# openpifpaf/openpifpaf

Measured on AMD Instinct MI355X. Metric: images/sec end-to-end (backbone+CifCaf decode), resnet50 641px, higher is better.
Workload: dtype f32; 1 GPU; BASELINE configs[1] scaled to a batch: resnet50 641x641, batch 32 per GPU, CIF/CAF fields [32,17,5,81,81]+[32,19,8,81,81]; backbone=resnet50, backbone_dtype=fp32, conv3x3=winograd F(2x2,3x3) f32 for the stride-1 ones, decode_dtype=f32 (+f64 where the reference uses double), global_batch=32, batch_per_gpu=32, parallelism=single GPU, force_complete_pose=False

## Files before the change

### include/openpifpaf_amd.h

```cpp
#ifndef OPENPIFPAF_AMD_H_
#define OPENPIFPAF_AMD_H_

#include <stddef.h>
#include <stdint.h>

#ifdef __cplusplus
extern "C" {
#endif

#define OPA_OK 0
#define OPA_ERR_INVALID_ARGUMENT 1
#define OPA_ERR_HIP 2
#define OPA_ERR_UNSUPPORTED 3
#define OPA_ERR_WORKSPACE 4
#define OPA_ERR_NO_DEVICE 5

#define OPA_COUNT_OVERFLOW 0x40000000
#define OPA_COUNT_FAILED 0x20000000
#define OPA_COUNT_ROWS(c) ((c) & 0x0FFFFFFF)

typedef struct opa_params {
    double cif_threshold;
    int64_t cifhr_neighbors;
    double seed_threshold;
// ... 158 lines not shown
                 int64_t rows, int32_t channels, int32_t dtype, int32_t relu, void* stream);

int opa_gemm_bias_act_bf16(const void* a_dev, const void* w_dev, const void* bias_dev, const void* residual_dev,
                           void* out_dev, int64_t m, int32_t n, int32_t k, int32_t relu, void* stream);

int opa_gemm_pro_bias_act_bf16(const void* a_dev, const void* a_bias_dev, const void* w_dev, const void* bias_dev,
                               const void* residual_dev, void* out_dev, int64_t m, int32_t n, int32_t k,
                               int32_t relu, void* stream);

int opa_gemm_bias_act_f16(const void* a_dev, const void* w_dev, const void* bias_dev, const void* residual_dev,
                          void* out_dev, int64_t m, int32_t n, int32_t k, int32_t relu, void* stream);
int opa_gemm_pro_bias_act_f16(const void* a_dev, const void* a_bias_dev, const void* w_dev, const void* bias_dev,
                              const void* residual_dev, void* out_dev, int64_t m, int32_t n, int32_t k,
                              int32_t relu, void* stream);

int opa_gemm_bias_act_f32(const float* a_dev, const float* a_bias_dev, const float* w_dev, const float* bias_dev,
                          const float* residual_dev, float* out_dev, int64_t m, int32_t n, int32_t k,
                          int32_t relu, void* stream);

int opa_gemm_bias_act_f32x3(const float* a_dev, const float* a_bias_dev, const void* w3_dev, const float* bias_dev,
                            const float* residual_dev, float* out_dev, int64_t m, int32_t n, int32_t k,
                            int32_t relu, int32_t terms, void* stream);

int opa_gemm2_bias_act_f32x3(const float* a1_dev, int32_t k1, const float* a2_dev, int32_t k2, int32_t batch, int32_t h_in,
                             int32_t w_in, int32_t stride, const float* a_bias_dev, const void* w3cat_dev, const float* bias_dev,
                             float* out_dev, int32_t n, int32_t relu, int32_t terms, void* stream);

int opa_conv3x3_f32x3(const float* x_dev, const void* w3_dev, const float* bias_dev, float* out_dev, int32_t batch, int32_t h_in,
                      int32_t w_in, int32_t c_in, int32_t c_out, int32_t stride, int32_t relu, int32_t terms, void* stream);

int opa_conv3x3_dilated_f32x3(const float* x_dev, const void* w3_dev, const float* bias_dev, float* out_dev, int32_t batch, int32_t h_in,
                              int32_t w_in, int32_t c_in, int32_t c_out, int32_t stride, int32_t dilation, int32_t relu, int32_t terms,
                              void* stream);

int opa_maxpool3x3_bias_act(const void* x_dev, const void* bias_dev, void* out_dev, int32_t dtype, int32_t batch, int32_t h, int32_t w,
                            int32_t c, int32_t stride, int32_t relu, void* stream);

int opa_maxpool3x3_ceil_bias_act(const void* x_dev, const void* bias_dev, void* out_dev, int32_t dtype, int32_t batch, int32_t h, int32_t w,
                                 int32_t c, int32_t stride, int32_t relu, void* stream);

int opa_fire_expand_f32x3(const float* h_dev, const void* w_dev, const float* bias_dev, float* out_dev, int32_t batch, int32_t h, int32_t w,
                          int32_t c_squeeze, int32_t c_e1, int32_t c_e3, int32_t terms, void* stream);

int opa_conv_rows_f32x3(const float* x_dev, const void* w3_dev, const float* bias_dev, float* out_dev, int32_t batch, int32_t hp,
                        int32_t wp, int32_t pix, int32_t ho, int32_t wo, int32_t stride, int32_t ntaps, int32_t tap_floats,
                        int32_t c_out, int32_t relu, int32_t terms, void* stream);

int opa_gemm_unit_bias_act_f32x3(const float* a_dev, int64_t a_pitch, const void* w3_dev, const float* bias_dev,
                                 const float* partner_dev, int64_t partner_pitch, float* out_dev,
                                 int64_t m, int32_t n, int32_t k, int32_t relu, int32_t terms, void* stream);

int opa_gemm_unit_act_f32x3(const float* a_dev, int64_t a_pitch, const void* w3_dev, const float* bias_dev,
                            const float* partner_dev, int64_t partner_pitch, const float* residual_dev, int64_t residual_pitch,
                            float* out_dev, int64_t m, int32_t n, int32_t k, int32_t act, int32_t terms, void* stream);

int opa_gemm_unit_actp_f32x3(const float* a_dev, int64_t a_pitch, const void* w3_dev, const float* bias_dev,
                             const float* partner_dev, int64_t partner_pitch, const float* residual_dev, int64_t residual_pitch,
                             float* out_dev, int64_t m, int32_t n, int32_t k, int32_t act, float act_param, int32_t terms, void* stream);

int opa_gemm_unit_actp_bf16(const void* a_dev, int64_t a_pitch, const void* w_dev, const float* bias_dev,
                            const void* partner_dev, int64_t partner_pitch, const void* residual_dev, int64_t residual_pitch,
                            void* out_dev, int64_t m, int32_t n, int32_t k, int32_t act, float act_param, void* stream);

int opa_conv3x3_act_bf16(const void* x_dev, const void* w_dev, const float* bias_dev, const void* residual_dev, void* out_dev,
                         int32_t batch, int32_t h_in, int32_t w_in, int32_t c_in, int32_t c_out,
                         int32_t stride, int32_t dilation, int32_t relu, void* stream);

int opa_conv3x3_act_f16(const void* x_dev, const void* w_dev, const float* bias_dev, const void* residual_dev, void* out_dev,
                        int32_t batch, int32_t h_in, int32_t w_in, int32_t c_in, int32_t c_out,
                        int32_t stride, int32_t dilation, int32_t relu, void* stream);

int opa_gconv3x3_act_bf16(const void* x_dev, const void* w_dev, const float* bias_dev, void* out_dev,
                          int32_t batch, int32_t h_in, int32_t w_in, int32_t channels, int32_t group_width,
                          int32_t stride, int32_t dilation, int32_t relu, void* stream);

int opa_stem7x7_act_bf16(const void* x_dev, int64_t x_batch_stride, int64_t x_channel_stride, int64_t x_row_stride,
                         int64_t x_pixel_stride, const void* w_dev, const float* bias_dev, void* out_dev,
                         int32_t batch, int32_t h, int32_t w, int32_t c_out, int32_t stride, int32_t relu, void* stream);

int opa_gemm2_bias_act_bf16(const void* a1_dev, int32_t k1, const void* a2_dev, int32_t k2, int32_t batch, int32_t h_in, int32_t w_in,
                            int32_t stride, const void* a_bias_dev, const void* wcat_dev, const float* bias_dev, void* out_dev,
                            int32_t n, int32_t relu, void* stream);

int opa_gemm2_bias_act_f16(const void* a1_dev, int32_t k1, const void* a2_dev, int32_t k2, int32_t batch, int32_t h_in, int32_t w_in,
                           int32_t stride, const void* a_bias_dev, const void* wcat_dev, const float* bias_dev, void* out_dev,
                           int32_t n, int32_t relu, void* stream);

int opa_conv3x3_winograd_f32(const float* x_dev, const float* u_dev, const float* bias_dev, float* out_dev, int32_t batch,
                             int32_t h, int32_t w, int32_t c_in, int32_t c_out, int32_t relu, int32_t variant,
                             int32_t order, void* stream);

int opa_conv3x3_winograd_f32x3(const float* x_dev, const void* u3_dev, const float* bias_dev, float* out_dev, int32_t batch,
                               int32_t h, int32_t w, int32_t c_in, int32_t c_out, int32_t relu, int32_t variant,
                               int32_t order, void* stream);

int opa_dwconv_bias_act(const void* x_dev, int64_t x_pixel_stride, const void* w_dev, const void* bias_dev,
                        void* out_dev, int64_t out_pixel_stride, int32_t batch, int32_t h, int32_t w,
                        int32_t channels, int32_t k, int32_t stride, int32_t dtype, int32_t relu, void* stream);

int opa_dwconv_act(const void* x_dev, int64_t x_pixel_stride, const void* w_dev, const void* bias_dev,
                   void* out_dev, int64_t out_pixel_stride, int32_t batch, int32_t h, int32_t w,
                   int32_t channels, int32_t k, int32_t stride, int32_t dtype, int32_t act, void* stream);

int opa_dwconv_dilated_act(const void* x_dev, int64_t x_pixel_stride, const void* w_dev, const void* bias_dev,
                           void* out_dev, int64_t out_pixel_stride, int32_t batch, int32_t h, int32_t w,
                           int32_t channels, int32_t k, int32_t stride, int32_t dilation, int32_t dtype, int32_t act, void* stream);

int opa_dwconv_actp(const void* x_dev, int64_t x_pixel_stride, const void* w_dev, const void* bias_dev,
                    void* out_dev, int64_t out_pixel_stride, int32_t batch, int32_t h, int32_t w,
                    int32_t channels, int32_t k, int32_t stride, int32_t dilation, int32_t dtype, int32_t act, float act_param, void* stream);

int opa_stem3x3_actp(const float* x_dev, int64_t x_batch_stride, int64_t x_channel_stride, int64_t x_row_stride,
                     int64_t x_pixel_stride, const float* w_dev, const float* bias_dev, float* out_dev,
                     int32_t batch, int32_t h, int32_t w, int32_t channels_out, int32_t stride,
                     int32_t act, float act_param, void* stream);

int opa_gconv3x3_bias_act_f32(const float* x_dev, int64_t x_pixel_stride, const float* wt_dev, const float* bias_dev,
                              float* out_dev, int64_t out_pixel_stride, int32_t batch, int32_t h, int32_t w, int32_t channels,
                              int32_t group_width, int32_t stride, int32_t relu, void* stream);

int opa_channel_interleave(const void* a_dev, int64_t a_pixel_stride, const void* b_dev, int64_t b_pixel_stride,
                           void* out_dev, int64_t rows, int32_t half, int32_t dtype, void* stream);

#define OPA_SE_POOL_PIXELS 512
size_t opa_se_workspace_bytes(int32_t batch, int64_t pixels, int32_t channels);
int opa_se_pool(const float* x_dev, int64_t x_pixel_stride, int32_t batch, int64_t pixels, int32_t channels,
                void* workspace_dev, size_t workspace_bytes, void* stream);
int opa_se_gate(const void* workspace_dev, size_t workspace_bytes, int32_t batch, int64_t pixels, int32_t channels, int32_t squeeze,
                const float* w1_dev, const float* b1_dev, const float* w2_dev, const float* b2_dev, float* gate_dev, float* mean_dev,
                void* stream);
int opa_se_scale(float* x_dev, int64_t x_pixel_stride, int32_t batch, int64_t pixels, int32_t channels, const float* gate_dev,
                 void* stream);

#define OPA_GN_CHUNK_PIXELS 512
size_t opa_groupnorm_workspace_bytes(int32_t batch, int64_t pixels, int32_t channels);
int opa_groupnorm_actp(const float* x_dev, int64_t x_pixel_stride, const float* gamma_dev, const float* beta_dev, float* out_dev,
                       int64_t out_pixel_stride, int32_t batch, int64_t pixels, int32_t channels, int32_t groups, float eps,
                       int32_t act, float act_param, void* workspace_dev, size_t workspace_bytes, void* stream);

int opa_head_epilogue(const void* conv_dev, int32_t dtype, int32_t batch, int32_t hc, int32_t wc,
                      int32_t n_fields, int32_t n_components, int32_t upsample, int32_t n_confidences,
                      int32_t n_vectors, uint32_t vector_offset_mask, int32_t n_scales, float* out_dev, void* stream);

int opa_head_conv_fields_bf16(const void* x_dev, const void* w_dev, const float* bias_dev, float* out_dev,
                              int32_t batch, int32_t hc, int32_t wc, int32_t k,
                              int32_t n_fields, int32_t n_components, int32_t upsample, int32_t n_confidences,
                              int32_t n_vectors, uint32_t vector_offset_mask, int32_t n_scales, void* stream);

int opa_head_conv_fields_f16(const void* x_dev, const void* w_dev, const float* bias_dev, float* out_dev,
                             int32_t batch, int32_t hc, int32_t wc, int32_t k,
                             int32_t n_fields, int32_t n_components, int32_t upsample, int32_t n_confidences,
                             int32_t n_vectors, uint32_t vector_offset_mask, int32_t n_scales, void* stream);

typedef struct opa_pre_image {
    int64_t src_offset;
    int64_t mid_offset;
    int32_t h0, w0;
    int32_t th, tw;
    int32_t top, left;
    int32_t x_table, x_ksize;
    int32_t y_table, y_ksize;
} opa_pre_image;
size_t opa_pre_image_bytes(void);

size_t opa_preprocess_workspace_bytes(const opa_pre_image* images_host, int32_t batch, int32_t mode);

int opa_preprocess_u8(const opa_pre_image* images_host, const opa_pre_image* images_dev, int32_t batch,
                      const uint8_t* frames_dev, size_t frames_bytes, const int32_t* tables_dev, size_t tables_words,
                      uint8_t* workspace_dev, size_t workspace_bytes, const float* lut_dev, float* out_dev,
                      int32_t canvas_h, int32_t canvas_w, int32_t mode, int32_t channels_last, uint32_t fill_rgb,
                      void* stream);

int opa_profile_begin(void* stream);
int opa_profile_end(int32_t capacity, const char** names_out, float* ms_out, int32_t* n_out);

#ifdef __cplusplus
}
#endif
#endif
```

### openpifpaf_amd/_lib.py

```python
import ctypes
import os

HERE = os.path.dirname(os.path.abspath(__file__))
LIB_PATH = os.environ.get('OPA_LIB_PATH') or os.path.join(HERE, 'lib', 'libopenpifpaf_amd.so')

OPA_OK = 0
ERROR_NAMES = {1: 'INVALID_ARGUMENT', 2: 'HIP', 3: 'UNSUPPORTED', 4: 'WORKSPACE', 5: 'NO_DEVICE'}


class NativeLibraryMissing(ImportError):
    pass


class NativeError(RuntimeError):
    pass


class Params(ctypes.Structure):
    _fields_ = [
        ('cif_threshold', ctypes.c_double),
        ('cifhr_neighbors', ctypes.c_int64),
        ('seed_threshold', ctypes.c_double),
        ('caf_threshold', ctypes.c_double),
        ('cif_floor', ctypes.c_double),
        ('keypoint_threshold', ctypes.c_double),
        ('keypoint_threshold_rel', ctypes.c_double),
        ('nms_suppression', ctypes.c_double),
        ('nms_instance_threshold', ctypes.c_double),
        ('nms_keypoint_threshold', ctypes.c_double),
        ('force_complete_caf_th', ctypes.c_double),
        ('occupancy_reduction', ctypes.c_double),
        ('occupancy_min_scale', ctypes.c_double),
        ('greedy', ctypes.c_int32),
        ('reverse_match', ctypes.c_int32),
        ('force_complete', ctypes.c_int32),
        ('block_joints', ctypes.c_int32),
        ('ablation_cifseeds_nms', ctypes.c_int32),
        ('ablation_cifseeds_no_rescore', ctypes.c_int32),
        ('ablation_caf_no_rescore', ctypes.c_int32),
        ('ablation_cifhr_skip', ctypes.c_int32),
    ]

    def copy(self):
        other = Params()
        ctypes.memmove(ctypes.byref(other), ctypes.byref(self), ctypes.sizeof(Params))
        return other


ABI_VERSION = 9


class Debug(ctypes.Structure):
    _fields_ = [
        ('stage_worklist', ctypes.c_int32), ('scored_one_pass', ctypes.c_int32),
        ('assoc_growers', ctypes.c_int32), ('assoc_bbox', ctypes.c_int32),
        ('assoc_dedup', ctypes.c_int32), ('assoc_prededup', ctypes.c_int32), ('assoc_predict', ctypes.c_int32),
        ('assoc_predict_min_v', ctypes.c_float), ('assoc_predict_th', ctypes.c_float),
        ('assoc_collide', ctypes.c_int32), ('assoc_collide_shift', ctypes.c_int32), ('assoc_inherit', ctypes.c_int32),
        ('assoc_lookahead', ctypes.c_int32),
        ('assoc_timing', ctypes.c_int32), ('assoc_persistent', ctypes.c_int32), ('fc_split', ctypes.c_int32),
        ('assoc_watchdog_ticks', ctypes.c_int64),
    ]


class DetShape(ctypes.Structure):
    _fields_ = [(n, ctypes.c_int32) for n in ('batch', 'n_fields', 'field_h', 'field_w', 'stride', 'max_detections')]


class DetPost(ctypes.Structure):
    _fields_ = [('iou_threshold', ctypes.c_double), ('suppression', ctypes.c_double),
                ('instance_threshold', ctypes.c_double), ('by_category', ctypes.c_int32)]


CIFDET_NMS_MAX = 1024


class PreImage(ctypes.Structure):
    _fields_ = [('src_offset', ctypes.c_int64), ('mid_offset', ctypes.c_int64)] + [(n, ctypes.c_int32) for n in (
        'h0', 'w0', 'th', 'tw', 'top', 'left', 'x_table', 'x_ksize', 'y_table', 'y_ksize')]


class Shape(ctypes.Structure):
    _fields_ = [(n, ctypes.c_int32) for n in (
        'batch', 'n_cif', 'n_caf', 'cif_h', 'cif_w', 'caf_h', 'caf_w',
        'cif_stride', 'caf_stride', 'max_annotations', 'n_keypoints', 'cifhr_pool_tiles')]


_vp, _i32, _i64, _dbl, _sz = ctypes.c_void_p, ctypes.c_int32, ctypes.c_int64, ctypes.c_double, ctypes.c_size_t
_P = ctypes.POINTER
SYMBOLS = {
    'opa_abi_version': (ctypes.c_int, []),
    'opa_shape_bytes': (_sz, []),
    'opa_params_bytes': (_sz, []),
    'opa_debug_bytes': (_sz, []),
    'opa_default_debug': (None, [_P(Debug)]),
    'opa_cifcaf_set_debug': (ctypes.c_int, [_vp, _P(Debug)]),
    'opa_cifcaf_get_debug': (ctypes.c_int, [_vp, _P(Debug)]),
    'opa_version': (ctypes.c_char_p, []),
    'opa_last_error': (ctypes.c_char_p, []),
    'opa_device_count': (ctypes.c_int, []),
    'opa_set_quiet': (None, [ctypes.c_int]),
    'opa_set_seed_tie_order': (None, [ctypes.c_int]),
    'opa_get_seed_tie_order': (ctypes.c_int, []),
    'opa_default_params': (None, [_P(Params)]),
    'opa_get_params': (None, [_P(Params)]),
    'opa_set_params': (ctypes.c_int, [_P(Params)]),
    'opa_cifcaf_create': (ctypes.c_int, [_P(_vp), _i32, _vp, _i32]),
    'opa_cifcaf_destroy': (None, [_vp]),
    'opa_cifcaf_get_state': (ctypes.c_int, [_vp, _P(_i32), _vp, _P(_i32)]),
    'opa_cifcaf_set_tie_placement': (ctypes.c_int, [_vp, _i32]),
    'opa_cifcaf_workspace_bytes': (_sz, [_P(Shape)]),
    'opa_cifcaf_workspace_bytes_for': (_sz, [_P(Shape), _P(Params)]),
    'opa_cifcaf_decode': (ctypes.c_int, [_vp, _P(Shape), _P(Params), _vp, _vp, _vp, _vp, _i32,
                                         _vp, _sz, _vp, _vp, _vp, _vp]),
    'opa_cifcaf_cifhr_view': (ctypes.c_int, [_P(Shape), _P(_sz), _P(_i32), _P(_i32), _P(_i32), _P(_dbl)]),
    'opa_cifcaf_get_cifhr': (ctypes.c_int, [_P(Shape), _vp, _i32, _vp, _vp]),
    'opa_cifcaf_workspace_view': (ctypes.c_int, [_P(Shape), ctypes.c_char_p, _P(_sz), _P(_sz)]),
    'opa_cifhr_pitch': (_i32, [_i32, _i32]),
    'opa_cifhr_scratch_bytes': (_sz, [_i32, _i32, _i32, _i32]),
    'opa_cifhr_accumulate': (ctypes.c_int, [_vp, _i32, _i32, _i32, _i32, _i32, _dbl, _dbl, _P(Params),
                                            _vp, _vp, _sz, _vp]),
    'opa_cifseeds_scratch_bytes': (_sz, [_i32, _i32, _i32, _i32]),
    'opa_cifseeds_fill': (ctypes.c_int, [_vp, _i32, _i32, _i32, _i32, _i32, _vp, _P(Params),
                                         _vp, _vp, _vp, _vp, _sz, _vp]),
    'opa_cifdetseeds_fill': (ctypes.c_int, [_vp, _i32, _i32, _i32, _i32, _i32, _vp, _P(Params),
                                            _vp, _vp, _vp, _vp, _sz, _vp]),
    'opa_cafscored_fill': (ctypes.c_int, [_vp, _i32, _i32, _i32, _i32, _i32, _vp, _i32, _i32, _i32, _i32,
                                          _vp, _dbl, _dbl, _P(Params), _vp, _vp, _vp]),
    'opa_grow_connection_blend': (ctypes.c_int, [_vp, _i32, _dbl, _dbl, _dbl, _dbl, _i32, _P(_dbl), _vp]),
    'opa_cifdet_workspace_bytes': (_sz, [_P(DetShape)]),
    'opa_cifdet_decode': (ctypes.c_int, [_P(DetShape), _P(Params), _vp, _vp, _sz, _vp, _vp, _vp, _vp, _vp]),
    'opa_det_post_bytes': (_sz, []),
    'opa_default_det_post': (None, [_P(DetPost)]),
    'opa_cifdet_nms': (ctypes.c_int, [_P(DetPost), _i32, _i32, _vp, _vp, _vp, _vp, _vp, _vp, _vp, _vp, _vp]),
    'opa_cifdet_decode_nms': (ctypes.c_int, [_P(DetShape), _P(Params), _P(DetPost), _vp, _vp, _sz, _vp, _vp, _vp, _vp, _vp]),
    'opa_bias_act': (ctypes.c_int, [_vp, _vp, _vp, _i64, _i32, _i32, _i32, _vp]),
    'opa_gemm_bias_act_bf16': (ctypes.c_int, [_vp, _vp, _vp, _vp, _vp, _i64, _i32, _i32, _i32, _vp]),
    'opa_gemm_pro_bias_act_bf16': (ctypes.c_int, [_vp, _vp, _vp, _vp, _vp, _vp, _i64, _i32, _i32, _i32, _vp]),
    'opa_gemm_bias_act_f16': (ctypes.c_int, [_vp, _vp, _vp, _vp, _vp, _i64, _i32, _i32, _i32, _vp]),
    'opa_gemm_pro_bias_act_f16': (ctypes.c_int, [_vp, _vp, _vp, _vp, _vp, _vp, _i64, _i32, _i32, _i32, _vp]),
    'opa_gemm_bias_act_f32': (ctypes.c_int, [_vp, _vp, _vp, _vp, _vp, _vp, _i64, _i32, _i32, _i32, _vp]),
    'opa_gemm_bias_act_f32x3': (ctypes.c_int, [_vp, _vp, _vp, _vp, _vp, _vp, _i64, _i32, _i32, _i32, _i32, _vp]),
    'opa_gemm_unit_bias_act_f32x3': (ctypes.c_int, [_vp, _i64, _vp, _vp, _vp, _i64, _vp, _i64, _i32, _i32, _i32, _i32, _vp]),
    'opa_gemm_unit_act_f32x3': (ctypes.c_int, [_vp, _i64, _vp, _vp, _vp, _i64, _vp, _i64, _vp, _i64, _i32, _i32, _i32, _i32, _vp]),
    'opa_gemm_unit_actp_f32x3': (ctypes.c_int, [_vp, _i64, _vp, _vp, _vp, _i64, _vp, _i64, _vp, _i64, _i32, _i32, _i32, ctypes.c_float, _i32,
                                                _vp]),
    'opa_gemm_unit_actp_bf16': (ctypes.c_int, [_vp, _i64, _vp, _vp, _vp, _i64, _vp, _i64, _vp, _i64, _i32, _i32, _i32, ctypes.c_float, _vp]),
    'opa_conv3x3_act_bf16': (ctypes.c_int, [_vp, _vp, _vp, _vp, _vp] + [_i32] * 8 + [_vp]),
    'opa_conv3x3_act_f16': (ctypes.c_int, [_vp, _vp, _vp, _vp, _vp] + [_i32] * 8 + [_vp]),
    'opa_gconv3x3_act_bf16': (ctypes.c_int, [_vp, _vp, _vp, _vp] + [_i32] * 8 + [_vp]),
    'opa_stem7x7_act_bf16': (ctypes.c_int, [_vp, _i64, _i64, _i64, _i64, _vp, _vp, _vp] + [_i32] * 6 + [_vp]),
    'opa_conv_rows_f32x3': (ctypes.c_int, [_vp, _vp, _vp, _vp] + [_i32] * 12 + [_vp]),
    'opa_conv3x3_f32x3': (ctypes.c_int, [_vp, _vp, _vp, _vp, _i32, _i32, _i32, _i32, _i32, _i32, _i32, _i32, _vp]),
    'opa_conv3x3_dilated_f32x3': (ctypes.c_int, [_vp, _vp, _vp, _vp] + [_i32] * 9 + [_vp]),
    'opa_maxpool3x3_bias_act': (ctypes.c_int, [_vp, _vp, _vp] + [_i32] * 7 + [_vp]),
    'opa_maxpool3x3_ceil_bias_act': (ctypes.c_int, [_vp, _vp, _vp] + [_i32] * 7 + [_vp]),
    'opa_fire_expand_f32x3': (ctypes.c_int, [_vp, _vp, _vp, _vp] + [_i32] * 7 + [_vp]),
    'opa_gemm2_bias_act_f32x3': (ctypes.c_int, [_vp, _i32, _vp, _i32, _i32, _i32, _i32, _i32, _vp, _vp, _vp, _vp, _i32, _i32, _i32, _vp]),
    'opa_gemm2_bias_act_bf16': (ctypes.c_int, [_vp, _i32, _vp, _i32, _i32, _i32, _i32, _i32, _vp, _vp, _vp, _vp, _i32, _i32, _vp]),
    'opa_gemm2_bias_act_f16': (ctypes.c_int, [_vp, _i32, _vp, _i32, _i32, _i32, _i32, _i32, _vp, _vp, _vp, _vp, _i32, _i32, _vp]),
    'opa_conv3x3_winograd_f32': (ctypes.c_int, [_vp, _vp, _vp, _vp] + [_i32] * 8 + [_vp]),
    'opa_conv3x3_winograd_f32x3': (ctypes.c_int, [_vp, _vp, _vp, _vp] + [_i32] * 8 + [_vp]),
    'opa_dwconv_bias_act': (ctypes.c_int, [_vp, _i64, _vp, _vp, _vp, _i64, _i32, _i32, _i32, _i32, _i32, _i32, _i32, _i32, _vp]),
    'opa_dwconv_act': (ctypes.c_int, [_vp, _i64, _vp, _vp, _vp, _i64, _i32, _i32, _i32, _i32, _i32, _i32, _i32, _i32, _vp]),
    'opa_dwconv_dilated_act': (ctypes.c_int, [_vp, _i64, _vp, _vp, _vp, _i64, _i32, _i32, _i32, _i32, _i32, _i32, _i32, _i32, _i32, _vp]),
    'opa_dwconv_actp': (ctypes.c_int, [_vp, _i64, _vp, _vp, _vp, _i64, _i32, _i32, _i32, _i32, _i32, _i32, _i32, _i32, _i32, ctypes.c_float,
                                       _vp]),
    'opa_stem3x3_actp': (ctypes.c_int, [_vp, _i64, _i64, _i64, _i64, _vp, _vp, _vp, _i32, _i32, _i32, _i32, _i32, _i32, ctypes.c_float, _vp]),
    'opa_gconv3x3_bias_act_f32': (ctypes.c_int, [_vp, _i64, _vp, _vp, _vp, _i64, _i32, _i32, _i32, _i32, _i32, _i32, _i32, _vp]),
    'opa_se_workspace_bytes': (_sz, [_i32, _i64, _i32]),
    'opa_se_pool': (ctypes.c_int, [_vp, _i64, _i32, _i64, _i32, _vp, _sz, _vp]),
    'opa_se_gate': (ctypes.c_int, [_vp, _sz, _i32, _i64, _i32, _i32, _vp, _vp, _vp, _vp, _vp, _vp, _vp]),
    'opa_se_scale': (ctypes.c_int, [_vp, _i64, _i32, _i64, _i32, _vp, _vp]),
    'opa_groupnorm_workspace_bytes': (_sz, [_i32, _i64, _i32]),
    'opa_groupnorm_actp': (ctypes.c_int, [_vp, _i64, _vp, _vp, _vp, _i64, _i32, _i64, _i32, _i32, ctypes.c_float, _i32, ctypes.c_float, _vp, _sz,
                                          _vp]),
    'opa_channel_interleave': (ctypes.c_int, [_vp, _i64, _vp, _i64, _vp, _i64, _i32, _i32, _vp]),
    'opa_head_epilogue': (ctypes.c_int, [_vp, _i32, _i32, _i32, _i32, _i32, _i32, _i32, _i32, _i32, ctypes.c_uint32, _i32, _vp, _vp]),
    'opa_head_conv_fields_bf16': (ctypes.c_int, [_vp, _vp, _vp, _vp] + [_i32] * 9 + [ctypes.c_uint32, _i32, _vp]),
    'opa_head_conv_fields_f16': (ctypes.c_int, [_vp, _vp, _vp, _vp] + [_i32] * 9 + [ctypes.c_uint32, _i32, _vp]),
    'opa_pre_image_bytes': (_sz, []),
    'opa_preprocess_workspace_bytes': (_sz, [_P(PreImage), _i32, _i32]),
    'opa_preprocess_u8': (ctypes.c_int, [_P(PreImage), _vp, _i32, _vp, _sz, _vp, _sz, _vp, _sz, _vp, _vp, _i32, _i32, _i32, _i32,
                                         ctypes.c_uint32, _vp]),
    'opa_profile_begin': (ctypes.c_int, [_vp]),
    'opa_profile_end': (ctypes.c_int, [_i32, _P(ctypes.c_char_p), _P(ctypes.c_float), _P(_i32)]),
}

_lib = None


def available():
    return os.path.exists(LIB_PATH)


def lib():
    global _lib
    if _lib is None:
        if not os.path.exists(LIB_PATH):
            raise NativeLibraryMissing(
                'openpifpaf_amd: %s not found. The HIP extension is required (there is no CPU path); '
                'build it with `python -c "import __graft_entry__ as g; g.build()"`.' % LIB_PATH)
        handle = ctypes.CDLL(LIB_PATH)
        for name, (restype, argtypes) in SYMBOLS.items():
            fn = getattr(handle, name)
            fn.restype = restype
            fn.argtypes = argtypes
        if handle.opa_abi_version() != ABI_VERSION or handle.opa_shape_bytes() != ctypes.sizeof(Shape) or \
                handle.opa_params_bytes() != ctypes.sizeof(Params) or handle.opa_debug_bytes() != ctypes.sizeof(Debug) or \
                handle.opa_det_post_bytes() != ctypes.sizeof(DetPost) or \
                handle.opa_pre_image_bytes() != ctypes.sizeof(PreImage):
            raise NativeError('openpifpaf_amd: %s was built from another include/openpifpaf_amd.h (ABI %d, opa_shape %d bytes, '
                              'opa_params %d, opa_debug %d, opa_det_post %d, opa_pre_image %d; this package: ABI %d, %d, %d, %d, %d, %d): '
                              'rebuild it' % (
                                  LIB_PATH, handle.opa_abi_version(), handle.opa_shape_bytes(), handle.opa_params_bytes(),
                                  handle.opa_debug_bytes(), handle.opa_det_post_bytes(), handle.opa_pre_image_bytes(),
                                  ABI_VERSION, ctypes.sizeof(Shape), ctypes.sizeof(Params), ctypes.sizeof(Debug),
                                  ctypes.sizeof(DetPost), ctypes.sizeof(PreImage)))
        _lib = handle
    return _lib


def check(code, what=''):
    if code != OPA_OK:
        msg = lib().opa_last_error().decode('utf-8', 'replace')
        raise NativeError('%s failed: OPA_ERR_%s: %s' % (what or 'native call', ERROR_NAMES.get(code, code), msg))


def default_params(**overrides):
    p = Params()
    lib().opa_default_params(ctypes.byref(p))
    for k, v in overrides.items():
        if not hasattr(p, k):
            raise AttributeError('opa_params has no field %r' % k)
        setattr(p, k, v)
    return p


def default_debug(**overrides):
    d = Debug()
    lib().opa_default_debug(ctypes.byref(d))
    for k, v in overrides.items():
        if not hasattr(d, k):
            raise AttributeError('opa_debug has no field %r' % k)
        setattr(d, k, v)
    return d


def get_params():
    p = Params()
    lib().opa_get_params(ctypes.byref(p))
    return p


def set_params(p):
    check(lib().opa_set_params(ctypes.byref(p)), 'opa_set_params')


def profile_begin(stream_ptr):
    check(lib().opa_profile_begin(stream_ptr), 'opa_profile_begin')


def profile_end(capacity=64):
    names = (ctypes.c_char_p * capacity)()
    ms = (ctypes.c_float * capacity)()
    n = ctypes.c_int32()
    check(lib().opa_profile_end(capacity, names, ms, ctypes.byref(n)), 'opa_profile_end')
    return [(names[i].decode(), float(ms[i])) for i in range(min(n.value, capacity))]
```

### openpifpaf_amd/csrc/capi_trunk.hip

```cpp
#include "capi_internal.hpp"

#include <algorithm>
#include <cmath>
#include <initializer_list>
#include <string>

using namespace opa;

namespace {
struct Entry {
    const char* fn; hipStream_t st;
    Entry(const char* fn_, void* stream) : fn(fn_), st((hipStream_t)stream) {}
    int refuse(int code, const std::string& what) const { return fail(code, std::string(fn) + ": " + what); }
    int refuse(const char* what) const { return refuse(OPA_ERR_INVALID_ARGUMENT, what); }
    int launched(hipError_t e, const char* where, const char* mark = nullptr) const {
        if (e != hipSuccess) return fail_hip(e, where);
        if (mark) prof_mark(st, mark);
        return OPA_OK;
    }
};

bool misaligned(uintptr_t mask, std::initializer_list<const void*> pointers) {
    uintptr_t bits = 0;
    for (const void* p : pointers) bits |= (uintptr_t)p;
    return (bits & mask) != 0;
}

bool bad_terms(int32_t terms) { return terms != 6 && terms != 9; }

const char* bad_act_param(int32_t act, float act_param) {
    if (!std::isfinite(act_param)) return "act_param must be finite";
    if (act == 3 && act_param < 0.0f) return "act_param must not be negative with act 3 (the LeakyReLU's slope)";
    if (act == 4 && act_param <= 0.0f) return "act_param must be positive with act 4 (the clipped ReLU's cap)";
    return nullptr;
}
}

extern "C" {

int opa_bias_act(void* x_dev, const void* bias_dev, const void* residual_dev, int64_t rows, int32_t channels,
                 int32_t dtype, int32_t relu, void* stream) {
    const Entry E("opa_bias_act", stream);
    if (!x_dev || !bias_dev || rows < 0 || channels <= 0 || dtype < 0 || dtype > 2) return E.refuse("bad arguments");
    if (channels % (dtype == 0 ? 4 : 8) != 0 || misaligned(15, {x_dev, bias_dev, residual_dev}))
        return E.refuse("channels must fill 16-byte vectors and pointers be 16-B aligned");
    if (rows == 0) return OPA_OK;
    return E.launched(launch_bias_act(x_dev, bias_dev, residual_dev, rows, channels, dtype, relu, E.st), "bias_act", "bias_act_kernel");
}

static int gemm_bf16(const char* fn, int dtype, bool pro, const void* a_dev, const void* a_bias_dev, const void* w_dev, const void* bias_dev,
                     const void* residual_dev, void* out_dev, int64_t m, int32_t n, int32_t k, int32_t relu, void* stream) {
    const Entry E(fn, stream);
    if (!a_dev || (pro && !a_bias_dev) || !w_dev || !bias_dev || !out_dev || m < 0 || n <= 0 || k <= 0 || m > 0x7fffffffll)
        return E.refuse("bad arguments");
    if (k % 64 != 0 || n % 64 != 0) return E.refuse("K and N must be multiples of 64");
    if (misaligned(15, {a_dev, a_bias_dev, w_dev, out_dev, residual_dev})) return E.refuse("pointers must be 16-B aligned");
    if (m == 0) return OPA_OK;
    const hipError_t e = launch_gemm_bias_act(a_dev, w_dev, bias_dev, residual_dev, out_dev, (int)m, n, k, relu, E.st, a_bias_dev, dtype);
    if (dtype == 1)
        return E.launched(e, pro ? "gemm_pro_bias_act_f16" : "gemm_bias_act_f16", pro ? "gemm_pro_bias_act_f16_kernel" : "gemm_bias_act_f16_kernel");
    return E.launched(e, pro ? "gemm_pro_bias_act" : "gemm_bias_act", pro ? "gemm_pro_bias_act_kernel" : "gemm_bias_act_kernel");
}

int opa_gemm_bias_act_bf16(const void* a_dev, const void* w_dev, const void* bias_dev, const void* residual_dev,
                           void* out_dev, int64_t m, int32_t n, int32_t k, int32_t relu, void* stream) {
    return gemm_bf16("opa_gemm_bias_act_bf16", 2, false, a_dev, nullptr, w_dev, bias_dev, residual_dev, out_dev, m, n, k, relu, stream);
}

int opa_gemm_pro_bias_act_bf16(const void* a_dev, const void* a_bias_dev, const void* w_dev, const void* bias_dev,
                               const void* residual_dev, void* out_dev, int64_t m, int32_t n, int32_t k,
                               int32_t relu, void* stream) {
    return gemm_bf16("opa_gemm_pro_bias_act_bf16", 2, true, a_dev, a_bias_dev, w_dev, bias_dev, residual_dev, out_dev, m, n, k, relu, stream);
}

int opa_gemm_bias_act_f16(const void* a_dev, const void* w_dev, const void* bias_dev, const void* residual_dev,
                          void* out_dev, int64_t m, int32_t n, int32_t k, int32_t relu, void* stream) {
    return gemm_bf16("opa_gemm_bias_act_f16", 1, false, a_dev, nullptr, w_dev, bias_dev, residual_dev, out_dev, m, n, k, relu, stream);
}

int opa_gemm_pro_bias_act_f16(const void* a_dev, const void* a_bias_dev, const void* w_dev, const void* bias_dev,
                              const void* residual_dev, void* out_dev, int64_t m, int32_t n, int32_t k,
                              int32_t relu, void* stream) {
    return gemm_bf16("opa_gemm_pro_bias_act_f16", 1, true, a_dev, a_bias_dev, w_dev, bias_dev, residual_dev, out_dev, m, n, k, relu, stream);
}

int opa_gemm_bias_act_f32(const float* a_dev, const float* a_bias_dev, const float* w_dev, const float* bias_dev,
                          const float* residual_dev, float* out_dev, int64_t m, int32_t n, int32_t k,
                          int32_t relu, void* stream) {
    const Entry E("opa_gemm_bias_act_f32", stream);
    if (!a_dev || !w_dev || !bias_dev || !out_dev || m < 0 || n <= 0 || k <= 0 || m > 0x7fffffffll) return E.refuse("bad arguments");
    if (k % 32 != 0 || n % 64 != 0) return E.refuse("K must be a multiple of 32 and N of 64");
    if (misaligned(15, {a_dev, a_bias_dev, w_dev, out_dev, residual_dev, bias_dev})) return E.refuse("pointers must be 16-B aligned");
    if (m == 0) return OPA_OK;
    return E.launched(launch_gemm_f32_bias_act(a_dev, w_dev, bias_dev, residual_dev, out_dev, (int)m, n, k, relu, E.st, a_bias_dev),
                      "gemm_f32_bias_act", a_bias_dev ? "gemm_f32_pro_bias_act_kernel" : "gemm_f32_bias_act_kernel");
}

int opa_gemm_bias_act_f32x3(const float* a_dev, const float* a_bias_dev, const void* w3_dev, const float* bias_dev,
                            const float* residual_dev, float* out_dev, int64_t m, int32_t n, int32_t k,
                            int32_t relu, int32_t terms, void* stream) {
    const Entry E("opa_gemm_bias_act_f32x3", stream);
    if (!a_dev || !w3_dev || !bias_dev || !out_dev || m < 0 || n <= 0 || k <= 0 || m > 0x7fffffffll || bad_terms(terms))
        return E.refuse("bad arguments");
    if (k % 64 != 0 || n % 64 != 0) return E.refuse("K and N must be multiples of 64");
    if (misaligned(15, {a_dev, a_bias_dev, w3_dev, out_dev, residual_dev, bias_dev})) return E.refuse("pointers must be 16-B aligned");
    if (m == 0) return OPA_OK;
    return E.launched(launch_gemm_f32x3_bias_act(a_dev, (const unsigned short*)w3_dev, bias_dev, residual_dev, out_dev, (int)m, n, k, relu,
                                                 terms, E.st, a_bias_dev), "gemm_f32x3_bias_act", "gemm_f32x3_bias_act_kernel");
}

int opa_gemm2_bias_act_f32x3(const float* a1_dev, int32_t k1, const float* a2_dev, int32_t k2, int32_t batch, int32_t h_in,
                             int32_t w_in, int32_t stride, const float* a_bias_dev, const void* w3cat_dev, const float* bias_dev,
                             float* out_dev, int32_t n, int32_t relu, int32_t terms, void* stream) {
    const Entry E("opa_gemm2_bias_act_f32x3", stream);
    if (!a1_dev || !a2_dev || !w3cat_dev || !bias_dev || !out_dev || batch <= 0 || h_in <= 0 || w_in <= 0 || stride < 1 || n <= 0 ||
        k1 <= 0 || k2 <= 0 || bad_terms(terms))
        return E.refuse("bad arguments");
    if (k1 % 32 != 0 || (k1 + k2) % 64 != 0 || k2 % 4 != 0 || n % 64 != 0) return E.refuse("k1 % 32, (k1 + k2) % 64, k2 % 4, N % 64 must be 0");
    if (misaligned(15, {a1_dev, a2_dev, a_bias_dev, w3cat_dev, out_dev, bias_dev})) return E.refuse("pointers must be 16-B aligned");
    const long long ho = (h_in - 1) / stride + 1, wo = (w_in - 1) / stride + 1;
    if ((long long)batch * ho * wo > 0x7fffffffll || (long long)batch * h_in * w_in > 0x7fffffffll) return E.refuse("too many pixels");
    return E.launched(launch_gemm2_f32x3_bias_act(a1_dev, k1, a2_dev, k2, batch, h_in, w_in, stride, (const unsigned short*)w3cat_dev,
                                                  bias_dev, out_dev, n, relu, terms, E.st, a_bias_dev),
                      "gemm2_f32x3_bias_act", "gemm2_f32x3_bias_act_kernel");
}

int opa_conv_rows_f32x3(const float* x_dev, const void* w3_dev, const float* bias_dev, float* out_dev, int32_t batch, int32_t hp,
                        int32_t wp, int32_t pix, int32_t ho, int32_t wo, int32_t stride, int32_t ntaps, int32_t tap_floats,
                        int32_t c_out, int32_t relu, int32_t terms, void* stream) {
    const Entry E("opa_conv_rows_f32x3", stream);
    if (!x_dev || !w3_dev || !bias_dev || !out_dev || batch <= 0 || hp <= 0 || wp <= 0 || pix <= 0 || ho <= 0 || wo <= 0 || stride < 1 ||
        ntaps < 1 || ntaps > 32 || tap_floats <= 0 || c_out <= 0 || bad_terms(terms))
        return E.refuse("bad arguments");
    if (tap_floats % 32 != 0 || (ntaps * tap_floats) % 64 != 0 || c_out % 64 != 0 || pix % 4 != 0)
        return E.refuse("tap_floats % 32, ntaps * tap_floats % 64, c_out % 64, pix % 4 must be 0");
    if (misaligned(15, {x_dev, w3_dev, out_dev, bias_dev})) return E.refuse("pointers must be 16-B aligned");
    if ((long long)(ho - 1) * stride + ntaps > hp || ((long long)(wo - 1) * stride) * pix + tap_floats > (long long)wp * pix ||
        (long long)batch * hp * wp * pix * 4 > 0x7fffffffll || (long long)batch * ho * wo > 0x7fffffffll)
        return E.refuse("the taps leave the (padded) input, or it is 2 GB or more");
    return E.launched(launch_convrows_f32x3(x_dev, batch, hp, wp, pix, ho, wo, stride, ntaps, tap_floats, (const unsigned short*)w3_dev,
                                            bias_dev, out_dev, c_out, relu, terms, E.st), "conv_rows_f32x3", "conv_rows_f32x3_kernel");
}

static int conv3x3_f32x3(const char* fn, const float* x_dev, const void* w3_dev, const float* bias_dev, float* out_dev, int32_t batch,
                         int32_t h_in, int32_t w_in, int32_t c_in, int32_t c_out, int32_t stride, int32_t dilation, int32_t relu,
                         int32_t terms, void* stream) {
    const Entry E(fn, stream);
    if (!x_dev || !w3_dev || !bias_dev || !out_dev || batch < 0 || h_in < 0 || w_in < 0 || stride < 1 || dilation < 1 || c_in <= 0 ||
        c_out <= 0 || bad_terms(terms))
        return E.refuse("bad arguments");
    if (c_in % 64 != 0 || c_out % 64 != 0) return E.refuse("c_in and c_out must be multiples of 64");
    if (misaligned(15, {x_dev, w3_dev, out_dev, bias_dev})) return E.refuse("pointers must be 16-B aligned");
    if (((double)batch * h_in * w_in + (double)dilation * ((double)w_in + 1.0)) * c_in * 4.0 >= 2147483648.0)
// ... 360 lines not shown
    if (!stem3x3_channels_ok(channels_out)) return E.refuse("channels_out must be 16, 24, 32, 42 or 64");
    if (act < 0 || act > 4) return E.refuse("act must be 0 (none), 1 (ReLU), 2 (hardswish), 3 (LeakyReLU) or 4 (clipped ReLU)");
    if (const char* why = bad_act_param(act, act_param)) return E.refuse(why);
    if (batch == 0) return OPA_OK;
    const double last = ((double)batch - 1.0) * (double)x_batch_stride + 2.0 * (double)x_channel_stride +
                        ((double)h - 1.0) * (double)x_row_stride + ((double)w - 1.0) * (double)x_pixel_stride;
    if (last >= 2147483648.0) return E.refuse("x must span fewer than 2^31 elements (32-bit indices)");
    const double ho = (h - 1) / stride + 1, wo = (w - 1) / stride + 1;
    if ((double)batch * ho * wo * channels_out >= 2147483648.0) return E.refuse("out must hold fewer than 2^31 elements (32-bit indices)");
    if (batch > 65535) return E.refuse("batch must not exceed 65535 (grid.y)");
    return E.launched(launch_stem3x3(x_dev, x_batch_stride, x_channel_stride, x_row_stride, x_pixel_stride, w_dev, bias_dev, out_dev, batch,
                                     h, w, channels_out, stride, act, act_param, E.st), "stem3x3", "stem3x3_kernel");
}

static const char* se_check(int64_t x_pixel_stride, int32_t batch, int64_t pixels, int32_t channels) {
    if (batch <= 0 || batch > 65535 || pixels <= 0 || pixels > 65535ll * kSePoolPixels || channels <= 0 || channels > 8192)
        return "batch, pixels or channels out of range";
    if (channels % 4 != 0 || x_pixel_stride % 4 != 0 || x_pixel_stride < channels) return "channels and the pixel stride must be multiples of 4, the stride >= channels";
    return nullptr;
}

size_t opa_se_workspace_bytes(int32_t batch, int64_t pixels, int32_t channels) {
    if (batch <= 0 || pixels <= 0 || channels <= 0) return 0;
    return (size_t)batch * (size_t)se_pool_chunks(pixels) * (size_t)channels * sizeof(double);
}

int opa_se_pool(const float* x_dev, int64_t x_pixel_stride, int32_t batch, int64_t pixels, int32_t channels,
                void* workspace_dev, size_t workspace_bytes, void* stream) {
    const Entry E("opa_se_pool", stream);
    if (!x_dev || !workspace_dev) return E.refuse("bad arguments");
    if (const char* why = se_check(x_pixel_stride, batch, pixels, channels)) return E.refuse(why);
    if (misaligned(15, {x_dev, workspace_dev})) return E.refuse("pointers must be 16-B aligned");
    if (workspace_bytes < opa_se_workspace_bytes(batch, pixels, channels)) return E.refuse(OPA_ERR_WORKSPACE, "the workspace is too small");
    return E.launched(launch_se_pool(x_dev, x_pixel_stride, batch, pixels, channels, (double*)workspace_dev, E.st), "se pool");
}

int opa_se_gate(const void* workspace_dev, size_t workspace_bytes, int32_t batch, int64_t pixels, int32_t channels, int32_t squeeze,
                const float* w1_dev, const float* b1_dev, const float* w2_dev, const float* b2_dev, float* gate_dev, float* mean_dev,
                void* stream) {
    const Entry E("opa_se_gate", stream);
    if (!workspace_dev || !w1_dev || !b1_dev || !w2_dev || !b2_dev || !gate_dev || squeeze <= 0 || squeeze > 4096)
        return E.refuse("bad arguments");
    if (const char* why = se_check(channels, batch, pixels, channels)) return E.refuse(why);
    if (misaligned(15, {workspace_dev})) return E.refuse("workspace_dev must be 16-B aligned");
    if (workspace_bytes < opa_se_workspace_bytes(batch, pixels, channels)) return E.refuse(OPA_ERR_WORKSPACE, "the workspace is too small");
    return E.launched(launch_se_gate((const double*)workspace_dev, batch, pixels, channels, squeeze, w1_dev, b1_dev, w2_dev, b2_dev,
                                     gate_dev, mean_dev, E.st), "se gate");
}

int opa_se_scale(float* x_dev, int64_t x_pixel_stride, int32_t batch, int64_t pixels, int32_t channels, const float* gate_dev,
                 void* stream) {
    const Entry E("opa_se_scale", stream);
    if (!x_dev || !gate_dev) return E.refuse("bad arguments");
    if (const char* why = se_check(x_pixel_stride, batch, pixels, channels)) return E.refuse(why);
    if (misaligned(15, {x_dev, gate_dev})) return E.refuse("pointers must be 16-B aligned");
    return E.launched(launch_se_scale(x_dev, x_pixel_stride, batch, pixels, channels, gate_dev, E.st), "se scale");
}

size_t opa_groupnorm_workspace_bytes(int32_t batch, int64_t pixels, int32_t channels) {
    if (batch <= 0 || pixels <= 0 || channels <= 0) return 0;
    return groupnorm_partial_bytes(batch, pixels, channels) + (size_t)batch * (size_t)channels * 2 * sizeof(float);
}

int opa_groupnorm_actp(const float* x_dev, int64_t x_pixel_stride, const float* gamma_dev, const float* beta_dev, float* out_dev,
                       int64_t out_pixel_stride, int32_t batch, int64_t pixels, int32_t channels, int32_t groups, float eps,
                       int32_t act, float act_param, void* workspace_dev, size_t workspace_bytes, void* stream) {
    const Entry E("opa_groupnorm_actp", stream);
    if (!x_dev || !out_dev) return E.refuse("x_dev and out_dev must not be NULL");
    if (misaligned(7, {x_dev, out_dev}) || misaligned(3, {gamma_dev, beta_dev}) || misaligned(15, {workspace_dev}))
        return E.refuse("x_dev / out_dev must be 8-B, gamma_dev / beta_dev 4-B, workspace_dev 16-B aligned");
    if (batch < 0 || pixels <= 0 || channels <= 0 || groups <= 0)
        return E.refuse("batch must not be negative, pixels, channels and groups must be positive");
    if (channels % groups != 0) return E.refuse("channels must be a multiple of groups");
    if ((channels / groups) % 2 != 0) return E.refuse("channels / groups must be even");
    if (x_pixel_stride % 2 != 0 || out_pixel_stride % 2 != 0 || x_pixel_stride < channels || out_pixel_stride < channels)
        return E.refuse("pixel strides must be even and at least channels");
    if (!std::isfinite(eps) || eps < 0.0f) return E.refuse("eps must be finite and not negative");
    if (act < 0 || act > 4) return E.refuse("act must be 0 (none), 1 (ReLU), 2 (hardswish), 3 (LeakyReLU) or 4 (clipped ReLU)");
    if (const char* why = bad_act_param(act, act_param)) return E.refuse(why);
    if (out_dev == x_dev && out_pixel_stride != x_pixel_stride) return E.refuse("out_dev == x_dev (in place) needs equal pixel strides");
    if (batch == 0) return OPA_OK;
    if (batch > 65535) return E.refuse("batch must not exceed 65535 (grid.y)");
    if (pixels > 65535ll * kGnChunkPixels) return E.refuse("pixels must not exceed 65535 * OPA_GN_CHUNK_PIXELS (grid.y)");
    if (channels / groups > kGnMaxGroupWidth) return E.refuse("channels / groups must not exceed 2048");
    if ((double)pixels * (double)(channels / 2) >= 2147483648.0)
        return E.refuse("pixels * channels / 2 must stay below 2^31 (32-bit vector indices within an image)");
    if (!workspace_dev) return E.refuse(OPA_ERR_WORKSPACE, "workspace_dev must not be NULL");
    if (workspace_bytes < opa_groupnorm_workspace_bytes(batch, pixels, channels)) return E.refuse(OPA_ERR_WORKSPACE, "the workspace is too small");
    return E.launched(launch_groupnorm(x_dev, x_pixel_stride, gamma_dev, beta_dev, out_dev, out_pixel_stride, batch, pixels, channels, groups,
                                       eps, act, act_param, workspace_dev, E.st), "group norm");
}

int opa_channel_interleave(const void* a_dev, int64_t a_pixel_stride, const void* b_dev, int64_t b_pixel_stride,
                           void* out_dev, int64_t rows, int32_t half, int32_t dtype, void* stream) {
    const Entry E("opa_channel_interleave", stream);
    if (!a_dev || !b_dev || !out_dev || rows <= 0 || half <= 0 || a_pixel_stride < half || b_pixel_stride < half ||
        dtype < 0 || dtype > 2)
        return E.refuse("bad arguments");
    return E.launched(launch_channel_interleave(a_dev, a_pixel_stride, b_dev, b_pixel_stride, out_dev, rows, half, dtype, E.st),
                      "channel interleave");
}

int opa_head_epilogue(const void* conv_dev, int32_t dtype, int32_t batch, int32_t hc, int32_t wc,
                      int32_t n_fields, int32_t n_components, int32_t upsample, int32_t n_confidences,
                      int32_t n_vectors, uint32_t vector_offset_mask, int32_t n_scales, float* out_dev, void* stream) {
    const Entry E("opa_head_epilogue", stream);
    if (!conv_dev || !out_dev || batch <= 0 || hc <= 0 || wc <= 0 || n_fields <= 0 || n_components <= 0 ||
        dtype < 0 || dtype > 2 || (upsample != 1 && upsample != 2) || n_confidences < 0 || n_vectors < 0 || n_scales < 0 ||
        1 + n_confidences + 2 * n_vectors + n_scales > n_components)
        return E.refuse("bad arguments");
    return E.launched(launch_head_epilogue(conv_dev, dtype, batch, hc, wc, n_fields, n_components, upsample, n_confidences,
                                           n_vectors, vector_offset_mask, n_scales, out_dev, E.st), "head epilogue");
}

static int head_conv_fields_16(const char* fn, int dtype, const void* x_dev, const void* w_dev, const float* bias_dev, float* out_dev,
                               int32_t batch, int32_t hc, int32_t wc, int32_t k, int32_t n_fields, int32_t n_components, int32_t upsample,
                               int32_t n_confidences, int32_t n_vectors, uint32_t vector_offset_mask, int32_t n_scales, void* stream) {
    const Entry E(fn, stream);
    if (!x_dev || !w_dev || !bias_dev || !out_dev) return E.refuse("x_dev, w_dev, bias_dev and out_dev must not be NULL");
    if (misaligned(15, {x_dev, w_dev}) || misaligned(3, {bias_dev, out_dev}))
        return E.refuse("x_dev / w_dev must be 16-B, bias_dev / out_dev 4-B aligned");
    if (batch < 0) return E.refuse("negative batch");
    if (hc <= 0 || wc <= 0 || k <= 0 || n_fields <= 0 || n_components <= 0) return E.refuse("hc, wc, k, n_fields and n_components must be positive");
    if (k % 64 != 0) return E.refuse("k must be a multiple of 64");
    if (upsample != 1 && upsample != 2) return E.refuse("upsample must be 1 or 2");
    if (n_confidences < 0 || n_vectors < 0 || n_scales < 0 || 1ll + n_confidences + 2ll * n_vectors + n_scales != n_components)
        return E.refuse("n_components must be 1 + n_confidences + 2 * n_vectors + n_scales, no count negative");
    const double pixels = (double)batch * hc * wc, n = (double)n_fields * n_components * upsample * upsample;
    if (pixels * k >= 2147483648.0) return E.refuse("x must hold fewer than 2^31 elements (32-bit offsets)");
    if (n > 2147483584.0) return E.refuse("n_fields * n_components * upsample^2 must not exceed 2^31 - 64");
    const double ho = (double)hc * upsample - (upsample - 1), wo = (double)wc * upsample - (upsample - 1);
    if ((double)batch * n_fields * n_components * ho * wo >= 2147483648.0) return E.refuse("out must hold fewer than 2^31 elements (32-bit offsets)");
    if (batch == 0) return OPA_OK;
    if (head16_workgroups(batch, hc, wc, n_fields, n_components, upsample) > 0x7fffffffll) return E.refuse("too many tiles for grid.x");
    return E.launched(launch_head16(x_dev, w_dev, bias_dev, out_dev, batch, hc, wc, k, n_fields, n_components, upsample, n_confidences, n_vectors,
                                    vector_offset_mask, n_scales, E.st, dtype), dtype == 1 ? "head_conv_fields_f16" : "head_conv_fields_bf16",
                      dtype == 1 ? "head16_f16_kernel" : "head16_bf16_kernel");
}

int opa_head_conv_fields_bf16(const void* x_dev, const void* w_dev, const float* bias_dev, float* out_dev,
                              int32_t batch, int32_t hc, int32_t wc, int32_t k,
                              int32_t n_fields, int32_t n_components, int32_t upsample, int32_t n_confidences,
                              int32_t n_vectors, uint32_t vector_offset_mask, int32_t n_scales, void* stream) {
    return head_conv_fields_16("opa_head_conv_fields_bf16", 2, x_dev, w_dev, bias_dev, out_dev, batch, hc, wc, k, n_fields, n_components, upsample,
                               n_confidences, n_vectors, vector_offset_mask, n_scales, stream);
}

int opa_head_conv_fields_f16(const void* x_dev, const void* w_dev, const float* bias_dev, float* out_dev,
                             int32_t batch, int32_t hc, int32_t wc, int32_t k,
                             int32_t n_fields, int32_t n_components, int32_t upsample, int32_t n_confidences,
                             int32_t n_vectors, uint32_t vector_offset_mask, int32_t n_scales, void* stream) {
    return head_conv_fields_16("opa_head_conv_fields_f16", 1, x_dev, w_dev, bias_dev, out_dev, batch, hc, wc, k, n_fields, n_components, upsample,
                               n_confidences, n_vectors, vector_offset_mask, n_scales, stream);
}

size_t opa_pre_image_bytes(void) { return sizeof(opa_pre_image); }

static size_t pre_mid_bytes(const opa_pre_image& d) { return align_up((size_t)d.h0 * (((size_t)d.tw * 3 + 15) & ~(size_t)15)); }

static bool check_pre_sizes(const opa_pre_image* images, int32_t batch, const char* who, std::string* why) {
    if (!images) { *why = std::string(who) + ": images_host is null"; return false; }
    if (batch < 1 || batch > 65535) { *why = std::string(who) + ": batch must be 1..65535"; return false; }
    for (int32_t b = 0; b < batch; b++) {
        const opa_pre_image& d = images[b];
        const char* field = d.h0 < 1 ? "h0" : d.w0 < 1 ? "w0" : d.th < 1 ? "th" : d.tw < 1 ? "tw" : nullptr;
        if (field) { *why = std::string(who) + ": images[" + std::to_string(b) + "]." + field + " must be at least 1"; return false; }
        if ((int64_t)d.h0 * d.w0 > 0x3fffffff || (int64_t)d.h0 * d.tw > 0x3fffffff) {
            *why = std::string(who) + ": images[" + std::to_string(b) + "]: h0 * w0 and h0 * tw must stay below 2^30"; return false;
        }
    }
    return true;
}

size_t opa_preprocess_workspace_bytes(const opa_pre_image* images_host, int32_t batch, int32_t mode) {
    std::string why;
    if (!check_pre_sizes(images_host, batch, "opa_preprocess_workspace_bytes", &why)) { fail(0, why); return 0; }
    if (mode != 0 && mode != 1) { fail(0, "opa_preprocess_workspace_bytes: mode must be 0 or 1"); return 0; }
    size_t total = 0;
    if (mode == 0)
        for (int32_t b = 0; b < batch; b++)
            if (images_host[b].tw != images_host[b].w0) total += pre_mid_bytes(images_host[b]);
    return total;
}

int opa_preprocess_u8(const opa_pre_image* images_host, const opa_pre_image* images_dev, int32_t batch,
                      const uint8_t* frames_dev, size_t frames_bytes, const int32_t* tables_dev, size_t tables_words,
                      uint8_t* workspace_dev, size_t workspace_bytes, const float* lut_dev, float* out_dev,
                      int32_t canvas_h, int32_t canvas_w, int32_t mode, int32_t channels_last, uint32_t fill_rgb,
                      void* stream) {
    const char* who = "opa_preprocess_u8";
    auto bad = [&](const std::string& what) { return fail(OPA_ERR_INVALID_ARGUMENT, std::string(who) + ": " + what); };
    if (!images_dev) return bad("images_dev is null");
    if (!frames_dev) return bad("frames_dev is null");
    if (!tables_dev) return bad("tables_dev is null");
    if (!lut_dev) return bad("lut_dev is null");
    if (!out_dev) return bad("out_dev is null");
    std::string why;
    if (!check_pre_sizes(images_host, batch, who, &why)) return fail(OPA_ERR_INVALID_ARGUMENT, why);
    if (mode != 0 && mode != 1) return bad("mode must be 0 (Pillow) or 1 (zoom)");
    if (canvas_h < 1 || canvas_h > 65535) return bad("canvas_h must be 1..65535");
    if (canvas_w < 1) return bad("canvas_w must be at least 1");
    if (((uintptr_t)frames_dev | (uintptr_t)tables_dev | (uintptr_t)workspace_dev | (uintptr_t)images_dev) & 15)
        return bad("frames_dev, tables_dev, workspace_dev and images_dev must be 16-B aligned");
    if (frames_bytes % 16) return bad("frames_bytes must be a multiple of 16");
    unsigned h_blocks = 0;
    int in_cap = 1;
    size_t ws_need = 0;
    for (int32_t b = 0; b < batch; b++) {
        const opa_pre_image& d = images_host[b];
        const std::string at = "images[" + std::to_string(b) + "].";
        if (d.top < 0 || d.left < 0 || (int64_t)d.top + d.th > canvas_h || (int64_t)d.left + d.tw > canvas_w)
            return bad(at + "top / left: the placement lies outside the canvas");
        if (d.x_ksize < 1) return bad(at + "x_ksize must be at least 1");
        if (d.y_ksize < 1) return bad(at + "y_ksize must be at least 1");
        if (d.src_offset < 0 || (uint64_t)d.src_offset + (uint64_t)d.h0 * d.w0 * 3 > frames_bytes)
            return bad(at + "src_offset: the frame lies outside frames_bytes");
        const size_t x_words = mode ? ((3 * (size_t)d.tw + 1) & ~(size_t)1) + 4 * (size_t)d.tw : (size_t)(1 + d.x_ksize) * d.tw;
        const size_t y_words = mode ? ((3 * (size_t)d.th + 1) & ~(size_t)1) + 4 * (size_t)d.th : (size_t)(1 + d.y_ksize) * d.th;
        if (d.x_table < 0 || d.x_table % 4 || (size_t)d.x_table + x_words > tables_words)
            return bad(at + "x_table: the table lies outside tables_words or is not a multiple of 4 words");
        if (d.y_table < 0 || d.y_table % 4 || (size_t)d.y_table + y_words > tables_words)
            return bad(at + "y_table: the table lies outside tables_words or is not a multiple of 4 words");
        double span;
        if (mode) {
            if (d.x_ksize != 2 || d.y_ksize != 2) return bad(at + "x_ksize / y_ksize must be 2 in mode 1");
            span = std::ceil(255.0 * (d.tw > 1 ? (double)(d.w0 - 1) / (d.tw - 1) : 0.0)) + 3.0;
        } else if (d.tw != d.w0) {
            const double scale = (double)d.w0 / d.tw;
            span = std::ceil(255.0 * scale) + 2.0 * std::ceil(std::max(scale, 1.0)) + 4.0;
            if (d.mid_offset < 0 || d.mid_offset % 16) return bad(at + "mid_offset must be a non-negative multiple of 16");
            ws_need = std::max(ws_need, (size_t)d.mid_offset + pre_mid_bytes(d));
            const unsigned chunks = ((unsigned)d.tw + 255u) / 256u;
            h_blocks = std::max(h_blocks, (unsigned)d.h0 * chunks);
        } else {
            span = 1.0;
        }
        in_cap = std::max(in_cap, (int)std::min(span, (double)d.w0));
    }
    const size_t lds = mode ? preprocess_zoom_lds_bytes(in_cap) : preprocess_h_lds_bytes(in_cap);
    if (lds > 65536) return bad("w0 / tw: 256 output columns reach more source pixels than 64 KB of LDS hold");
    if (ws_need > 0 && !workspace_dev) return bad("workspace_dev is null");
    if (ws_need > workspace_bytes)
        return fail(OPA_ERR_WORKSPACE, std::string(who) + ": workspace_bytes is " + std::to_string(workspace_bytes) + ", the batch needs " + std::to_string(ws_need));
    hipError_t e = launch_preprocess(images_dev, batch, frames_dev, tables_dev, workspace_dev, lut_dev, out_dev, canvas_h, canvas_w,
                                     mode, channels_last, fill_rgb, h_blocks, in_cap, (hipStream_t)stream);
    if (e != hipSuccess) return fail_hip(e, "image preprocessing");
    return OPA_OK;
}

}
```

### openpifpaf_amd/csrc/common.hpp

```cpp
#pragma once

#include <hip/hip_runtime.h>
#include <stdint.h>
#include <stddef.h>
#include <type_traits>

#include "../../include/openpifpaf_amd.h"

namespace opa {

constexpr int kWave = 64;
constexpr int kHrTileW = 64;
constexpr int kHrTileH = 32;
constexpr int kHrLdsPitch = kHrTileW + 16;
constexpr int kSortLdsKeys = 8192;

struct Layout {
    int B, F, K, A, H, W, cH, cW, stride, cstride, max_ann;
    int hr_rows, hr_cols, hr_pitch;
    int hr_tpp, hr_pool_cap;
    int hr_spill_cap;
    int occ_h, occ_w;
    int cif_cells;
    int caf_cells;
// ... 119 lines not shown

struct AssocArgs {
    int B, K, F, A, max_ann, n_initial;
    int hr_rows, hr_cols;
    int occ_h, occ_w;
    int seed_cap, list_cap;
    const int32_t* seed_f; const float* seed_vxys; const int32_t* seed_count;
    const int32_t* seed_cell;
    const float* lists; const int32_t* list_counts;
    const float* lists_fc; const int32_t* list_counts_fc;
    const float* list_bbox;
    const float* list_bbox_fc;
    int bbox_chunks;
    const int32_t* hr_overflow;
    int tie_fused;
    TieArgs tie; SortArgs tie_sort;
    int timing;
    int collide;
    int inherit;
    size_t private_bytes;
    int dedup;
    const float* caf_raw; int caf_w; float caf_stride;
    int coll_shift;
    int lookahead;
    float predict_min_v;
    int predict; float predict_th;
    int prededup;
    int32_t* fc_meta;
    long long watchdog_ticks;
    int32_t* queue_order; int32_t* queue_head;
    int max_growers, fc_split;
    unsigned* occ;
    size_t occ_image_words;
    int32_t* stats;
    int32_t* trace;
    double* anns;
    int64_t* ann_ids;
    const float* initial; const int64_t* initial_ids;
    float* out; int64_t* out_ids; int32_t* out_count;
    int32_t* status;
};
void make_tie_args(TieArgs* a, SortArgs* g, unsigned long long* keys, int sort_cap, const int32_t* seed_count, const float* cif,
                   int F, int NC, int HW, int stride, int32_t* seed_f, float* seed_vxys, int32_t* seed_cell, int occ_h, int occ_w,
                   const TieScratch& t);
hipError_t launch_cifseeds_ties(const TieArgs& a, const SortArgs& g, int B, const DevParams& p, hipStream_t st);
hipError_t launch_assoc(const AssocArgs& a, const DevSkeleton& sk, const DevParams& p, hipStream_t st, const opa_debug& dbg);

struct DetArgs {
    int B, F, max_det, occ_h, occ_w, seed_cap;
    const int32_t* seed_f; const float* seed_vxywh; const int32_t* seed_count;
    unsigned char* occ;
    int64_t* categories; float* scores; float* boxes; int32_t* counts;
};
hipError_t launch_cifdet_collect(const DetArgs& a, const DevParams& p, hipStream_t st);

constexpr int kDetNmsMax = 1024;
struct DetNmsArgs {
    int B, max_det, by_category;
    double iou_threshold; float suppression, instance_threshold;
    const int64_t* categories; const float* scores; const float* boxes; const int32_t* counts;
    int64_t* out_categories; float* out_scores; float* out_boxes; int32_t* out_counts;
};
size_t cifdet_nms_lds_bytes(int max_det);
hipError_t launch_cifdet_nms(const DetNmsArgs& a, hipStream_t st);

hipError_t launch_bias_act(void* x, const void* bias, const void* res, long long rows, int channels, int dtype,
                           int relu, hipStream_t st);

template <auto... Vs, typename T, typename F>
hipError_t with_value(T v, F&& f) {
    hipError_t e = hipErrorInvalidValue;
    (void)((v == Vs && (e = f(std::integral_constant<decltype(Vs), Vs>{}), true)) || ...);
    return e;
}
template <typename F>
hipError_t with_flag(bool v, F&& f) { return with_value<false, true>(v, f); }

hipError_t launch_gemm_bias_act(const void* A, const void* W, const void* bias, const void* res, void* out,
                                int M, int N, int K, int relu, hipStream_t st, const void* a_bias, int dtype);

hipError_t launch_gemm_f32x3_bias_act(const float* A, const unsigned short* W3, const float* bias, const float* res, float* out,
                                      int M, int N, int K, int relu, int terms, hipStream_t st, const float* a_bias);
hipError_t launch_gemm2_f32x3_bias_act(const float* A1, int K1, const float* A2, int K2, int batch, int hi, int wi, int stride,
                                       const unsigned short* W3, const float* bias, float* out, int N, int relu, int terms,
                                       hipStream_t st, const float* a_bias);
hipError_t launch_convrows_f32x3(const float* x, int batch, int hp, int wp, int pix, int ho, int wo, int stride, int ntaps, int tap_floats,
                                 const unsigned short* W3, const float* bias, float* out, int N, int relu, int terms, hipStream_t st);
hipError_t launch_conv3x3_f32x3(const float* x, int batch, int hi, int wi, int C, int stride, int dilation, const unsigned short* W3,
                                const float* bias, float* out, int N, int relu, int terms, hipStream_t st);
int maxpool3x3_out(int h, int ceil_mode);
long long maxpool3x3_blocks(int B, int H, int W, int C, int ceil_mode = 0);
hipError_t launch_maxpool3x3(const void* x, const void* bias, void* out, int dtype, int B, int H, int W, int C, int relu, hipStream_t st,
                             int ceil_mode = 0);
bool stem3x3_channels_ok(int C);
long long stem3x3_tiles(int H, int W, int S);
hipError_t launch_stem3x3(const float* x, long long xb, long long xc, long long xr, long long xp, const float* w, const float* bias,
                          float* out, int B, int H, int W, int C, int S, int act, float act_param, hipStream_t st);
long long fire_expand_workgroups(int B, int H, int W);
hipError_t launch_fire_expand(const float* h, const unsigned short* w3, const float* bias, float* out, int B, int H, int W, int S,
                              int E1, int E3, int terms, hipStream_t st);
hipError_t launch_gemm_unit_act_f32x3(const float* A, int lda, const unsigned short* W3, const float* bias, const float* partner, int ldp,
                                      const float* residual, int ldr, float* out, int M, int N, int K, int act, int terms, hipStream_t st,
                                      float act_param = 0.0f);
hipError_t launch_gemm_unit_act_bf16(const void* A, long long lda, const void* W, const float* bias, const void* partner, long long ldp,
                                     const void* residual, long long ldr, void* out, int M, int n, int k, int act, float act_param,
                                     hipStream_t st);
long long conv3x3_bf16_workgroups(int B, int H, int W, int c_out, int S);
hipError_t launch_conv3x3_bf16(const void* x, const void* w, const float* bias, const void* residual, void* out, int B, int H, int W,
                               int c_in, int c_out, int S, int D, int relu, hipStream_t st, int dtype);
long long gconv3x3_bf16_workgroups(int B, int H, int W, int C, int S);
hipError_t launch_gconv3x3_bf16(const void* x, const void* w, const float* bias, void* out, int B, int H, int W, int C, int CG, int S,
                                int D, int relu, hipStream_t st);
long long stem7x7_bf16_workgroups(int B, int H, int W, int c_out, int S);
hipError_t launch_stem7x7_bf16(const void* x, long long xb, long long xc, long long xr, long long xp, const void* w, const float* bias,
                               void* out, int B, int H, int W, int c_out, int S, int relu, hipStream_t st);
long long gemm2_bf16_workgroups(int B, int H, int W, int n, int S);
hipError_t launch_gemm2_bf16(const void* a1, int k1, const void* x, int k2, int B, int H, int W, int S, const void* a_bias,
                             const void* wcat, const float* bias, void* out, int n, int relu, hipStream_t st, int dtype);
hipError_t launch_gemm_f32_bias_act(const float* A, const float* W, const float* bias, const float* res, float* out,
                                    int M, int N, int K, int relu, hipStream_t st, const float* a_bias = nullptr);
hipError_t launch_winograd_f23(const float* x, const float* U, float* y, const float* bias, int N, int H, int W, int Cin,
                               int Cout, int relu, int variant, int nb_major, hipStream_t st);
hipError_t launch_winograd_f23x3(const float* x, const unsigned short* U3, float* y, const float* bias, int N, int H, int W,
                                 int Cin, int Cout, int relu, int variant, int nb_major, hipStream_t st);

hipError_t launch_dwconv(const void* x, long long xs, const void* w, const void* bias, void* out, long long os,
                         int B, int H, int W, int C, int K, int S, int D, int dtype, int act, hipStream_t st, float cap = 0.0f);
hipError_t launch_channel_interleave(const void* a, long long as, const void* b, long long bs, void* out,
                                     long long rows, int half, int dtype, hipStream_t st);

long long gconv3x3_workgroups(int H, int W, int C, int S);
hipError_t launch_gconv3x3(const float* x, long long xs, const float* wt, const float* bias, float* out, long long os,
                           int B, int H, int W, int C, int CG, int S, int relu, hipStream_t st);

constexpr int kSePoolPixels = 512;
inline long long se_pool_chunks(long long hw) { return (hw + kSePoolPixels - 1) / kSePoolPixels; }
hipError_t launch_se_pool(const float* x, long long xs, int B, long long HW, int C, double* partial, hipStream_t st);
hipError_t launch_se_gate(const double* partial, int B, long long HW, int C, int S, const float* w1, const float* b1,
                          const float* w2, const float* b2, float* gate, float* mean_out, hipStream_t st);
hipError_t launch_se_scale(float* x, long long xs, int B, long long HW, int C, const float* gate, hipStream_t st);

constexpr int kGnChunkPixels = 512;
constexpr int kGnMaxGroupWidth = 2048;
inline long long gn_chunks(long long hw) { return (hw + kGnChunkPixels - 1) / kGnChunkPixels; }
size_t groupnorm_partial_bytes(int B, long long HW, int C);
hipError_t launch_groupnorm(const float* x, long long xs, const float* gamma, const float* beta, float* out, long long os, int B,
                            long long HW, int C, int G, float eps, int act, float act_param, void* workspace, hipStream_t st);

hipError_t launch_head_epilogue(const void* conv, int dtype, int B, int Hc, int Wc, int n_fields, int n_comp, int us,
                                int n_conf, int n_vec, unsigned offset_mask, int n_scales, float* out, hipStream_t st);
long long head16_workgroups(int B, int hc, int wc, int n_fields, int n_comp, int us);
hipError_t launch_head16(const void* x, const void* w, const float* bias, float* out, int B, int hc, int wc, int K, int n_fields,
                         int n_comp, int us, int n_conf, int n_vec, unsigned offset_mask, int n_scales, hipStream_t st, int dtype);

size_t preprocess_h_lds_bytes(int in_cap);
size_t preprocess_zoom_lds_bytes(int in_cap);
hipError_t launch_preprocess(const opa_pre_image* images, int batch, const unsigned char* frames, const int32_t* tables,
                             unsigned char* ws, const float* lut, float* out, int ch, int cw, int precise, int channels_last,
                             unsigned fill, unsigned h_blocks, int in_cap, hipStream_t st);

hipError_t launch_blend(const float* rows, int n, double x, double y, double s, double filter_sigmas,
                        int only_max, double* out4_dev, hipStream_t st);

}

#ifdef __HIPCC__
namespace opa {

__device__ __forceinline__ void sync_global() {
    __builtin_amdgcn_fence(__ATOMIC_RELEASE, "workgroup");
    __builtin_amdgcn_s_waitcnt(0x0F70);
    __builtin_amdgcn_s_barrier();
    __builtin_amdgcn_fence(__ATOMIC_ACQUIRE, "agent");
}

__device__ __forceinline__ int seed_cell_pack(const DevParams& p, int occ_h, int occ_w, double x, double y, double sigma);

__device__ __forceinline__ int lane_id() { return threadIdx.x & (kWave - 1); }

__device__ __forceinline__ float hardsigmoid_f32(float x) { return fminf(fmaxf(x + 3.0f, 0.0f), 6.0f) / 6.0f; }
__device__ __forceinline__ float hardswish_f32(float x) { return x * fminf(fmaxf(x + 3.0f, 0.0f), 6.0f) / 6.0f; }

__device__ __forceinline__ float x3_act_param(float x, int act, float p) {
    if (act == 3) return x < 0.0f ? x * p : x;
    return x < 0.0f ? 0.0f : (x > p ? p : x);
}

__device__ __forceinline__ float act_f32(float x, int act, float p) {
    if (act == 0) return x;
    if (act == 1) return x < 0.0f ? 0.0f : x;
    if (act == 2) return hardswish_f32(x);
    return x3_act_param(x, act, p);
}

__device__ __forceinline__ long long clampll(long long v, long long lo, long long hi) {
    return v < lo ? lo : (v > hi ? hi : v);
}

__device__ __forceinline__ long long trunc_ll(float v) { return (long long)v; }
__device__ __forceinline__ long long trunc_ll(double v) { return (long long)v; }

__device__ __forceinline__ int seed_cell_pack(const DevParams& p, int occ_h, int occ_w, double x, double y, double sigma) {
    if (p.occupancy_inv_reduction != 0.0) {
        x *= p.occupancy_inv_reduction; y *= p.occupancy_inv_reduction;
        sigma = fmax(p.occupancy_min_scale_reduced, sigma * p.occupancy_inv_reduction);
    } else if (p.occupancy_reduction != 1.0) {
        x /= p.occupancy_reduction; y /= p.occupancy_reduction;
        sigma = fmax(p.occupancy_min_scale_reduced, sigma / p.occupancy_reduction);
    }
    const int xi = (int)clampll(trunc_ll(x), 0, occ_w - 1), yi = (int)clampll(trunc_ll(y), 0, occ_h - 1);
    const int half = (int)fmin(fmax(sigma, 1.0), 255.0);
    return xi | (yi << 12) | (half << 24);
}

__device__ __forceinline__ float cifhr_value(const float* hr_image, int F, int rows, int cols, int pitch,
                                             long long f, float x, float y, float default_value,
                                             const unsigned* touch = nullptr, int touch_words = 0, int tiles_x = 0,
                                             const int32_t* slot = nullptr, int tpp = 0) {
    const float max_x = (float)((double)(float)cols - 0.51);
    const float max_y = (float)((double)(float)rows - 0.51);
    if (f >= F || (double)x < -0.49 || (double)y < -0.49 || x > max_x || y > max_y) return default_value;
    const long long yi = (long long)((double)y + 0.5);
    const long long xi = (long long)((double)x + 0.5);
    float raw;
    if (slot) {
        const int t = (int)(yi / kHrTileH) * tiles_x + (int)(xi / kHrTileW);
        const int sl = slot[(size_t)f * tpp + t];
        if (sl < 0) return default_value;
        raw = hr_image[(size_t)sl * (kHrTileH * kHrTileW) + (size_t)(yi % kHrTileH) * kHrTileW + (size_t)(xi % kHrTileW)];
    } else {
        if (touch) {
            const int t = (int)(yi / kHrTileH) * tiles_x + (int)(xi / kHrTileW);
            if (!((touch[(size_t)f * touch_words + (t >> 5)] >> (t & 31)) & 1u)) return default_value;
        }
        raw = hr_image[((size_t)f * rows + yi) * pitch + xi];
    }
    const float value = (float)((double)raw - 1.0);
    if ((double)value < 0.0) return default_value;
    return value;
}

}
#endif
```

### openpifpaf_amd/csrc/gemm_f32x3.hip

```cpp
#include <cstdlib>
#include <type_traits>
#include "common.hpp"
#include "split_bf16.hpp"

namespace opa {

typedef __attribute__((ext_vector_type(8))) __bf16 bf16x8_t;
typedef __attribute__((ext_vector_type(16))) float f32x16_t;
typedef __attribute__((ext_vector_type(4))) float f32x4_t;
typedef __attribute__((ext_vector_type(4))) unsigned int u32x4_t;
typedef __attribute__((ext_vector_type(2))) unsigned int u32x2_t;
typedef __attribute__((ext_vector_type(2))) float f32x2_t;

#ifndef OPA_X3_BK
#define OPA_X3_BK 32
#endif
#ifndef OPA_X3_WGS
#define OPA_X3_WGS 2
#endif
#ifndef OPA_X3_DIAG
#define OPA_X3_DIAG 0
#endif
#ifndef OPA_X3_ONE_ACC
#define OPA_X3_ONE_ACC 0
#endif
#ifndef OPA_X3_SWIZZLE
#define OPA_X3_SWIZZLE 1
#endif
constexpr int kX3BM = 128, kX3BK = OPA_X3_BK, kX3Pitch = OPA_X3_SWIZZLE ? kX3BK : kX3BK + 8;
__device__ __forceinline__ int x3_lds(int row, int k) {
    if (OPA_X3_SWIZZLE && kX3BK == 32) return row * kX3Pitch + ((((k >> 3) ^ (row >> 2)) & 3) << 3) + (k & 7);
    return row * kX3Pitch + k;
}

struct X3Second {
    const float* A2 = nullptr;
    int K1 = 0;
    int ho_wo = 1, wo = 1, hi_wi = 1, wi = 1, stride = 1;
    int hi = 1, C = 0, batch = 1;
    int pix = 1, taps_x = 1, ntaps = 1, padded = 0;
    int dil = 1;
    int lda = 0, ldp = 0, n_real = 0, k_real = 0;
    int act = 0; float act_param = 0.0f;
};

constexpr int kUxAct = 3, kUxHardswish = 2, kUxResidual = 4, kUxActParam = 8;

template <int BN, bool PARTNER, bool RELU, int UX = 0>
__device__ __forceinline__ void x3_unit_epilogue(float* smem_f, const f32x16_t (&acc)[2][BN / 64], const f32x16_t (&low)[2][BN / 64],
                                                 const float* __restrict__ bias, const float* __restrict__ partner,
                                                 float* __restrict__ out, int M, int m0, int n0, int lane, int wave, int ldp, int n_real,
                                                 int act, float act_param) {
    constexpr int WN = BN / 2, NT = WN / 32;
    constexpr int PPR = WN / 2;
    constexpr int PPL = 32 * PPR / 64;
    constexpr int PPRE = PPL > 8 ? 8 : PPL;
    const int wm = wave >> 1, wn = wave & 1;
    float* patch = smem_f + wave * (32 * WN);
#pragma unroll
    for (int i = 0; i < 2; i++) {
        f32x2_t pv[PPRE];
        if (PARTNER) {
#pragma unroll
            for (int t = 0; t < PPRE; t++) {
                const int v = t * 64 + lane;
                const int row = v / PPR, col = n0 + wn * WN + (v % PPR) * 2;
                const int m = m0 + wm * 64 + i * 32 + row;
                pv[t] = (f32x2_t){0.f, 0.f};
                if (m < M && col < n_real) pv[t] = *reinterpret_cast<const f32x2_t*>(partner + (size_t)m * ldp + col);
            }
        }
#pragma unroll
        for (int j = 0; j < NT; j++) {
            const int col = j * 32 + (lane & 31);
            const float b = bias[n0 + wn * WN + col];
#pragma unroll
            for (int r = 0; r < 16; r++) {
                const int row = (r & 3) + 8 * (r >> 2) + 4 * (lane >> 5);
                patch[row * WN + col] = (OPA_X3_ONE_ACC ? acc[i][j][r] : acc[i][j][r] + low[i][j][r]) + b;
            }
        }
        __builtin_amdgcn_fence(__ATOMIC_ACQ_REL, "wavefront");
        __builtin_amdgcn_wave_barrier();
#pragma unroll
        for (int t = 0; t < PPL; t++) {
            const int v = t * 64 + lane;
            const int row = v / PPR, c2 = (v % PPR) * 2, col = n0 + wn * WN + c2;
            const int m = m0 + wm * 64 + i * 32 + row;
            if (m < M && col < n_real) {
                f32x2_t f = *reinterpret_cast<const f32x2_t*>(patch + row * WN + c2);
                if constexpr (PARTNER && (UX & kUxResidual) != 0) {
                    f32x2_t pp;
                    if (t < PPRE) pp = pv[t < PPRE ? t : 0];
                    else pp = *reinterpret_cast<const f32x2_t*>(partner + (size_t)m * ldp + col);
                    f[0] += pp[0]; f[1] += pp[1];
                }
                if (RELU) { f[0] = fmaxf(f[0], 0.0f); f[1] = fmaxf(f[1], 0.0f); }
                if constexpr ((UX & kUxAct) == kUxHardswish) { f[0] = hardswish_f32(f[0]); f[1] = hardswish_f32(f[1]); }
                if constexpr ((UX & kUxActParam) != 0) { f[0] = x3_act_param(f[0], act, act_param); f[1] = x3_act_param(f[1], act, act_param); }
                if (PARTNER && (UX & kUxResidual) == 0) {
                    f32x2_t pp;
                    if (t < PPRE) pp = pv[t < PPRE ? t : 0];
                    else pp = *reinterpret_cast<const f32x2_t*>(partner + (size_t)m * ldp + col);
                    *reinterpret_cast<f32x4_t*>(out + (size_t)m * (2 * (size_t)n_real) + 2 * col) = (f32x4_t){pp[0], f[0], pp[1], f[1]};
                } else {
                    *reinterpret_cast<f32x2_t*>(out + (size_t)m * n_real + col) = f;
                }
            }
        }
        __builtin_amdgcn_fence(__ATOMIC_ACQ_REL, "wavefront");
        __builtin_amdgcn_wave_barrier();
        asm volatile("" ::: "memory");
    }
}

template <int BN, bool RES, bool RELU, bool PRO, int TERMS, int SRC, bool UNIT = false, int UX = 0>
__global__ __launch_bounds__(256, OPA_X3_WGS) void gemm_f32x3_bias_act_kernel(
        const float* __restrict__ A, const unsigned short* __restrict__ W3, const float* __restrict__ bias,
        const float* __restrict__ res, float* __restrict__ out, int M, int N, int K, const float* __restrict__ a_bias,
        const X3Second sec) {
    constexpr int WN = BN / 2;
    constexpr int NT = WN / 32;
    constexpr int LDS_A = kX3BM * kX3Pitch, LDS_B = BN * kX3Pitch;
#ifndef OPA_X3_PAD_LDS
#define OPA_X3_PAD_LDS 0
#endif
    constexpr int STAGE_BYTES = 3 * (LDS_A + LDS_B) * 2 + OPA_X3_PAD_LDS;
    constexpr int EPI_BYTES = 4 * 32 * WN * 4;
    constexpr int SMEM_BYTES = STAGE_BYTES > EPI_BYTES ? STAGE_BYTES : EPI_BYTES;
    __shared__ __attribute__((aligned(16))) unsigned char smem[SMEM_BYTES + (RES && !UNIT ? BN * 4 : 0)];
    unsigned short* sA = reinterpret_cast<unsigned short*>(smem);
    unsigned short* sB = sA + 3 * LDS_A;

    const int tid = threadIdx.x, lane = tid & 63, wave = tid >> 6;
    const int wm = wave >> 1, wn = wave & 1;
    const int n_tiles = N / BN;
    const unsigned nwg = gridDim.x, xcd = blockIdx.x & 7u, in_xcd = blockIdx.x >> 3;
    const unsigned q = nwg >> 3, r8 = nwg & 7u;
    const unsigned logical = (xcd < r8 ? xcd * (q + 1) : r8 * (q + 1) + (xcd - r8) * q) + in_xcd;
    const int m0 = (int)(logical / n_tiles) * kX3BM;
    const int n0 = (int)(logical % n_tiles) * BN;

    constexpr int NL = OPA_X3_ONE_ACC ? 1 : 2;
    f32x16_t acc[2][NT], low_[NL][NT];
    f32x16_t (&low)[2][NT] = OPA_X3_ONE_ACC ? acc : reinterpret_cast<f32x16_t (&)[2][NT]>(low_);
#pragma unroll
    for (int i = 0; i < 2; i++)
#pragma unroll
        for (int j = 0; j < NT; j++)
#pragma unroll
            for (int r = 0; r < 16; r++) { acc[i][j][r] = 0.0f; if (!OPA_X3_ONE_ACC) low[i][j][r] = 0.0f; }

    constexpr int VA = kX3BK / 4;
    constexpr int RPP = 256 / VA;
    constexpr int NPA = kX3BM / RPP;
    constexpr int WQ = kX3BK / 8;
    const int s_row = tid / VA, s_col = (tid % VA) * 4;
    constexpr int WTOT = 3 * BN * WQ;
    constexpr int WV = (WTOT + 255) / 256;
    f32x4_t ra0[NPA], ra1[NPA];
    u32x4_t rb[WV];
    constexpr bool TWO = SRC == 1, TAPS = SRC == 2;
    const int rows_here = M - m0 < kX3BM ? M - m0 : kX3BM;
    const int KA = TWO ? sec.K1 : TAPS ? sec.C : UNIT ? sec.lda : K;
    const int shift = TAPS && !sec.padded ? sec.dil * (sec.wi + 1) * sec.pix : 0;
    const float* a1_base = TAPS ? A - (size_t)shift : A + (size_t)m0 * KA;
    const int a1_bytes = TAPS ? (int)(((size_t)sec.batch * sec.hi_wi * sec.pix + shift) * 4)
                       : UNIT ? (int)(((size_t)(rows_here - 1) * KA + sec.k_real) * 4) : (int)((size_t)rows_here * KA * 4);
    const __amdgpu_buffer_rsrc_t a_rsrc = __builtin_amdgcn_make_buffer_rsrc(const_cast<float*>(a1_base), 0, a1_bytes, 0x00020000);
    const int K2 = K - KA;
    auto in_row = [&](int m) -> long long {
        const int b = m / sec.ho_wo, r = m - b * sec.ho_wo, oy = r / sec.wo, ox = r - oy * sec.wo;
        return (long long)b * sec.hi_wi + (long long)oy * sec.stride * sec.wi + (long long)ox * sec.stride;
    };
    long long row0_2 = 0;
    const float* a2_base = nullptr;
    int a2_bytes = 0;
    unsigned pa2[NPA];
    if constexpr (TWO) {
        row0_2 = in_row(__builtin_amdgcn_readfirstlane(m0));
        const int m_end = m0 + rows_here - 1;
        a2_base = sec.A2 + (size_t)row0_2 * K2;
        a2_bytes = (int)((size_t)(in_row(__builtin_amdgcn_readfirstlane(m_end)) - row0_2 + 1) * K2 * 4);
    }
    const __amdgpu_buffer_rsrc_t w_rsrc = __builtin_amdgcn_make_buffer_rsrc(
        const_cast<unsigned short*>(W3 + (size_t)n0 * K), 0, (int)(((size_t)3 * N - n0) * K * 2), 0x00020000);
    unsigned pa[NPA], pb[WV];
    unsigned vmask[NPA];
    int sb_off[WV];
#pragma unroll
    for (int p = 0; p < NPA; p++) {
        int m = m0 + p * RPP + s_row;
        if (m > M - 1) m = M - 1;
        pa[p] = ((unsigned)(m - m0) * (unsigned)KA + (unsigned)s_col) * 4u;
        vmask[p] = 0u;
        if constexpr (TAPS) {
            const int b = m / sec.ho_wo, r = m - b * sec.ho_wo, oy = r / sec.wo, ox = r - oy * sec.wo;
            pa[p] = (unsigned)((long long)b * sec.hi_wi + (long long)oy * sec.stride * sec.wi + (long long)ox * sec.stride) * (unsigned)sec.pix * 4u
                    + (unsigned)s_col * 4u;
            if (sec.padded) vmask[p] = 0xffffffffu;
            else
                for (int t = 0; t < sec.ntaps; t++) {
                    const int iy = oy * sec.stride - sec.dil + sec.dil * (t / sec.taps_x), ix = ox * sec.stride - sec.dil + sec.dil * (t % sec.taps_x);
                    if (iy >= 0 && iy < sec.hi && ix >= 0 && ix < sec.wi) vmask[p] |= 1u << t;
                }
        }
        if constexpr (TWO) pa2[p] = ((unsigned)(in_row(m) - row0_2) * (unsigned)K2 + (unsigned)s_col) * 4u;
    }
#pragma unroll
    for (int t = 0; t < WV; t++) {
        const int v = t * 256 + tid < WTOT ? t * 256 + tid : WTOT - 1;
        const int plane = v / (BN * WQ), rem = v - plane * (BN * WQ), row = rem / WQ, c = (rem % WQ) * 8;
        pb[t] = (((unsigned)plane * (unsigned)N + (unsigned)row) * (unsigned)K + (unsigned)c) * 2u;
        sb_off[t] = plane * LDS_B + x3_lds(row, c);
    }
    auto fetch_a = [&](f32x4_t (&ra)[NPA], int k0) {
        if constexpr (TAPS) {
            const int t = k0 / KA, kc = k0 - t * KA;
            const int soff = (int)((((unsigned)(sec.dil * (t / sec.taps_x)) * (unsigned)sec.wi + (unsigned)(sec.dil * (t % sec.taps_x))) * (unsigned)sec.pix + (unsigned)kc) * 4u);
#pragma unroll
            for (int p = 0; p < NPA; p++)
                ra[p] = __builtin_bit_cast(f32x4_t, __builtin_amdgcn_raw_buffer_load_b128(a_rsrc, (vmask[p] >> t) & 1u ? pa[p] : 0xFFFFFFF0u, soff, 0));
        } else if constexpr (TWO) {
            const bool second = k0 >= KA;
            const __amdgpu_buffer_rsrc_t rs = __builtin_amdgcn_make_buffer_rsrc(
                const_cast<float*>(second ? a2_base : a1_base), 0, second ? a2_bytes : a1_bytes, 0x00020000);
            const int ks = (second ? k0 - KA : k0) * 4;
#pragma unroll
            for (int p = 0; p < NPA; p++)
                ra[p] = __builtin_bit_cast(f32x4_t, __builtin_amdgcn_raw_buffer_load_b128(rs, second ? pa2[p] : pa[p], ks, 0));
        } else if constexpr (UNIT) {
#pragma unroll
            for (int p = 0; p < NPA; p++) {
                const f32x2_t lo = __builtin_bit_cast(f32x2_t, __builtin_amdgcn_raw_buffer_load_b64(a_rsrc, pa[p], k0 * 4, 0));
                const f32x2_t hi = __builtin_bit_cast(f32x2_t, __builtin_amdgcn_raw_buffer_load_b64(a_rsrc, pa[p] + 8u, k0 * 4, 0));
                ra[p] = (f32x4_t){lo[0], lo[1], hi[0], hi[1]};
            }
        } else {
#pragma unroll
            for (int p = 0; p < NPA; p++) ra[p] = __builtin_bit_cast(f32x4_t, __builtin_amdgcn_raw_buffer_load_b128(a_rsrc, pa[p], k0 * 4, 0));
        }
        if (PRO) {
            const f32x4_t ab = *reinterpret_cast<const f32x4_t*>(a_bias + k0 + s_col);
#pragma unroll
            for (int p = 0; p < NPA; p++)
#pragma unroll
                for (int e = 0; e < 4; e++) ra[p][e] = fmaxf(ra[p][e] + ab[e], 0.0f);
        }
    };
    auto fetch_b = [&](int k0) {
#pragma unroll
        for (int t = 0; t < WV; t++) rb[t] = __builtin_bit_cast(u32x4_t, __builtin_amdgcn_raw_buffer_load_b128(w_rsrc, pb[t], k0 * 2, 0));
    };
    auto store = [&](const f32x4_t (&ra)[NPA], int kt) {
#pragma unroll
        for (int p = 0; p < NPA; p++) {
            u32x2_t p1, p2, p3;
            if (OPA_X3_DIAG == 1) { p1[0] = __float_as_uint(ra[p][0]); p1[1] = __float_as_uint(ra[p][2]); p2 = p1; p3 = p1; }
            else if constexpr (UNIT) {
                const bool in0 = kt + s_col < sec.k_real, in1 = kt + s_col + 2 < sec.k_real;
                const f32x4_t v = {in0 ? ra[p][0] : 0.0f, in0 ? ra[p][1] : 0.0f, in1 ? ra[p][2] : 0.0f, in1 ? ra[p][3] : 0.0f};
                split4(v, p1, p2, p3);
            }
            else split4(ra[p], p1, p2, p3);
            unsigned short* d = sA + x3_lds(p * RPP + s_row, s_col);
            *reinterpret_cast<u32x2_t*>(d) = p1;
            *reinterpret_cast<u32x2_t*>(d + LDS_A) = p2;
            *reinterpret_cast<u32x2_t*>(d + 2 * LDS_A) = p3;
        }
#pragma unroll
        for (int t = 0; t < WV; t++)
            if (WTOT % 256 == 0 || t * 256 + tid < WTOT) *reinterpret_cast<u32x4_t*>(sB + sb_off[t]) = rb[t];
    };
    constexpr int VEC_PER_ROW = WN / 4;
    constexpr int VPL = 32 * VEC_PER_ROW / 64;
    constexpr int VRA = 1;
    constexpr bool TAIL_RES = RES && !UNIT;
    f32x4_t rres[2][TAIL_RES ? VPL : 1];
    auto fetch_res = [&](int i, int t_begin, int t_end) {
        if constexpr (TAIL_RES) {
            const __amdgpu_buffer_rsrc_t r_rsrc = __builtin_amdgcn_make_buffer_rsrc(
                const_cast<float*>(res + (size_t)m0 * N + n0), 0, (int)(((size_t)(rows_here - 1) * N + BN) * 4), 0x00020000);
            const int lrow = wm * 64 + lane / VEC_PER_ROW;
            const unsigned off = ((unsigned)lrow * (unsigned)N + (unsigned)(wn * WN + (lane % VEC_PER_ROW) * 4)) * 4u;
#pragma unroll
            for (int t = t_begin; t < t_end; t++) {
                const int urow = i * 32 + t * (64 / VEC_PER_ROW);
                rres[i][t] = __builtin_bit_cast(f32x4_t, __builtin_amdgcn_raw_buffer_load_b128(
                    r_rsrc, lrow < rows_here - urow ? off : 0xFFFFFFF0u, urow * N * 4, 0));
            }
        }
    };
    int frag_a[kX3BK / 16], frag_b[kX3BK / 16];
    if constexpr (TAIL_RES) {
#pragma unroll
        for (int h = 0; h < kX3BK / 16; h++) {
            frag_a[h] = 2 * x3_lds(wm * 64 + (lane & 31), h * 16 + (lane >> 5) * 8);
            frag_b[h] = 2 * x3_lds(wn * WN + (lane & 31), h * 16 + (lane >> 5) * 8);
            asm volatile("" : "+v"(frag_a[h]), "+v"(frag_b[h]));
        }
    }
    auto step = [&](auto tail, int k0, f32x4_t (&cur)[NPA], f32x4_t (&nxt)[NPA]) {
        constexpr int TAIL = decltype(tail)::value;
        const bool more = TAIL == 1 || (TAIL == 0 && k0 + kX3BK < K);
        const int k_last = K - kX3BK;
        if constexpr (TAIL == 0) {
            fetch_b(k0 + kX3BK < k_last ? k0 + kX3BK : k_last);
            fetch_a(nxt, k0 + 2 * kX3BK < k_last ? k0 + 2 * kX3BK : k_last);
        } else if constexpr (TAIL == 1) {
            fetch_b(k_last);
            fetch_res(0, 0, VRA);
        } else {
            fetch_res(0, VRA, VPL);
        }
        __builtin_amdgcn_sched_barrier(0);
#pragma unroll
        for (int kk = 0; kk < kX3BK; kk += 16) {
            bf16x8_t fa[3][2], fb[3][NT];
            const int kh = OPA_X3_DIAG == 4 ? 0 : kk / 16;
            const int kof = kh * 16 + (lane >> 5) * 8;
#pragma unroll
            for (int pl = 0; pl < 3; pl++) {
#pragma unroll
                for (int i = 0; i < 2; i++)
                    fa[pl][i] = *reinterpret_cast<const bf16x8_t*>(TAIL_RES ? reinterpret_cast<const unsigned short*>(smem + frag_a[kh]) + (pl * LDS_A + i * 32 * kX3Pitch)
                                                                       : sA + pl * LDS_A + x3_lds(wm * 64 + i * 32 + (lane & 31), kof));
#pragma unroll
                for (int j = 0; j < NT; j++)
                    fb[pl][j] = *reinterpret_cast<const bf16x8_t*>(TAIL_RES ? reinterpret_cast<const unsigned short*>(smem + frag_b[kh]) + (3 * LDS_A + pl * LDS_B + j * 32 * kX3Pitch)
                                                                       : sB + pl * LDS_B + x3_lds(wn * WN + j * 32 + (lane & 31), kof));
            }
#pragma unroll
            for (int i = 0; i < 2; i++)
#pragma unroll
                for (int j = 0; j < NT; j++)
                    acc[i][j] = __builtin_amdgcn_mfma_f32_32x32x16_bf16(fa[0][i], fb[0][j], acc[i][j], 0, 0, 0);
#pragma unroll
            for (int s = 4; s >= 1; s--) {
                if ((TERMS == 6 && s > 2) || OPA_X3_DIAG == 3) continue;
#pragma unroll
                for (int pa_ = 0; pa_ < 3; pa_++) {
                    const int pb_ = s - pa_;
                    if (pb_ < 0 || pb_ > 2) continue;
#pragma unroll
                    for (int i = 0; i < 2; i++)
#pragma unroll
                        for (int j = 0; j < NT; j++)
                            low[i][j] = __builtin_amdgcn_mfma_f32_32x32x16_bf16(fa[pa_][i], fb[pb_][j], low[i][j], 0, 0, 0);
                }
            }
        }
        __syncthreads();
        if (more && (OPA_X3_DIAG != 2 || cur[0][0] == 12345.678f)) store(cur, k0 + kX3BK);
        __syncthreads();
    };
    fetch_b(0);
    fetch_a(ra0, 0);
    if constexpr (TAIL_RES) {
        if (tid < BN) reinterpret_cast<float*>(smem + SMEM_BYTES)[tid] = bias[n0 + tid];
    }
    store(ra0, 0);
    __syncthreads();
    fetch_a(ra1, kX3BK);
    constexpr std::integral_constant<int, 0> any_step{};
    if constexpr (TAIL_RES) {
        int k0 = 0;
        for (; k0 < K - 2 * kX3BK; k0 += 2 * kX3BK) {
            step(any_step, k0, ra1, ra0);
            step(any_step, k0 + kX3BK, ra0, ra1);
        }
        step(std::integral_constant<int, 1>{}, k0, ra1, ra0);
        step(std::integral_constant<int, 2>{}, k0 + kX3BK, ra0, ra1);
    } else {
        for (int k0 = 0; k0 < K; k0 += 2 * kX3BK) {
            step(any_step, k0, ra1, ra0);
            step(any_step, k0 + kX3BK, ra0, ra1);
        }
    }
    if constexpr (UNIT) {
        x3_unit_epilogue<BN, RES, RELU, UX>(reinterpret_cast<float*>(smem), acc, low, bias, res, out, M, m0, n0, lane, wave, sec.ldp, sec.n_real,
                                            sec.act, sec.act_param);
        return;
    }

    float* patch = reinterpret_cast<float*>(smem) + wave * (32 * WN);
    if constexpr (TAIL_RES) {
        fetch_res(1, 0, VPL);
        __builtin_amdgcn_sched_barrier(0);
    }
#pragma unroll
    for (int i = 0; i < 2; i++) {
#pragma unroll
        for (int j = 0; j < NT; j++) {
            const int col = j * 32 + (lane & 31);
            const float b = TAIL_RES ? reinterpret_cast<const float*>(smem + SMEM_BYTES)[wn * WN + col] : bias[n0 + wn * WN + col];
#pragma unroll
            for (int r = 0; r < 16; r++) {
                const int row = (r & 3) + 8 * (r >> 2) + 4 * (lane >> 5);
                patch[row * WN + col] = (OPA_X3_ONE_ACC ? acc[i][j][r] : acc[i][j][r] + low[i][j][r]) + b;
            }
        }
        __builtin_amdgcn_fence(__ATOMIC_ACQ_REL, "wavefront");
        __builtin_amdgcn_wave_barrier();
#pragma unroll
        for (int t = 0; t < VPL; t++) {
            const int v = t * 64 + lane;
            const int row = v / VEC_PER_ROW, c4 = (v % VEC_PER_ROW) * 4;
            const int m = m0 + wm * 64 + i * 32 + row;
            if (m < M) {
                f32x4_t f = *reinterpret_cast<const f32x4_t*>(patch + row * WN + c4);
                if constexpr (TAIL_RES) f += rres[i][t];
                if (RELU) {
#pragma unroll
                    for (int e = 0; e < 4; e++) f[e] = fmaxf(f[e], 0.0f);
                }
                *reinterpret_cast<f32x4_t*>(out + (size_t)m * N + n0 + wn * WN + c4) = f;
            }
        }
        __builtin_amdgcn_fence(__ATOMIC_ACQ_REL, "wavefront");
        __builtin_amdgcn_wave_barrier();
        asm volatile("" ::: "memory");
    }
}

#if OPA_X3_BK == 32 && OPA_X3_SWIZZLE && !OPA_X3_ONE_ACC && OPA_X3_DIAG == 0
#define OPA_X3_HAS_WIDE 1
constexpr int kX3WideBN = 256, kX3WideThreads = 512;
constexpr int kX3WideStageBytes = 3 * (kX3BM + kX3WideBN) * kX3Pitch * 2;
constexpr int kX3WideLdsBytes = 2 * kX3WideStageBytes + kX3WideBN * 4;
constexpr unsigned kX3WideCUs = 256;
constexpr int kX3WideMinKRes = 768;
constexpr bool x3_wide_pays(unsigned long long wide_blocks, bool res, int K) {
    if (res && K < kX3WideMinKRes) return false;
    const unsigned long long rounds = (wide_blocks + kX3WideCUs - 1) / kX3WideCUs;
    return wide_blocks >= 2 * kX3WideCUs && rounds * kX3WideCUs * 15 <= (wide_blocks + kX3WideCUs / 4) * 16;
}

template <bool RES, bool RELU, bool PRO, int SRC>
__global__ __launch_bounds__(kX3WideThreads, 2) void gemm_f32x3_wide_kernel(
        const float* __restrict__ A, const unsigned short* __restrict__ W3, const float* __restrict__ bias,
        const float* __restrict__ res, float* __restrict__ out, int M, int N, int K, const float* __restrict__ a_bias,
        const X3Second sec) {
    constexpr int BN = kX3WideBN, WN = 64, NT = 2;
    constexpr int LDS_A = kX3BM * kX3Pitch, LDS_B = BN * kX3Pitch;
    static_assert(kX3WideThreads / 64 * 32 * WN * 4 <= kX3WideStageBytes, "the epilogue patches alias stage 0 alone");
    extern __shared__ __attribute__((aligned(16))) unsigned char x3w_smem[];
    float* s_bias = reinterpret_cast<float*>(x3w_smem + 2 * kX3WideStageBytes);

    const int tid = threadIdx.x, lane = tid & 63, wave = __builtin_amdgcn_readfirstlane(tid >> 6);
    const int wm = wave >> 2, wn = wave & 3;
    const int n_tiles = N / BN;
    const unsigned nwg = gridDim.x, xcd = blockIdx.x & 7u, in_xcd = blockIdx.x >> 3;
    const unsigned q = nwg >> 3, r8 = nwg & 7u;
    const unsigned logical = (xcd < r8 ? xcd * (q + 1) : r8 * (q + 1) + (xcd - r8) * q) + in_xcd;
    const int m0 = (int)(logical / n_tiles) * kX3BM;
    const int n0 = (int)(logical % n_tiles) * BN;

    f32x16_t acc[2][NT], low[2][NT];
#pragma unroll
    for (int i = 0; i < 2; i++)
#pragma unroll
        for (int j = 0; j < NT; j++)
#pragma unroll
            for (int r = 0; r < 16; r++) { acc[i][j][r] = 0.0f; low[i][j][r] = 0.0f; }

    constexpr int VA = kX3BK / 4, RPP = kX3WideThreads / VA, NPA = kX3BM / RPP, WV = 6;
    static_assert(NPA == 2 && 3 * BN * (kX3BK / 8) == WV * kX3WideThreads, "staging maps");
    const int s_row = tid / VA, s_col = (tid % VA) * 4;
    f32x4_t ra0[NPA], ra1[NPA], ab0, ab1;
    u32x4_t rb[WV];
    constexpr bool TWO = SRC == 1, TAPS = SRC == 2;
    const int rows_here = M - m0 < kX3BM ? M - m0 : kX3BM;
    const int KA = TWO ? sec.K1 : TAPS ? sec.C : K;
    const int shift = TAPS && !sec.padded ? sec.dil * (sec.wi + 1) * sec.pix : 0;
    const float* a1_base = TAPS ? A - (size_t)shift : A + (size_t)m0 * KA;
    const int a1_bytes = TAPS ? (int)(((size_t)sec.batch * sec.hi_wi * sec.pix + shift) * 4) : (int)((size_t)rows_here * KA * 4);
    const __amdgpu_buffer_rsrc_t a_rsrc = __builtin_amdgcn_make_buffer_rsrc(const_cast<float*>(a1_base), 0, a1_bytes, 0x00020000);
    const int K2 = K - KA;
    auto in_row = [&](int m) -> long long {
        const int b = m / sec.ho_wo, r = m - b * sec.ho_wo, oy = r / sec.wo, ox = r - oy * sec.wo;
        return (long long)b * sec.hi_wi + (long long)oy * sec.stride * sec.wi + (long long)ox * sec.stride;
    };
    long long row0_2 = 0;
    const float* a2_base = nullptr;
    int a2_bytes = 0;
    unsigned pa2[NPA];
    if constexpr (TWO) {
        row0_2 = in_row(__builtin_amdgcn_readfirstlane(m0));
        const int m_end = m0 + rows_here - 1;
        a2_base = sec.A2 + (size_t)row0_2 * K2;
        a2_bytes = (int)((size_t)(in_row(__builtin_amdgcn_readfirstlane(m_end)) - row0_2 + 1) * K2 * 4);
    }
    const __amdgpu_buffer_rsrc_t w_rsrc = __builtin_amdgcn_make_buffer_rsrc(
        const_cast<unsigned short*>(W3 + (size_t)n0 * K), 0, (int)(((size_t)3 * N - n0) * K * 2), 0x00020000);
    unsigned pa[NPA], vmask[NPA];
#pragma unroll
    for (int p = 0; p < NPA; p++) {
        int m = m0 + p * RPP + s_row;
        if (m > M - 1) m = M - 1;
        pa[p] = ((unsigned)(m - m0) * (unsigned)KA + (unsigned)s_col) * 4u;
        vmask[p] = 0u;
        if constexpr (TAPS) {
            const int b = m / sec.ho_wo, r = m - b * sec.ho_wo, oy = r / sec.wo, ox = r - oy * sec.wo;
            pa[p] = (unsigned)((long long)b * sec.hi_wi + (long long)oy * sec.stride * sec.wi + (long long)ox * sec.stride) * (unsigned)sec.pix * 4u
                    + (unsigned)s_col * 4u;
            if (sec.padded) vmask[p] = 0xffffffffu;
            else
                for (int t = 0; t < sec.ntaps; t++) {
                    const int iy = oy * sec.stride - sec.dil + sec.dil * (t / sec.taps_x), ix = ox * sec.stride - sec.dil + sec.dil * (t % sec.taps_x);
                    if (iy >= 0 && iy < sec.hi && ix >= 0 && ix < sec.wi) vmask[p] |= 1u << t;
                }
        }
        if constexpr (TWO) pa2[p] = ((unsigned)(in_row(m) - row0_2) * (unsigned)K2 + (unsigned)s_col) * 4u;
    }
    const unsigned pb = ((unsigned)(tid >> 2) * (unsigned)K + (unsigned)(tid & 3) * 8u) * 2u;
    const int sb_off = x3_lds(tid >> 2, (tid & 3) * 8);
    const int sa_off = x3_lds(s_row, s_col);
    auto fetch_a = [&](f32x4_t (&ra)[NPA], f32x4_t& ab, int k0) {
        if constexpr (TAPS) {
            const int t = k0 / KA, kc = k0 - t * KA;
            const int soff = (int)((((unsigned)(sec.dil * (t / sec.taps_x)) * (unsigned)sec.wi + (unsigned)(sec.dil * (t % sec.taps_x))) * (unsigned)sec.pix + (unsigned)kc) * 4u);
#pragma unroll
            for (int p = 0; p < NPA; p++)
                ra[p] = __builtin_bit_cast(f32x4_t, __builtin_amdgcn_raw_buffer_load_b128(a_rsrc, (vmask[p] >> t) & 1u ? pa[p] : 0xFFFFFFF0u, soff, 0));
        } else if constexpr (TWO) {
            const bool second = k0 >= KA;
            const __amdgpu_buffer_rsrc_t rs = __builtin_amdgcn_make_buffer_rsrc(
                const_cast<float*>(second ? a2_base : a1_base), 0, second ? a2_bytes : a1_bytes, 0x00020000);
            const int ks = (second ? k0 - KA : k0) * 4;
#pragma unroll
            for (int p = 0; p < NPA; p++)
                ra[p] = __builtin_bit_cast(f32x4_t, __builtin_amdgcn_raw_buffer_load_b128(rs, second ? pa2[p] : pa[p], ks, 0));
        } else {
#pragma unroll
            for (int p = 0; p < NPA; p++) ra[p] = __builtin_bit_cast(f32x4_t, __builtin_amdgcn_raw_buffer_load_b128(a_rsrc, pa[p], k0 * 4, 0));
        }
        if (PRO) ab = *reinterpret_cast<const f32x4_t*>(a_bias + k0 + s_col);
    };
    auto fetch_b = [&](int k0) {
#pragma unroll
        for (int t = 0; t < WV; t++)
            rb[t] = __builtin_bit_cast(u32x4_t, __builtin_amdgcn_raw_buffer_load_b128(
                w_rsrc, pb, (int)((((unsigned)(t >> 1) * (unsigned)N + (unsigned)(t & 1) * 128u) * (unsigned)K + (unsigned)k0) * 2u), 0));
    };
    auto store_a = [&](const f32x4_t (&ra)[NPA], const f32x4_t& ab, int stage) {
        unsigned short* sA = reinterpret_cast<unsigned short*>(x3w_smem + stage * kX3WideStageBytes);
#pragma unroll
        for (int p = 0; p < NPA; p++) {
            f32x4_t v = ra[p];
            if (PRO) {
#pragma unroll
                for (int e = 0; e < 4; e++) v[e] = fmaxf(v[e] + ab[e], 0.0f);
            }
            u32x2_t p1, p2, p3;
            split4(v, p1, p2, p3);
            unsigned short* d = sA + sa_off + p * RPP * kX3Pitch;
            *reinterpret_cast<u32x2_t*>(d) = p1;
            *reinterpret_cast<u32x2_t*>(d + LDS_A) = p2;
            *reinterpret_cast<u32x2_t*>(d + 2 * LDS_A) = p3;
        }
    };
    auto store_b = [&](int stage) {
        unsigned short* sB = reinterpret_cast<unsigned short*>(x3w_smem + stage * kX3WideStageBytes) + 3 * LDS_A;
#pragma unroll
        for (int t = 0; t < WV; t++)
            *reinterpret_cast<u32x4_t*>(sB + (t >> 1) * LDS_B + (t & 1) * 128 * kX3Pitch + sb_off) = rb[t];
    };
    constexpr int VEC_PER_ROW = WN / 4, VPL = 32 * VEC_PER_ROW / 64, VRA = 1;
    f32x4_t rres[2][RES ? VPL : 1];
    auto fetch_res = [&](int i, int t_begin, int t_end) {
        if constexpr (RES) {
            const __amdgpu_buffer_rsrc_t r_rsrc = __builtin_amdgcn_make_buffer_rsrc(
                const_cast<float*>(res + (size_t)m0 * N + n0), 0, (int)(((size_t)(rows_here - 1) * N + BN) * 4), 0x00020000);
            const int lrow = wm * 64 + lane / VEC_PER_ROW;
            const unsigned off = ((unsigned)lrow * (unsigned)N + (unsigned)(wn * WN + (lane % VEC_PER_ROW) * 4)) * 4u;
// ... 83 lines not shown
    constexpr std::integral_constant<int, 2> c2{};
    int k0 = 0;
    for (; k0 < K - 2 * kX3BK; k0 += 2 * kX3BK) {
        step(c0, c0, k0, ra1, ab1, ra0, ab0);
        step(c0, c1, k0 + kX3BK, ra0, ab0, ra1, ab1);
    }
    step(c1, c0, k0, ra1, ab1, ra0, ab0);
    step(c2, c1, k0 + kX3BK, ra0, ab0, ra1, ab1);

    float* patch = reinterpret_cast<float*>(x3w_smem) + wave * (32 * WN);
    if constexpr (RES) {
        fetch_res(1, 0, VPL);
        __builtin_amdgcn_sched_barrier(0);
    }
#pragma unroll
    for (int i = 0; i < 2; i++) {
#pragma unroll
        for (int j = 0; j < NT; j++) {
            const int col = j * 32 + (lane & 31);
            const float b = s_bias[wn * WN + col];
#pragma unroll
            for (int r = 0; r < 16; r++) {
                const int row = (r & 3) + 8 * (r >> 2) + 4 * (lane >> 5);
                patch[row * WN + col] = acc[i][j][r] + low[i][j][r] + b;
            }
        }
        __builtin_amdgcn_fence(__ATOMIC_ACQ_REL, "wavefront");
        __builtin_amdgcn_wave_barrier();
#pragma unroll
        for (int t = 0; t < VPL; t++) {
            const int v = t * 64 + lane;
            const int row = v / VEC_PER_ROW, c4 = (v % VEC_PER_ROW) * 4;
            const int m = m0 + wm * 64 + i * 32 + row;
            if (m < M) {
                f32x4_t f = *reinterpret_cast<const f32x4_t*>(patch + row * WN + c4);
                if constexpr (RES) f += rres[i][t];
                if (RELU) {
#pragma unroll
                    for (int e = 0; e < 4; e++) f[e] = fmaxf(f[e], 0.0f);
                }
                *reinterpret_cast<f32x4_t*>(out + (size_t)m * N + n0 + wn * WN + c4) = f;
            }
        }
        __builtin_amdgcn_fence(__ATOMIC_ACQ_REL, "wavefront");
        __builtin_amdgcn_wave_barrier();
        asm volatile("" ::: "memory");
    }
}
#else
#define OPA_X3_HAS_WIDE 0
#endif

enum X3Mode { kX3Plain = 0, kX3Pair = 1, kX3Taps = 2, kX3Unit = 3 };

constexpr bool x3_exists(int BN, bool RES, bool RELU, bool PRO, int TERMS, int SRC, bool UNIT, int UX) {
    if (!UNIT) return UX == 0 && !(SRC != 0 && RES) && !(SRC == 2 && PRO);
    if (SRC != 0 || PRO || (BN == 128 && TERMS == 9)) return false;
    const bool known = UX == 0 || UX == kUxHardswish || UX == kUxResidual || UX == (kUxResidual | kUxHardswish) || UX == kUxActParam;
    return known && !(RELU && (UX & ~kUxResidual) != 0) && !((UX & kUxResidual) != 0 && !RES);
}

static hipError_t launch_x3(X3Mode mode, const float* A, const unsigned short* W3, const float* bias, const float* third, float* out,
                            int M, int N, int K, bool relu, int ux, int terms, const float* a_bias, hipStream_t st, const X3Second& sec) {
    const int bn = mode != kX3Unit ? (N % 128 == 0 ? 128 : 64)
                                   : (N % 128 == 0 && terms == 6 ? 128 : 64);
    const unsigned blocks = (unsigned)((long long)((M + kX3BM - 1) / kX3BM) * (N / bn));
#if OPA_X3_HAS_WIDE
    if (mode != kX3Unit && terms == 6 && N % kX3WideBN == 0) {
        const char* env = std::getenv("OPA_X3_TILE");
        const int forced = env && *env ? std::atoi(env) : 0;
        const unsigned wide_blocks = blocks / 2;
        if (forced == kX3WideBN || (forced != 128 && x3_wide_pays(wide_blocks, third != nullptr, K)))
            return with_value<kX3Plain, kX3Pair, kX3Taps>(mode, [&](auto MODE) {
            return with_flag(third != nullptr, [&](auto RES) {
            return with_flag(relu, [&](auto RELU) {
            return with_flag(a_bias != nullptr, [&](auto PRO) {
                constexpr int SRC = (int)decltype(MODE)::value;
                if constexpr (x3_exists(kX3WideBN, RES, RELU, PRO, 6, SRC, false, 0)) {
                    auto* kernel = &gemm_f32x3_wide_kernel<RES, RELU, PRO, SRC>;
                    hipError_t e = hipFuncSetAttribute(reinterpret_cast<const void*>(kernel), hipFuncAttributeMaxDynamicSharedMemorySize, kX3WideLdsBytes);
                    if (e != hipSuccess) return e;
                    kernel<<<wide_blocks, kX3WideThreads, kX3WideLdsBytes, st>>>(A, W3, bias, third, out, M, N, K, a_bias, sec);
                    return hipGetLastError();
                } else {
                    return hipErrorInvalidValue;
                }
            }); }); }); });
    }
#endif
    return with_value<64, 128>(bn, [&](auto BN) {
    return with_value<6, 9>(terms == 6 ? 6 : 9, [&](auto TERMS) {
    return with_value<kX3Plain, kX3Pair, kX3Taps, kX3Unit>(mode, [&](auto MODE) {
    return with_value<0, kUxHardswish, kUxResidual, kUxResidual | kUxHardswish, kUxActParam>(ux, [&](auto UX) {
    return with_flag(third != nullptr, [&](auto RES) {
    return with_flag(relu, [&](auto RELU) {
    return with_flag(a_bias != nullptr, [&](auto PRO) {
        constexpr bool UNIT = MODE == kX3Unit;
        constexpr int SRC = UNIT ? 0 : (int)MODE;
        if constexpr (x3_exists(BN, RES, RELU, PRO, TERMS, SRC, UNIT, UX)) {
            gemm_f32x3_bias_act_kernel<BN, RES, RELU, PRO, TERMS, SRC, UNIT, UX><<<blocks, 256, 0, st>>>(A, W3, bias, third, out, M, N, K, a_bias, sec);
            return hipGetLastError();
        } else {
            return hipErrorInvalidValue;
        }
    }); }); }); }); }); }); });
}

hipError_t launch_gemm_f32x3_bias_act(const float* A, const unsigned short* W3, const float* bias, const float* res, float* out,
                                      int M, int N, int K, int relu, int terms, hipStream_t st, const float* a_bias) {
    return launch_x3(kX3Plain, A, W3, bias, res, out, M, N, K, relu != 0, 0, terms, a_bias, st, X3Second{});
}

hipError_t launch_gemm2_f32x3_bias_act(const float* A1, int K1, const float* A2, int K2, int batch, int hi, int wi, int stride,
                                       const unsigned short* W3, const float* bias, float* out, int N, int relu, int terms,
                                       hipStream_t st, const float* a_bias) {
    const int ho = (hi - 1) / stride + 1, wo = (wi - 1) / stride + 1;
    X3Second sec;
    sec.A2 = A2; sec.K1 = K1;
    sec.ho_wo = ho * wo; sec.wo = wo; sec.hi_wi = hi * wi; sec.wi = wi; sec.stride = stride;
    return launch_x3(kX3Pair, A1, W3, bias, nullptr, out, batch * ho * wo, N, K1 + K2, relu != 0, 0, terms, a_bias, st, sec);
}

hipError_t launch_gemm_unit_act_f32x3(const float* A, int lda, const unsigned short* W3, const float* bias, const float* partner, int ldp,
                                      const float* residual, int ldr, float* out, int M, int N, int K, int act, int terms, hipStream_t st,
                                      float act_param) {
    if ((partner && residual) || act < 0 || act > 4) return hipErrorInvalidValue;
    X3Second sec;
    sec.lda = lda; sec.ldp = residual ? ldr : ldp; sec.n_real = N; sec.k_real = K;
    if (act >= 3) { sec.act = act; sec.act_param = act_param; }
    const int ux = (act == 2 ? kUxHardswish : 0) | (act >= 3 ? kUxActParam : 0) | (residual ? kUxResidual : 0);
    const int Np = (N + 63) / 64 * 64, Kp = (K + 63) / 64 * 64;
    return launch_x3(kX3Unit, A, W3, bias, residual ? residual : partner, out, M, Np, Kp, act == 1, ux, terms, nullptr, st, sec);
}

hipError_t launch_conv3x3_f32x3(const float* x, int batch, int hi, int wi, int C, int stride, int dilation, const unsigned short* W3,
                                const float* bias, float* out, int N, int relu, int terms, hipStream_t st) {
    const int ho = (hi - 1) / stride + 1, wo = (wi - 1) / stride + 1;
    X3Second sec;
    sec.ho_wo = ho * wo; sec.wo = wo; sec.hi_wi = hi * wi; sec.wi = wi; sec.stride = stride;
    sec.hi = hi; sec.C = C; sec.batch = batch;
    sec.pix = C; sec.taps_x = 3; sec.ntaps = 9; sec.dil = dilation;
    return launch_x3(kX3Taps, x, W3, bias, nullptr, out, batch * ho * wo, N, 9 * C, relu != 0, 0, terms, nullptr, st, sec);
}

hipError_t launch_convrows_f32x3(const float* x, int batch, int hp, int wp, int pix, int ho, int wo, int stride, int ntaps, int tap_floats,
                                 const unsigned short* W3, const float* bias, float* out, int N, int relu, int terms, hipStream_t st) {
    X3Second sec;
    sec.ho_wo = ho * wo; sec.wo = wo; sec.hi_wi = hp * wp; sec.wi = wp; sec.stride = stride;
    sec.hi = hp; sec.C = tap_floats; sec.batch = batch;
    sec.pix = pix; sec.taps_x = 1; sec.ntaps = ntaps; sec.padded = 1;
    return launch_x3(kX3Taps, x, W3, bias, nullptr, out, batch * ho * wo, N, ntaps * tap_floats, relu != 0, 0, terms, nullptr, st, sec);
}

}
```

### openpifpaf_amd/fused.py

```python
import functools
import os
import typing

import torch

from . import _lib
from .native import _ptr, _stream

_DTYPES = {torch.float32: 0, torch.float16: 1, torch.bfloat16: 2}
ACT_NONE, ACT_RELU, ACT_HARDSWISH = 0, 1, 2
ACT_LEAKY_RELU, ACT_RELU6 = 3, 4



def _launch(symbol, *args):
    _lib.check(getattr(_lib.lib(), symbol)(*args, _stream()), symbol)


def _act_code(relu, act):
    return int(bool(relu)) if act is None else int(act)



def _switch(name, default):
    return os.environ.get(name, default) != '0'


X3_TERMS = {'0': 0, '6': 6, '9': 9}.get(os.environ.get('OPA_GEMM3', '6'), 6)
FORCE_PICK = os.environ.get('OPA_GEMM3_PICK') or None
X3_PAIR = _switch('OPA_GEMM3_PAIR', '1')
X3_CONV3 = _switch('OPA_GEMM3_3X3', '1')
X3_HEAD = _switch('OPA_GEMM3_HEAD', '1')
X3_STEM = _switch('OPA_GEMM3_STEM', '1')
X3_UNIT = _switch('OPA_GEMM3_UNIT', '1')
GCONV = _switch('OPA_GCONV', '0')
MBV3 = _switch('OPA_MBV3', '0')
FIRE = _switch('OPA_FIRE', '0')
FIRE_TERMS = 9
MBV2 = _switch('OPA_MBV2', '0')
UNIT_LEAKY = _switch('OPA_UNIT_LEAKY', '0')
STEM = _switch('OPA_STEM', '0')
GN = _switch('OPA_GN', '0')
UNIT_BF16 = _switch('OPA_UNIT_BF16', '0')
CONV3_BF16 = _switch('OPA_CONV3_BF16', '0')
STEM7_BF16 = _switch('OPA_STEM7_BF16', '0')
PAIR_BF16 = _switch('OPA_PAIR_BF16', '0')
GCONV_BF16 = _switch('OPA_GCONV_BF16', '0')
F16 = _switch('OPA_F16', '0')
HEAD16 = _switch('OPA_HEAD16', '0')
_ROUTES16 = {torch.bfloat16: (lambda own: own, '_bf16'), torch.float16: (lambda own: F16, '_f16')}


def _route16(dtype, own=True):
    on, suffix = _ROUTES16.get(dtype, (lambda own: False, None))
    return suffix if on(own) else None



_CHOICE = {}
PINNED_FILE = os.path.join(os.path.dirname(os.path.abspath(__file__)), 'conv1x1_pinned.json')


def load_pinned(path=None):
    import json
    try:
        with open(path or PINNED_FILE) as f:
            table = json.load(f)['table']
    except (OSError, ValueError, KeyError):
        return 0
    for dtype, m, k, n, res, a_bias, choice in table:
        _CHOICE.setdefault((dtype, int(m), int(k), int(n), bool(res), bool(a_bias)), choice)
    return len(table)


def _in_multi_rank_job():
    try:
        import torch.distributed as dist
        return dist.is_available() and dist.is_initialized() and dist.get_world_size() > 1
    except Exception:
        return False


def choices():
    return dict(_CHOICE)


def set_choices(table, *, replace=False):
    if replace:
        _CHOICE.clear()
    _CHOICE.update(table)


def _time_ms(fn, reps=3):
    fn()
    torch.cuda.synchronize()
    best = None
    for _ in range(2):
        start, end = torch.cuda.Event(enable_timing=True), torch.cuda.Event(enable_timing=True)
        start.record()
        for _ in range(reps):
            fn()
        end.record()
        end.synchronize()
        ms = start.elapsed_time(end) / reps
        best = ms if best is None or ms < best else best
    return best


def _decide(key, default, timed, may_time=True):
    choice = _CHOICE.get(key)
    if choice is None:
        if not may_time or torch.cuda.is_current_stream_capturing() or _in_multi_rank_job():
            choice = default
        else:
            times = timed()
            choice = min(times, key=times.get)
        _CHOICE[key] = choice
    return choice


def pick(kind, m, k, n, flag_a, flag_b, run_x3, run_other, written=None, timing=True):
    if FORCE_PICK in ('x3', 'conv'):
        return run_x3() if FORCE_PICK == 'x3' else run_other()

    def timed():
        saved = written.clone() if written is not None else None
        times = {'x3': _time_ms(run_x3), 'conv': _time_ms(run_other)}
        if saved is not None:
            written.copy_(saved)
        return times
    key = ('torch.float32/' + kind, int(m), int(k), int(n), bool(flag_a), bool(flag_b))
    choice = _decide(key, 'x3' if m >= 16384 else 'conv', timed, may_time=timing)
    return run_x3() if choice == 'x3' else run_other()



def _nhwc_rows(x):
    if x.dim() == 4 and x.is_contiguous(memory_format=torch.channels_last):
        return x.shape[0] * x.shape[2] * x.shape[3], x.shape[1]
    if x.dim() == 2 and x.is_contiguous():
        return x.shape[0], x.shape[1]
    return None


def _pixel_stride(x):
    if x.dim() != 4 or x.stride(1) != 1:
        return None
    B, C, H, W = x.shape
    ps = x.stride(3) if W > 1 else (x.stride(2) if H > 1 else C)
    if ps < C or (H > 1 and x.stride(2) != W * ps) or (B > 1 and x.stride(0) != H * W * ps):
        return None
    return ps


def _out_hw(x, stride=1):
    return (x.shape[2] - 1) // stride + 1, (x.shape[3] - 1) // stride + 1


def out_pixels(x, stride=1):
    ho, wo = _out_hw(x, stride)
    return x.shape[0] * ho * wo


def _empty_nhwc(x, channels, hw=None, dtype=None):
    h, w = hw or x.shape[2:]
    return torch.empty((x.shape[0], channels, h, w), dtype=dtype or x.dtype, device=x.device, memory_format=torch.channels_last)



def derived(module, name, sources, make):
    key = tuple(None if t is None else (t.data_ptr(), t._version, str(t.device), t.dtype) for t in sources)
    cached = getattr(module, name, None)
    if cached is None or cached[0] != key:
        cached = (key, make(), [t.untyped_storage() for t in sources if t is not None])
        setattr(module, name, cached)
    return cached[1]


def split_weight(weight2d):
    w = weight2d.detach().to(torch.float32).contiguous()

    def top(x):
        return (x.view(torch.int32) & -65536).view(torch.float32)
    w1 = top(w)
    r1 = w - w1
    w2 = top(r1)
    w3 = r1 - w2
    out = torch.stack((w1, w2, w3)).to(torch.bfloat16)
    return out.contiguous()


def split_weight_3x3(weight):
    n, c = weight.shape[0], weight.shape[1]
    return split_weight(weight.detach().permute(0, 2, 3, 1).reshape(n, 9 * c))


def _split_weight_of(conv, w2d):
    return derived(conv, '_opa_w3', (conv.weight,), lambda: split_weight(w2d))


def _split_weight_3x3_of(conv):
    return derived(conv, '_opa_w3_3x3', (conv.weight,), lambda: split_weight_3x3(conv.weight))
# ... 394 lines not shown
    dt = x.dtype
    if not (_route16(dt, CONV3_BF16) and x.is_cuda and x.dim() == 4 and not torch.is_autocast_enabled()):
        return False
    if torch.is_grad_enabled() and (x.requires_grad or conv.weight.requires_grad or (bias is not None and bias.requires_grad)
                                    or (residual is not None and residual.requires_grad)):
        return False
    s, d = conv.stride[0], conv.dilation[0]
    if not (conv.kernel_size == (3, 3) and conv.groups == 1 and conv.bias is None and conv.stride == (s, s) and s in (1, 2)
            and conv.dilation == (d, d) and d in (1, 2, 4) and (d == 1 or s == 1) and conv.padding == (d, d)
            and conv.in_channels % 64 == 0 and conv.out_channels % 64 == 0 and x.shape[1] == conv.in_channels
            and conv.weight.dtype == dt and conv.weight.device == x.device
            and x.is_contiguous(memory_format=torch.channels_last) and x.data_ptr() % 16 == 0 and 0 < x.numel() < 2 ** 31
            and out_pixels(x, s) * conv.out_channels < 2 ** 31):
        return False
    if bias is not None and not (bias.dtype in (dt, torch.float32) and bias.device == x.device and bias.dim() == 1
                                 and bias.numel() == conv.out_channels):
        return False
    if residual is not None and not (residual.dtype == dt and residual.device == x.device and residual.is_cuda
                                     and tuple(residual.shape) == (x.shape[0], conv.out_channels) + _out_hw(x, s)
                                     and residual.is_contiguous(memory_format=torch.channels_last) and residual.data_ptr() % 16 == 0):
        return False
    return _lib.available()


def conv3x3_bias_act_bf16(conv, x, bias, residual=None, relu=True):
    w9, b32 = conv3x3_bf16_weight_of(conv, bias)
    B, C, H, W = x.shape
    s = conv.stride[0]
    out = _empty_nhwc(x, conv.out_channels, _out_hw(x, s))
    _launch('opa_conv3x3_act' + _ROUTES16[x.dtype][1], _ptr(x), _ptr(w9), _ptr(b32), _ptr(residual), _ptr(out), B, H, W, C, conv.out_channels, s,
            conv.dilation[0], int(bool(relu)))
    return out


GCONV_BF16_WIDTHS = (4, 8, 16, 32, 64)
GCONV_BF16_DECLINED = frozenset()


def gconv3x3_bf16_weight_of(conv, bias=None):
    def make():
        w = conv.weight.detach()
        c, cg = w.shape[0], w.shape[1]
        packed = w.new_zeros((c, 9, 64 // cg, cg))
        rows = torch.arange(c, device=w.device)
        packed[rows, :, (rows % 64) // cg, :] = w.permute(0, 2, 3, 1).reshape(c, 9, cg)
        return (packed.reshape(c, 9, 64), None if bias is None else bias.detach().to(torch.float32).contiguous())
    return derived(conv, '_opa_w_gconv_bf16', (conv.weight, bias), make)


def gconv3x3_bf16_supported(conv, x, bias):
    if not (GCONV_BF16 and x.is_cuda and x.dtype == torch.bfloat16 and x.dim() == 4 and not torch.is_autocast_enabled()):
        return False
    if torch.is_grad_enabled() and (x.requires_grad or conv.weight.requires_grad or (bias is not None and bias.requires_grad)):
        return False
    s, d, c = conv.stride[0], conv.dilation[0], conv.in_channels
    if not (conv.kernel_size == (3, 3) and conv.groups > 1 and conv.bias is None and conv.stride == (s, s) and s in (1, 2)
            and conv.dilation == (d, d) and d in (1, 2, 4) and (d == 1 or s == 1) and conv.padding == (d, d)
            and c == conv.out_channels and c % 64 == 0 and c % conv.groups == 0 and c // conv.groups in GCONV_BF16_WIDTHS
            and x.shape[1] == c and conv.weight.dtype == torch.bfloat16 and conv.weight.device == x.device
            and x.is_contiguous(memory_format=torch.channels_last) and x.data_ptr() % 16 == 0 and 0 < x.numel() < 2 ** 31
            and out_pixels(x, s) * c < 2 ** 31):
        return False
    if bias is not None and not (bias.dtype in (torch.bfloat16, torch.float32) and bias.device == x.device and bias.dim() == 1
                                 and bias.numel() == c):
        return False
    return _lib.available() and (c, c // conv.groups, s) not in GCONV_BF16_DECLINED


def gconv3x3_bias_act_bf16(conv, x, bias, relu=True):
    w9, b32 = gconv3x3_bf16_weight_of(conv, bias)
    B, C, H, W = x.shape
    s = conv.stride[0]
    out = _empty_nhwc(x, C, _out_hw(x, s))
    _launch('opa_gconv3x3_act_bf16', _ptr(x), _ptr(w9), _ptr(b32), _ptr(out), B, H, W, C, C // conv.groups, s, conv.dilation[0],
            int(bool(relu)))
    return out


def stem_x3_supported(conv, x, bias):
    return (X3_STEM and X3_TERMS in (6, 9) and x.is_cuda and x.dtype == torch.float32 and x.dim() == 4 and conv.kernel_size == (7, 7)
            and conv.stride == (2, 2) and conv.padding == (3, 3) and conv.dilation == (1, 1) and conv.groups == 1 and conv.bias is None
            and conv.in_channels == 3 and x.shape[1] == 3 and conv.out_channels % 64 == 0
            and bias.dtype == torch.float32 and bias.is_contiguous() and bias.data_ptr() % 16 == 0
            and x.shape[0] * (x.shape[2] + 7) * (x.shape[3] + 7) * 16 < 2 ** 31)


def stem7x7_bias_act_x3(conv, x, bias, relu=True):
    w3 = _stem_weight_of(conv)
    B, _, H, W = x.shape
    xp = torch.nn.functional.pad(x.permute(0, 2, 3, 1), (0, 1, 3, 4, 3, 4)).contiguous()
    ho, wo = _out_hw(x, 2)
    out = _empty_nhwc(x, conv.out_channels, (ho, wo), torch.float32)
    _launch('opa_conv_rows_f32x3', _ptr(xp), _ptr(w3), _ptr(bias), _ptr(out), B, H + 7, W + 7, 4, ho, wo, 2, 8, 32,
            conv.out_channels, int(bool(relu)), int(X3_TERMS))
    return out


STEM7_BF16_K = 192


def stem7x7_bf16_weight_of(conv, bias=None):
    def make():
        w = conv.weight.detach()
        wk = w.new_zeros((w.shape[0], 8, 8, 3))
        wk[:, :7, :7] = w.permute(0, 2, 3, 1)
        return (wk.reshape(w.shape[0], STEM7_BF16_K), None if bias is None else bias.detach().to(torch.float32).contiguous())
    return derived(conv, '_opa_w_stem7_bf16', (conv.weight, bias), make)


def stem7x7_bf16_supported(conv, x, bias):
    if not (STEM7_BF16 and x.is_cuda and x.dtype == torch.bfloat16 and x.dim() == 4 and x.shape[1] == 3
            and not torch.is_autocast_enabled()):
        return False
    if torch.is_grad_enabled() and (x.requires_grad or conv.weight.requires_grad or (bias is not None and bias.requires_grad)):
        return False
    s = conv.stride[0]
    if not (isinstance(conv, torch.nn.Conv2d) and conv.kernel_size == (7, 7) and conv.padding == (3, 3) and conv.dilation == (1, 1)
            and conv.groups == 1 and conv.bias is None and conv.padding_mode == 'zeros' and conv.stride == (s, s) and s in (1, 2)
            and conv.in_channels == 3 and conv.out_channels % 64 == 0
            and conv.weight.dtype == torch.bfloat16 and conv.weight.device == x.device):
        return False
    if bias is not None and not (bias.dtype in (torch.bfloat16, torch.float32) and bias.device == x.device and bias.dim() == 1
                                 and bias.numel() == conv.out_channels):
        return False
    last = sum((n - 1) * st for n, st in zip(x.shape, x.stride()))
    return (min(x.shape) > 0 and min(x.stride()) > 0 and x.data_ptr() % 2 == 0 and last < 2 ** 31
            and out_pixels(x, s) * conv.out_channels < 2 ** 31 and _lib.available())


def stem7x7_bias_act_bf16(conv, x, bias, relu=True):
    wk, b32 = stem7x7_bf16_weight_of(conv, bias)
    B, _, H, W = x.shape
    s = conv.stride[0]
    out = _empty_nhwc(x, conv.out_channels, _out_hw(x, s))
    _launch('opa_stem7x7_act_bf16', _ptr(x), x.stride(0), x.stride(1), x.stride(2), x.stride(3), _ptr(wk), _ptr(b32), _ptr(out),
            B, H, W, conv.out_channels, s, int(bool(relu)))
    return out


def head_conv_x3_supported(conv, x):
    return (X3_HEAD and X3_TERMS in (6, 9) and x.is_cuda and x.dtype == torch.float32 and x.dim() == 4 and not x.requires_grad
            and x.is_contiguous(memory_format=torch.channels_last) and conv.kernel_size == (1, 1) and conv.stride == (1, 1)
            and conv.padding == (0, 0) and conv.groups == 1 and conv.in_channels % 64 == 0 and x.shape[1] == conv.in_channels
            and conv.weight.dtype == torch.float32 and x.data_ptr() % 16 == 0)


def head_conv_x3(conv, x):
    n = conv.out_channels
    w3, bp = _unit_weight_of(conv)
    out = conv1x1_bias_act_x3(x, w3, bp, None, False, None, X3_TERMS)
    return out[:, :n].contiguous(memory_format=torch.channels_last) if w3.shape[1] != n else out


class UnitMode(typing.NamedTuple):
    dtype: torch.dtype
    align: int
    enabled: typing.Callable
    declines_autocast: bool
    weight: typing.Callable
    cache: str
    launch: typing.Callable
    gemm: str
    table: bool
    head: typing.Callable


def _launch_unit_x3(operands, code, act_param, terms):
    terms = int(X3_TERMS if terms is None else terms)
    if code in (ACT_LEAKY_RELU, ACT_RELU6):
        _launch('opa_gemm_unit_actp_f32x3', *operands, code, float(act_param), terms)
    else:
        _launch('opa_gemm_unit_act_f32x3', *operands, code, terms)


UNIT_MODE_X3 = UnitMode(torch.float32, 8, lambda: X3_UNIT and X3_TERMS in (6, 9), False, split_weight, '_opa_w3_unit', _launch_unit_x3,
                        'conv1x1_unit_x3', True, lambda: X3_HEAD)
UNIT_MODE_BF16 = UnitMode(torch.bfloat16, 4, lambda: UNIT_BF16, True, lambda wp: wp, '_opa_w_unit_bf16',
                          lambda operands, code, act_param, terms: _launch('opa_gemm_unit_actp_bf16', *operands, code, float(act_param)),
                          'conv1x1_unit_bf16', False, lambda: True)
_UNIT_MODES = {mode.dtype: mode for mode in (UNIT_MODE_X3, UNIT_MODE_BF16)}


def unit_mode_of(t):
    return _UNIT_MODES.get(t.dtype)


def _unit_conv_ok(mode, conv):
    return (mode.enabled() and conv.kernel_size == (1, 1) and conv.stride == (1, 1) and conv.padding == (0, 0)
            and conv.dilation == (1, 1) and conv.groups == 1 and conv.in_channels % 2 == 0 and conv.out_channels % 2 == 0
            and conv.weight.dtype == mode.dtype and (conv.bias is None or conv.bias.dtype == mode.dtype))


def _unit_operand_ok(mode, t, channels):
    ps = _pixel_stride(t)
    return (t.dtype == mode.dtype and not t.requires_grad and ps is not None and t.shape[1] == channels
            and ps % 2 == 0 and ps <= 2 ** 21 and t.data_ptr() % mode.align == 0)


def unit_conv_supported(conv, x, partner=None, residual=None, mode=None, head=False):
    mode = mode or unit_mode_of(x)
    if not (mode is not None and x.is_cuda and conv.weight.device == x.device and (not head or mode.head())
            and not (mode.declines_autocast and torch.is_autocast_enabled()) and _unit_conv_ok(mode, conv)
            and _unit_operand_ok(mode, x, conv.in_channels) and 0 < x.shape[0] * x.shape[2] * x.shape[3] < 2 ** 31):
        return False
    if partner is not None and residual is not None:
        return False
    for third in (partner, residual):
        if third is not None and not (third.device == x.device and _unit_operand_ok(mode, third, conv.out_channels)
                                      and (third.shape[0], third.shape[2], third.shape[3]) == (x.shape[0], x.shape[2], x.shape[3])):
            return False
    return True


def _conv1x1_unit(mode, conv, x, relu=True, partner=None, residual=None, act=None, terms=None, act_param=0.0):
    w, bp = _unit_operands_of(mode, conv)
    n = conv.out_channels
    out = _empty_nhwc(x, n if partner is None else 2 * n, dtype=mode.dtype)
    operands = (_ptr(x), _pixel_stride(x), _ptr(w), _ptr(bp),
                _ptr(partner), _pixel_stride(partner) if partner is not None else 0,
                _ptr(residual), _pixel_stride(residual) if residual is not None else 0,
                _ptr(out), out_pixels(x), n, x.shape[1])
    mode.launch(operands, _act_code(relu, act), act_param, terms)
    return out


def conv1x1_unit(conv, x, **kwargs):
    return globals()[unit_mode_of(x).gemm](conv, x, **kwargs)


def pick_unit(x, m, k, n, has_partner, run_unit, run_other):
    if unit_mode_of(x).table:
        return pick('unit', m, k, n, has_partner, False, run_unit, run_other, timing=False)
    return run_unit()


_unit_weight_of = functools.partial(_unit_operands_of, UNIT_MODE_X3)
_unit_weight_bf16_of = functools.partial(_unit_operands_of, UNIT_MODE_BF16)
unit_conv_x3_supported = functools.partial(unit_conv_supported, mode=UNIT_MODE_X3)
unit_conv_bf16_supported = functools.partial(unit_conv_supported, mode=UNIT_MODE_BF16)
conv1x1_unit_x3 = functools.partial(_conv1x1_unit, UNIT_MODE_X3)


def conv1x1_unit_bf16(conv, x, relu=True, partner=None, residual=None, act=None, act_param=0.0):
    return _conv1x1_unit(UNIT_MODE_BF16, conv, x, relu, partner, residual, act, None, act_param)



def _fragment_order(w3):
    n, k = w3.shape[1], w3.shape[2]
    return w3.reshape(3, n // 32, 32, k // 16, 2, 8).permute(0, 1, 3, 4, 2, 5).reshape(3, n * k)


def fire_weight_of(expand1x1, expand3x3):
    def make():
        w1, w3 = expand1x1.weight.detach(), expand3x3.weight.detach()
        blocks = (_fragment_order(split_weight(w1.reshape(w1.shape[0], w1.shape[1]))), _fragment_order(split_weight_3x3(w3)))
        biases = [torch.zeros(c.out_channels, dtype=torch.float32, device=w1.device) if c.bias is None else c.bias.detach().float()
                  for c in (expand1x1, expand3x3)]
        return torch.cat(blocks, dim=1).contiguous(), torch.cat(biases).contiguous()
    return derived(expand1x1, '_opa_w3_fire', (expand1x1.weight, expand1x1.bias, expand3x3.weight, expand3x3.bias), make)


def _fire_convs_ok(expand1x1, expand3x3):
    def ok(conv, k):
        return (conv.kernel_size == (k, k) and conv.stride == (1, 1) and conv.padding == (k // 2, k // 2) and conv.dilation == (1, 1)
                and conv.groups == 1 and conv.padding_mode == 'zeros' and conv.weight.dtype == torch.float32
                and (conv.bias is None or (conv.bias.dtype == torch.float32 and conv.bias.device == conv.weight.device)))
    s = expand1x1.in_channels
    return (ok(expand1x1, 1) and ok(expand3x3, 3) and expand3x3.in_channels == s and s % 16 == 0 and s <= 64
            and expand1x1.out_channels % 64 == 0 and expand3x3.out_channels % 64 == 0
            and expand1x1.weight.device == expand3x3.weight.device)


def fire_expand_supported(expand1x1, expand3x3, h, terms=None):
    if not (h.is_cuda and h.dim() == 4 and h.dtype == torch.float32 and not torch.is_autocast_enabled() and _fire_convs_ok(expand1x1, expand3x3)):
        return False
    if torch.is_grad_enabled() and (h.requires_grad or any(p.requires_grad for c in (expand1x1, expand3x3) for p in c.parameters())):
        return False
    return (h.shape[1] == expand1x1.in_channels and h.is_contiguous(memory_format=torch.channels_last) and h.data_ptr() % 16 == 0
            and fire_expand_shape_supported(expand1x1, expand3x3, h.device, h.shape[0] * h.shape[2] * h.shape[3], terms))


def fire_expand_shape_supported(expand1x1, expand3x3, device, pixels, terms=None):
    n = expand1x1.out_channels + expand3x3.out_channels
    return ((FIRE_TERMS if terms is None else terms) in (6, 9)
            and _fire_convs_ok(expand1x1, expand3x3) and expand1x1.weight.device == device and 0 < pixels
            and pixels * n * 4 < 2 ** 31 and _lib.available())


def fire_expand_bias_relu(expand1x1, expand3x3, h, terms=None):
    w3, bias = fire_weight_of(expand1x1, expand3x3)
    B, S, H, W = h.shape
    out = _empty_nhwc(h, expand1x1.out_channels + expand3x3.out_channels, dtype=torch.float32)
    _launch('opa_fire_expand_f32x3', _ptr(h), _ptr(w3), _ptr(bias), _ptr(out), B, H, W, S, expand1x1.out_channels,
            expand3x3.out_channels, int(FIRE_TERMS if terms is None else terms))
    return out



GCONV_WIDTHS = (4, 8, 16, 32, 64)


def gconv3x3_supported(conv, x, bias):
    if not (GCONV and x.is_cuda and x.dtype == torch.float32 and x.dim() == 4 and not torch.is_autocast_enabled()):
        return False
    if torch.is_grad_enabled() and (x.requires_grad or conv.weight.requires_grad or (bias is not None and bias.requires_grad)):
# ... 229 lines not shown
```

### openpifpaf_amd/network.py

```python
import math

import torch
from torch import nn

from . import fused, headmeta, winograd


def _take_biases(block, conv_names):
    for i, name in enumerate(conv_names, 1):
        conv = getattr(block, name)
        bias = conv.bias.detach().clone() if conv.bias is not None else torch.zeros(conv.out_channels)
        if i == len(conv_names) and block.downsample is not None:
            dconv = block.downsample[0]
            if dconv.bias is not None:
                bias = bias + dconv.bias.detach().to(bias.device)
                dconv.bias = None
        conv.bias = None
        block.register_buffer('fb%d' % i, bias)


_CONV3_ROUTES = (
    ('wino', lambda c, x, b, r, u: winograd.takes(c, x, u),
     lambda c, x, b, r, u, bare: winograd.run(c, x, u, bias=None if bare else b, relu=not bare), False, None),
    ('x3', lambda c, x, b, r, u: fused.conv3x3_x3_supported(c, x, b),
# ... 815 lines not shown
        self.expand1x1_activation = nn.ReLU(inplace=True)
        self.expand3x3 = nn.Conv2d(squeeze_planes, expand3x3_planes, 3, padding=1)
        self.expand3x3_activation = nn.ReLU(inplace=True)

    fused = False

    def enable_fused_(self):
        self.fused = True

    def _route_supported(self, x):
        if not (fused.FIRE and x.is_cuda and x.dim() == 4 and x.dtype == torch.float32 and not torch.is_autocast_enabled()
                and x.is_contiguous(memory_format=torch.channels_last)):
            return False
        if torch.is_grad_enabled() and (x.requires_grad or any(p.requires_grad for p in self.parameters())):
            return False
        return (self.squeeze.bias is not None and fused.FIRE_TERMS in (6, 9) and fused.unit_conv_x3_supported(self.squeeze, x)
                and fused.fire_expand_shape_supported(self.expand1x1, self.expand3x3, x.device, x.shape[0] * x.shape[2] * x.shape[3]))

    def _forward_unit(self, x):
        h = fused.conv1x1_unit_x3(self.squeeze, x, relu=True, terms=fused.FIRE_TERMS)
        return fused.fire_expand_bias_relu(self.expand1x1, self.expand3x3, h)

    def forward(self, x):
        if self.fused and self._route_supported(x):
            return self._forward_unit(x)
        x = self.squeeze_activation(self.squeeze(x))
        return torch.cat([self.expand1x1_activation(self.expand1x1(x)), self.expand3x3_activation(self.expand3x3(x))], 1)


class SqueezeNet(BaseNetwork):
    CONFIGS = {'squeezenet': ((64, 16, 64, 64), (128, 16, 64, 64), None, (128, 32, 128, 128), (256, 32, 128, 128), None,
                              (256, 48, 192, 192), (384, 48, 192, 192), (384, 64, 256, 256), (512, 64, 256, 256))}

    def __init__(self, name='squeezenet'):
        super().__init__(name, stride=16, out_features=512)

        def pool():
            return nn.MaxPool2d(kernel_size=3, stride=2, padding=1, ceil_mode=True)
        layers = [nn.Conv2d(3, 64, 3, stride=2, padding=1), nn.ReLU(inplace=True), pool()]
        layers += [pool() if cfg is None else _Fire(*cfg) for cfg in self.CONFIGS[name]]
        self.backbone = nn.Sequential(*layers)
        for m in self.modules():
            if isinstance(m, nn.Conv2d):
                nn.init.kaiming_uniform_(m.weight)
                nn.init.zeros_(m.bias)

    @staticmethod
    def _pool_route_supported(pool, x):
        return (isinstance(pool, nn.MaxPool2d) and pool.kernel_size == 3 and pool.stride == 2 and pool.padding == 1 and pool.dilation == 1
                and pool.ceil_mode and not pool.return_indices and fused.maxpool3x3_supported(x))

    def forward(self, x):
        modules = list(self.backbone)
        i = 0
        y = _stem_route(self, modules[0], modules[1], x)
        if y is not None:
            x, i = y, 2
        pools = self.fused and fused.FIRE and x.is_cuda and not torch.is_autocast_enabled()
        if not pools and i == 0:
            return self.backbone(x)
        while i < len(modules):
            m = modules[i]
            if pools and isinstance(m, nn.ReLU) and i + 1 < len(modules) and self._pool_route_supported(modules[i + 1], x):
                x = fused.maxpool3x3_bias_act_(x, relu=True, ceil_mode=True)
                i += 2
                continue
            x = fused.maxpool3x3_bias_act_(x, ceil_mode=True) if pools and self._pool_route_supported(m, x) else m(x)
            i += 1
        return x


BASE_FACTORIES = {
    **{n: (lambda n=n: Resnet(n)) for n in Resnet.CONFIGS},
    **{n: (lambda n=n: ShuffleNetV2K(n)) for n in ShuffleNetV2K.CONFIGS},
    **{n: (lambda n=n: ShuffleNetV2(n)) for n in ShuffleNetV2.CONFIGS},
    **{n: (lambda n=n: MobileNetV2(n)) for n in MobileNetV2.CONFIGS},
    **{n: (lambda n=n: MobileNetV3(n)) for n in MobileNetV3.CONFIGS},
    **{n: (lambda n=n: SqueezeNet(n)) for n in SqueezeNet.CONFIGS},
}


class CompositeField4(nn.Module):

    def __init__(self, meta: headmeta.Base, in_features):
        super().__init__()
        self.meta = meta
        self.n_components = 1 + meta.n_confidences + meta.n_vectors * 2 + meta.n_scales
        self.conv = nn.Conv2d(in_features, meta.n_fields * self.n_components * (meta.upsample_stride ** 2), 1)
        self.upsample_op = nn.PixelShuffle(meta.upsample_stride) if meta.upsample_stride > 1 else None

    fused_epilogue = True

    def forward(self, x):
        if not self.training and self.fused_epilogue and fused.head_conv_fields16_supported(self.conv, x, self.meta, self.training):
            return fused.head_conv_fields16(self.conv, x, self.meta)
        if not self.training and fused.head_conv_x3_supported(self.conv, x):
            conv, x0 = self.conv, x
            x = fused.pick('head', fused.out_pixels(x0), conv.in_channels, conv.out_channels, False, False,
                           lambda: fused.head_conv_x3(conv, x0), lambda: conv(x0))
        elif not self.training and self.conv.in_channels % 64 != 0 and fused.unit_conv_supported(self.conv, x, head=True):
            conv, x0 = self.conv, x
            x = fused.pick_unit(x0, fused.out_pixels(x0), conv.in_channels, conv.out_channels, False,
                                lambda: fused.conv1x1_unit(conv, x0, relu=False), lambda: conv(x0))
        else:
            x = self.conv(x)
        if self.fused_epilogue and fused.head_epilogue_supported(x, self.meta, self.training):
            return fused.head_epilogue(x, self.meta)
        if self.upsample_op is not None:
            x = self.upsample_op(x)
            us = self.meta.upsample_stride
            low_cut = (us - 1) // 2
            high_cut = math.ceil((us - 1) / 2.0)
            x = x[:, :, low_cut:x.shape[2] - high_cut, low_cut:x.shape[3] - high_cut]
        B, _, H, W = x.shape
        m = self.meta
        x = x.float().reshape(B, m.n_fields, self.n_components, H, W).contiguous()
        if not self.training:
            nc = m.n_confidences
            x[:, :, 1:1 + nc].sigmoid_()
            ii = torch.arange(W, device=x.device, dtype=x.dtype)
            jj = torch.arange(H, device=x.device, dtype=x.dtype).unsqueeze(1)
            for i, do_offset in enumerate(m.vector_offsets):
                if do_offset:
                    x[:, :, 1 + nc + 2 * i] += ii
                    x[:, :, 1 + nc + 2 * i + 1] += jj
            first_scale = 1 + nc + m.n_vectors * 2
            x[:, :, first_scale:first_scale + m.n_scales] = nn.functional.softplus(
                x[:, :, first_scale:first_scale + m.n_scales])
        return x


class Shell(nn.Module):

    def __init__(self, base_net, head_nets):
        super().__init__()
        self.base_net = base_net
        self.head_nets = None
        self.set_head_nets(head_nets)

    @property
    def head_metas(self):
        return [hn.meta for hn in self.head_nets] if self.head_nets is not None else None

    def set_head_nets(self, head_nets):
        if not isinstance(head_nets, nn.ModuleList):
            head_nets = nn.ModuleList(head_nets)
        for i, hn in enumerate(head_nets):
            hn.meta.head_index = i
            hn.meta.base_stride = self.base_net.stride
        self.head_nets = head_nets

    def forward(self, image_batch):
        x = self.base_net(image_batch)
        return tuple(hn(x) for hn in self.head_nets)


def factory(base_name='resnet50', head_metas=None, *, seed=0):
    if head_metas is None:
        head_metas = headmeta.cocokp_metas()
    gen_state = torch.random.get_rng_state()
    torch.manual_seed(seed)
    try:
        base = BASE_FACTORIES[base_name]()
        heads = [CompositeField4(m, base.out_features) for m in head_metas]
        net = Shell(base, heads)
    finally:
        torch.random.set_rng_state(gen_state)
    return net.eval()


def _folds(norm):
    return isinstance(norm, nn.BatchNorm2d) or (isinstance(norm, nn.InstanceNorm2d) and norm.affine and norm.track_running_stats
                                                and not norm.training)


def _fold(conv, bn):
    with torch.no_grad():
        scale = bn.weight / torch.sqrt(bn.running_var + bn.eps)
        conv.weight.mul_(scale.reshape(-1, 1, 1, 1))
        bias = bn.bias - bn.running_mean * scale
        if conv.bias is not None:
            bias = bias + conv.bias * scale
        conv.bias = nn.Parameter(bias)


def fuse_conv_bn_(model):
    assert not model.training
    for module in model.modules():
        if isinstance(module, nn.Sequential):
            prev_name, prev = None, None
            for name, child in list(module.named_children()):
                if _folds(child) and isinstance(prev, nn.Conv2d):
                    _fold(prev, child)
                    setattr(module, name, nn.Identity())
                prev_name, prev = name, child
        for i in (1, 2, 3):
            conv, bn = getattr(module, 'conv%d' % i, None), getattr(module, 'bn%d' % i, None)
            if isinstance(conv, nn.Conv2d) and isinstance(bn, nn.BatchNorm2d):
                _fold(conv, bn)
                setattr(module, 'bn%d' % i, nn.Identity())
    return model


def optimize_for_inference_(model):
    fuse_conv_bn_(model)
    for m in model.modules():
        if isinstance(m, (_Bottleneck, _BasicBlock, _InvertedResidualK, _InvertedResidual, _Fire, BaseNetwork)):
            m.enable_fused_()
    return model
```

Before: 675.2 images/s.

## Fuse all head 1x1 convs and field epilogues into one f32x3 GEMM launch

Adds a multi-head kernel that runs the CIF and CAF head 1x1 convolutions as one f32x3 split-bf16 GEMM over concatenated, tile-padded weights. Each N-tile looks up its head and writes field-layout outputs directly through the head16 plan epilogue. This aims to cut the separate per-head GEMM and epilogue launches and the intermediate conv output round trip through memory. It adds a per-tile head lookup, padding waste in the weight tiles, and a size heuristic that decides when the fused path is taken.

```diff
diff --git a/include/openpifpaf_amd.h b/include/openpifpaf_amd.h
--- a/include/openpifpaf_amd.h
+++ b/include/openpifpaf_amd.h
@@ -334,6 +334,16 @@
                              int32_t n_fields, int32_t n_components, int32_t upsample, int32_t n_confidences,
                              int32_t n_vectors, uint32_t vector_offset_mask, int32_t n_scales, void* stream);
 
+typedef struct opa_head_fields {
+    float* out_dev;
+    int32_t n_fields, n_components, n_confidences, n_vectors;
+    uint32_t vector_offset_mask;
+    int32_t n_scales;
+} opa_head_fields;
+int opa_heads_conv_fields_f32x3(const float* x_dev, const void* w3_dev, const float* bias_dev, const opa_head_fields* heads_host,
+                                int32_t n_heads, int32_t batch, int32_t hc, int32_t wc, int32_t k, int32_t upsample, int32_t terms,
+                                void* stream);
+
 typedef struct opa_pre_image {
     int64_t src_offset;
     int64_t mid_offset;
diff --git a/openpifpaf_amd/_lib.py b/openpifpaf_amd/_lib.py
--- a/openpifpaf_amd/_lib.py
+++ b/openpifpaf_amd/_lib.py
@@ -78,6 +78,11 @@
 class PreImage(ctypes.Structure):
     _fields_ = [('src_offset', ctypes.c_int64), ('mid_offset', ctypes.c_int64)] + [(n, ctypes.c_int32) for n in (
         'h0', 'w0', 'th', 'tw', 'top', 'left', 'x_table', 'x_ksize', 'y_table', 'y_ksize')]
+
+
+class HeadFields(ctypes.Structure):
+    _fields_ = [('out_dev', ctypes.c_void_p)] + [(n, ctypes.c_int32) for n in ('n_fields', 'n_components', 'n_confidences', 'n_vectors')] + [
+        ('vector_offset_mask', ctypes.c_uint32), ('n_scales', ctypes.c_int32)]
 
 
 class Shape(ctypes.Structure):
@@ -179,6 +184,7 @@
     'opa_head_epilogue': (ctypes.c_int, [_vp, _i32, _i32, _i32, _i32, _i32, _i32, _i32, _i32, _i32, ctypes.c_uint32, _i32, _vp, _vp]),
     'opa_head_conv_fields_bf16': (ctypes.c_int, [_vp, _vp, _vp, _vp] + [_i32] * 9 + [ctypes.c_uint32, _i32, _vp]),
     'opa_head_conv_fields_f16': (ctypes.c_int, [_vp, _vp, _vp, _vp] + [_i32] * 9 + [ctypes.c_uint32, _i32, _vp]),
+    'opa_heads_conv_fields_f32x3': (ctypes.c_int, [_vp, _vp, _vp, _vp] + [_i32] * 7 + [_vp]),
     'opa_pre_image_bytes': (_sz, []),
     'opa_preprocess_workspace_bytes': (_sz, [_P(PreImage), _i32, _i32]),
     'opa_preprocess_u8': (ctypes.c_int, [_P(PreImage), _vp, _i32, _vp, _sz, _vp, _sz, _vp, _sz, _vp, _vp, _i32, _i32, _i32, _i32,
diff --git a/openpifpaf_amd/csrc/capi_trunk.hip b/openpifpaf_amd/csrc/capi_trunk.hip
--- a/openpifpaf_amd/csrc/capi_trunk.hip
+++ b/openpifpaf_amd/csrc/capi_trunk.hip
@@ -1,4 +1,5 @@
 #include "capi_internal.hpp"
+#include "heads_x3_plan.hpp"
 
 #include <algorithm>
 #include <cmath>
@@ -665,6 +666,52 @@
                              int32_t n_vectors, uint32_t vector_offset_mask, int32_t n_scales, void* stream) {
     return head_conv_fields_16("opa_head_conv_fields_f16", 1, x_dev, w_dev, bias_dev, out_dev, batch, hc, wc, k, n_fields, n_components, upsample,
                                n_confidences, n_vectors, vector_offset_mask, n_scales, stream);
+}
+
+int opa_heads_conv_fields_f32x3(const float* x_dev, const void* w3_dev, const float* bias_dev, const opa_head_fields* heads_host,
+                                int32_t n_heads, int32_t batch, int32_t hc, int32_t wc, int32_t k, int32_t upsample, int32_t terms,
+                                void* stream) {
+    const Entry E("opa_heads_conv_fields_f32x3", stream);
+    if (!x_dev || !w3_dev || !bias_dev || !heads_host) return E.refuse("x_dev, w3_dev, bias_dev and heads_host must not be NULL");
+    if (n_heads < 1 || n_heads > kHeadsX3Max) return E.refuse("n_heads must be 1 .. 4");
+    for (int32_t i = 0; i < n_heads; i++)
+        if (!heads_host[i].out_dev) return E.refuse("every head's out_dev must not be NULL");
+    bool out_misaligned = false;
+    for (int32_t i = 0; i < n_heads; i++) out_misaligned |= misaligned(3, {heads_host[i].out_dev});
+    if (misaligned(15, {x_dev, w3_dev, bias_dev}) || out_misaligned)
+        return E.refuse("x_dev / w3_dev / bias_dev must be 16-B, every head's out_dev 4-B aligned");
+    if (batch < 0) return E.refuse("negative batch");
+    if (hc <= 0 || wc <= 0 || k <= 0) return E.refuse("hc, wc and k must be positive");
+    if (k % 64 != 0) return E.refuse("k must be a multiple of 64");
+    if (upsample != 1 && upsample != 2) return E.refuse("upsample must be 1 or 2");
+    if (bad_terms(terms)) return E.refuse("terms must be 6 or 9");
+    for (int32_t i = 0; i < n_heads; i++)
+        if (heads_host[i].n_fields <= 0 || heads_host[i].n_components <= 0) return E.refuse("every head's n_fields and n_components must be positive");
+    for (int32_t i = 0; i < n_heads; i++) {
+        const opa_head_fields& h = heads_host[i];
+        if (h.n_confidences < 0 || h.n_vectors < 0 || h.n_scales < 0 || 1ll + h.n_confidences + 2ll * h.n_vectors + h.n_scales != h.n_components)
+            return E.refuse("every head's n_components must be 1 + n_confidences + 2 * n_vectors + n_scales, no count negative");
+    }
+    if ((double)batch * hc * wc >= 2147483648.0) return E.refuse("batch * hc * wc must stay below 2^31");
+    double tiles = 0.0;
+    for (int32_t i = 0; i < n_heads; i++)
+        tiles += std::ceil((double)heads_host[i].n_fields * heads_host[i].n_components * upsample * upsample / kHeadsX3BN);
+    if (tiles * kHeadsX3BN * k * 6.0 >= 4294967296.0) return E.refuse("the weight's three planes must be smaller than 4 GB (32-bit offsets)");
+    const double ho = (double)hc * upsample - (upsample - 1), wo = (double)wc * upsample - (upsample - 1);
+    for (int32_t i = 0; i < n_heads; i++)
+        if ((double)batch * heads_host[i].n_fields * heads_host[i].n_components * ho * wo >= 2147483648.0)
+            return E.refuse("every head's out must hold fewer than 2^31 elements (32-bit offsets)");
+    if (batch == 0) return OPA_OK;
+    HeadsX3 d{n_heads, batch, hc, wc, upsample, {}};
+    int tile0 = 0;
+    for (int32_t i = 0; i < n_heads; i++) {
+        const opa_head_fields& h = heads_host[i];
+        d.head[i] = HeadsX3Head{tile0, h.n_fields, h.n_components, h.n_confidences, h.n_vectors, h.vector_offset_mask, h.n_scales, h.out_dev};
+        tile0 += heads_x3_tiles(heads_x3_n(d, d.head[i]));
+    }
+    if (heads_x3_workgroups(d) > 0x7fffffffll) return E.refuse("too many tiles for grid.x");
+    return E.launched(launch_heads_f32x3(x_dev, (const unsigned short*)w3_dev, bias_dev, d, k, terms, E.st), "heads_conv_fields_f32x3",
+                      "heads_f32x3_kernel");
 }
 
 size_t opa_pre_image_bytes(void) { return sizeof(opa_pre_image); }
diff --git a/openpifpaf_amd/csrc/common.hpp b/openpifpaf_amd/csrc/common.hpp
--- a/openpifpaf_amd/csrc/common.hpp
+++ b/openpifpaf_amd/csrc/common.hpp
@@ -295,6 +295,9 @@
 long long head16_workgroups(int B, int hc, int wc, int n_fields, int n_comp, int us);
 hipError_t launch_head16(const void* x, const void* w, const float* bias, float* out, int B, int hc, int wc, int K, int n_fields,
                          int n_comp, int us, int n_conf, int n_vec, unsigned offset_mask, int n_scales, hipStream_t st, int dtype);
+struct HeadsX3;
+long long heads_x3_workgroups(const HeadsX3& heads);
+hipError_t launch_heads_f32x3(const float* x, const unsigned short* W3, const float* bias, const HeadsX3& heads, int K, int terms, hipStream_t st);
 
 size_t preprocess_h_lds_bytes(int in_cap);
 size_t preprocess_zoom_lds_bytes(int in_cap);
diff --git a/openpifpaf_amd/csrc/gemm_f32x3.hip b/openpifpaf_amd/csrc/gemm_f32x3.hip
--- a/openpifpaf_amd/csrc/gemm_f32x3.hip
+++ b/openpifpaf_amd/csrc/gemm_f32x3.hip
@@ -1,6 +1,8 @@
 #include <cstdlib>
 #include <type_traits>
 #include "common.hpp"
+#include "head_field.hpp"
+#include "heads_x3_plan.hpp"
 #include "split_bf16.hpp"
 
 namespace opa {
@@ -114,313 +116,64 @@
     }
 }
 
+static_assert(4 * 32 * (kHead16WN + 2) * 4 <= 3 * (kX3BM + kHeadsX3BN) * kX3Pitch * 2, "the four patches at their widest pitch fit the staging LDS");
+static_assert(kHeadsX3BM == kX3BM && kHeadsX3BM == kBf16BM, "one M-tile for the kernel and both plans");
+template <int US, int NT>
+__device__ __forceinline__ void x3_heads_epilogue(float* smem_f, const f32x16_t (&acc)[2][NT], const f32x16_t (&low)[2][NT],
+                                                  const float* __restrict__ bias, const HeadsX3& heads, int m0, int n0, int lane, int wave) {
+    constexpr int PITCH = kHead16WN + US;
+    const int wn = wave & 1, tile = n0 / kHeadsX3BN;
+    HeadsX3 d = heads;
+    d.us = US;
+    const HeadsX3Head h = heads_x3_head_of(d, tile);
+    float* __restrict__ fields = h.out;
+    Head16Row rows[2];
+    heads_x3_plan_rows(d, h, m0, threadIdx.x, rows);
+    float* patch = smem_f + wave * (32 * PITCH);
+    const int col = lane & 31;
+    auto component = [&](int plane) { return (US == 2 ? __builtin_amdgcn_readfirstlane(plane) : plane) % h.n_comp; };
+#pragma unroll
+    for (int j = 0; j < NT; j++) {
+        const float b = bias[n0 + wn * (NT * 32) + j * 32 + col];
+#pragma unroll
+        for (int i = 0; i < 2; i++) {
+#pragma unroll
+            for (int r = 0; r < 16; r++) {
+                const int row = (r & 3) + 8 * (r >> 2) + 4 * (lane >> 5);
+                patch[row * PITCH + col] = (acc[i][j][r] + low[i][j][r]) + b;
+            }
+            __builtin_amdgcn_fence(__ATOMIC_ACQ_REL, "wavefront");
+            __builtin_amdgcn_wave_barrier();
+            heads_x3_plan_block(d, h, rows[i], tile, j, threadIdx.x, [&](int prow, int pcol, int at, int plane, int y, int x) {
+                fields[at] = head_field(patch[prow * PITCH + pcol], component(plane), x, y, h.n_conf, h.n_vec, h.offset_mask, h.n_scales);
+            });
+            __builtin_amdgcn_fence(__ATOMIC_ACQ_REL, "wavefront");
+            __builtin_amdgcn_wave_barrier();
+            asm volatile("" ::: "memory");
+        }
+    }
+}
+
 template <int BN, bool RES, bool RELU, bool PRO, int TERMS, int SRC, bool UNIT = false, int UX = 0>
 __global__ __launch_bounds__(256, OPA_X3_WGS) void gemm_f32x3_bias_act_kernel(
         const float* __restrict__ A, const unsigned short* __restrict__ W3, const float* __restrict__ bias,
         const float* __restrict__ res, float* __restrict__ out, int M, int N, int K, const float* __restrict__ a_bias,
         const X3Second sec) {
-    constexpr int WN = BN / 2;
-    constexpr int NT = WN / 32;
-    constexpr int LDS_A = kX3BM * kX3Pitch, LDS_B = BN * kX3Pitch;
-#ifndef OPA_X3_PAD_LDS
-#define OPA_X3_PAD_LDS 0
-#endif
-    constexpr int STAGE_BYTES = 3 * (LDS_A + LDS_B) * 2 + OPA_X3_PAD_LDS;
-    constexpr int EPI_BYTES = 4 * 32 * WN * 4;
-    constexpr int SMEM_BYTES = STAGE_BYTES > EPI_BYTES ? STAGE_BYTES : EPI_BYTES;
-    __shared__ __attribute__((aligned(16))) unsigned char smem[SMEM_BYTES + (RES && !UNIT ? BN * 4 : 0)];
-    unsigned short* sA = reinterpret_cast<unsigned short*>(smem);
-    unsigned short* sB = sA + 3 * LDS_A;
-
-    const int tid = threadIdx.x, lane = tid & 63, wave = tid >> 6;
-    const int wm = wave >> 1, wn = wave & 1;
-    const int n_tiles = N / BN;
-    const unsigned nwg = gridDim.x, xcd = blockIdx.x & 7u, in_xcd = blockIdx.x >> 3;
-    const unsigned q = nwg >> 3, r8 = nwg & 7u;
-    const unsigned logical = (xcd < r8 ? xcd * (q + 1) : r8 * (q + 1) + (xcd - r8) * q) + in_xcd;
-    const int m0 = (int)(logical / n_tiles) * kX3BM;
-    const int n0 = (int)(logical % n_tiles) * BN;
-
-    constexpr int NL = OPA_X3_ONE_ACC ? 1 : 2;
-    f32x16_t acc[2][NT], low_[NL][NT];
-    f32x16_t (&low)[2][NT] = OPA_X3_ONE_ACC ? acc : reinterpret_cast<f32x16_t (&)[2][NT]>(low_);
-#pragma unroll
-    for (int i = 0; i < 2; i++)
-#pragma unroll
-        for (int j = 0; j < NT; j++)
-#pragma unroll
-            for (int r = 0; r < 16; r++) { acc[i][j][r] = 0.0f; if (!OPA_X3_ONE_ACC) low[i][j][r] = 0.0f; }
-
-    constexpr int VA = kX3BK / 4;
-    constexpr int RPP = 256 / VA;
-    constexpr int NPA = kX3BM / RPP;
-    constexpr int WQ = kX3BK / 8;
-    const int s_row = tid / VA, s_col = (tid % VA) * 4;
-    constexpr int WTOT = 3 * BN * WQ;
-    constexpr int WV = (WTOT + 255) / 256;
-    f32x4_t ra0[NPA], ra1[NPA];
-    u32x4_t rb[WV];
-    constexpr bool TWO = SRC == 1, TAPS = SRC == 2;
-    const int rows_here = M - m0 < kX3BM ? M - m0 : kX3BM;
-    const int KA = TWO ? sec.K1 : TAPS ? sec.C : UNIT ? sec.lda : K;
-    const int shift = TAPS && !sec.padded ? sec.dil * (sec.wi + 1) * sec.pix : 0;
-    const float* a1_base = TAPS ? A - (size_t)shift : A + (size_t)m0 * KA;
-    const int a1_bytes = TAPS ? (int)(((size_t)sec.batch * sec.hi_wi * sec.pix + shift) * 4)
-                       : UNIT ? (int)(((size_t)(rows_here - 1) * KA + sec.k_real) * 4) : (int)((size_t)rows_here * KA * 4);
-    const __amdgpu_buffer_rsrc_t a_rsrc = __builtin_amdgcn_make_buffer_rsrc(const_cast<float*>(a1_base), 0, a1_bytes, 0x00020000);
-    const int K2 = K - KA;
-    auto in_row = [&](int m) -> long long {
-        const int b = m / sec.ho_wo, r = m - b * sec.ho_wo, oy = r / sec.wo, ox = r - oy * sec.wo;
-        return (long long)b * sec.hi_wi + (long long)oy * sec.stride * sec.wi + (long long)ox * sec.stride;
-    };
-    long long row0_2 = 0;
-    const float* a2_base = nullptr;
-    int a2_bytes = 0;
-    unsigned pa2[NPA];
-    if constexpr (TWO) {
-        row0_2 = in_row(__builtin_amdgcn_readfirstlane(m0));
-        const int m_end = m0 + rows_here - 1;
-        a2_base = sec.A2 + (size_t)row0_2 * K2;
-        a2_bytes = (int)((size_t)(in_row(__builtin_amdgcn_readfirstlane(m_end)) - row0_2 + 1) * K2 * 4);
-    }
-    const __amdgpu_buffer_rsrc_t w_rsrc = __builtin_amdgcn_make_buffer_rsrc(
-        const_cast<unsigned short*>(W3 + (size_t)n0 * K), 0, (int)(((size_t)3 * N - n0) * K * 2), 0x00020000);
-    unsigned pa[NPA], pb[WV];
-    unsigned vmask[NPA];
-    int sb_off[WV];
-#pragma unroll
-    for (int p = 0; p < NPA; p++) {
-        int m = m0 + p * RPP + s_row;
-        if (m > M - 1) m = M - 1;
-        pa[p] = ((unsigned)(m - m0) * (unsigned)KA + (unsigned)s_col) * 4u;
-        vmask[p] = 0u;
-        if constexpr (TAPS) {
-            const int b = m / sec.ho_wo, r = m - b * sec.ho_wo, oy = r / sec.wo, ox = r - oy * sec.wo;
-            pa[p] = (unsigned)((long long)b * sec.hi_wi + (long long)oy * sec.stride * sec.wi + (long long)ox * sec.stride) * (unsigned)sec.pix * 4u
-                    + (unsigned)s_col * 4u;
-            if (sec.padded) vmask[p] = 0xffffffffu;
-            else
-                for (int t = 0; t < sec.ntaps; t++) {
-                    const int iy = oy * sec.stride - sec.dil + sec.dil * (t / sec.taps_x), ix = ox * sec.stride - sec.dil + sec.dil * (t % sec.taps_x);
-                    if (iy >= 0 && iy < sec.hi && ix >= 0 && ix < sec.wi) vmask[p] |= 1u << t;
-                }
-        }
-        if constexpr (TWO) pa2[p] = ((unsigned)(in_row(m) - row0_2) * (unsigned)K2 + (unsigned)s_col) * 4u;
-    }
-#pragma unroll
-    for (int t = 0; t < WV; t++) {
-        const int v = t * 256 + tid < WTOT ? t * 256 + tid : WTOT - 1;
-        const int plane = v / (BN * WQ), rem = v - plane * (BN * WQ), row = rem / WQ, c = (rem % WQ) * 8;
-        pb[t] = (((unsigned)plane * (unsigned)N + (unsigned)row) * (unsigned)K + (unsigned)c) * 2u;
-        sb_off[t] = plane * LDS_B + x3_lds(row, c);
-    }
-    auto fetch_a = [&](f32x4_t (&ra)[NPA], int k0) {
-        if constexpr (TAPS) {
-            const int t = k0 / KA, kc = k0 - t * KA;
-            const int soff = (int)((((unsigned)(sec.dil * (t / sec.taps_x)) * (unsigned)sec.wi + (unsigned)(sec.dil * (t % sec.taps_x))) * (unsigned)sec.pix + (unsigned)kc) * 4u);
-#pragma unroll
-            for (int p = 0; p < NPA; p++)
-                ra[p] = __builtin_bit_cast(f32x4_t, __builtin_amdgcn_raw_buffer_load_b128(a_rsrc, (vmask[p] >> t) & 1u ? pa[p] : 0xFFFFFFF0u, soff, 0));
-        } else if constexpr (TWO) {
-            const bool second = k0 >= KA;
-            const __amdgpu_buffer_rsrc_t rs = __builtin_amdgcn_make_buffer_rsrc(
-                const_cast<float*>(second ? a2_base : a1_base), 0, second ? a2_bytes : a1_bytes, 0x00020000);
-            const int ks = (second ? k0 - KA : k0) * 4;
-#pragma unroll
-            for (int p = 0; p < NPA; p++)
-                ra[p] = __builtin_bit_cast(f32x4_t, __builtin_amdgcn_raw_buffer_load_b128(rs, second ? pa2[p] : pa[p], ks, 0));
-        } else if constexpr (UNIT) {
-#pragma unroll
-            for (int p = 0; p < NPA; p++) {
-                const f32x2_t lo = __builtin_bit_cast(f32x2_t, __builtin_amdgcn_raw_buffer_load_b64(a_rsrc, pa[p], k0 * 4, 0));
-                const f32x2_t hi = __builtin_bit_cast(f32x2_t, __builtin_amdgcn_raw_buffer_load_b64(a_rsrc, pa[p] + 8u, k0 * 4, 0));
-                ra[p] = (f32x4_t){lo[0], lo[1], hi[0], hi[1]};
-            }
-        } else {
-#pragma unroll
-            for (int p = 0; p < NPA; p++) ra[p] = __builtin_bit_cast(f32x4_t, __builtin_amdgcn_raw_buffer_load_b128(a_rsrc, pa[p], k0 * 4, 0));
-        }
-        if (PRO) {
-            const f32x4_t ab = *reinterpret_cast<const f32x4_t*>(a_bias + k0 + s_col);
-#pragma unroll
-            for (int p = 0; p < NPA; p++)
-#pragma unroll
-                for (int e = 0; e < 4; e++) ra[p][e] = fmaxf(ra[p][e] + ab[e], 0.0f);
-        }
-    };
-    auto fetch_b = [&](int k0) {
-#pragma unroll
-        for (int t = 0; t < WV; t++) rb[t] = __builtin_bit_cast(u32x4_t, __builtin_amdgcn_raw_buffer_load_b128(w_rsrc, pb[t], k0 * 2, 0));
-    };
-    auto store = [&](const f32x4_t (&ra)[NPA], int kt) {
-#pragma unroll
-        for (int p = 0; p < NPA; p++) {
-            u32x2_t p1, p2, p3;
-            if (OPA_X3_DIAG == 1) { p1[0] = __float_as_uint(ra[p][0]); p1[1] = __float_as_uint(ra[p][2]); p2 = p1; p3 = p1; }
-            else if constexpr (UNIT) {
-                const bool in0 = kt + s_col < sec.k_real, in1 = kt + s_col + 2 < sec.k_real;
-                const f32x4_t v = {in0 ? ra[p][0] : 0.0f, in0 ? ra[p][1] : 0.0f, in1 ? ra[p][2] : 0.0f, in1 ? ra[p][3] : 0.0f};
-                split4(v, p1, p2, p3);
-            }
-            else split4(ra[p], p1, p2, p3);
-            unsigned short* d = sA + x3_lds(p * RPP + s_row, s_col);
-            *reinterpret_cast<u32x2_t*>(d) = p1;
-            *reinterpret_cast<u32x2_t*>(d + LDS_A) = p2;
-            *reinterpret_cast<u32x2_t*>(d + 2 * LDS_A) = p3;
-        }
-#pragma unroll
-        for (int t = 0; t < WV; t++)
-            if (WTOT % 256 == 0 || t * 256 + tid < WTOT) *reinterpret_cast<u32x4_t*>(sB + sb_off[t]) = rb[t];
-    };
-    constexpr int VEC_PER_ROW = WN / 4;
-    constexpr int VPL = 32 * VEC_PER_ROW / 64;
-    constexpr int VRA = 1;
-    constexpr bool TAIL_RES = RES && !UNIT;
-    f32x4_t rres[2][TAIL_RES ? VPL : 1];
-    auto fetch_res = [&](int i, int t_begin, int t_end) {
-        if constexpr (TAIL_RES) {
-            const __amdgpu_buffer_rsrc_t r_rsrc = __builtin_amdgcn_make_buffer_rsrc(
-                const_cast<float*>(res + (size_t)m0 * N + n0), 0, (int)(((size_t)(rows_here - 1) * N + BN) * 4), 0x00020000);
-            const int lrow = wm * 64 + lane / VEC_PER_ROW;
-            const unsigned off = ((unsigned)lrow * (unsigned)N + (unsigned)(wn * WN + (lane % VEC_PER_ROW) * 4)) * 4u;
-#pragma unroll
-            for (int t = t_begin; t < t_end; t++) {
-                const int urow = i * 32 + t * (64 / VEC_PER_ROW);
-                rres[i][t] = __builtin_bit_cast(f32x4_t, __builtin_amdgcn_raw_buffer_load_b128(
-                    r_rsrc, lrow < rows_here - urow ? off : 0xFFFFFFF0u, urow * N * 4, 0));
-            }
-        }
-    };
-    int frag_a[kX3BK / 16], frag_b[kX3BK / 16];
-    if constexpr (TAIL_RES) {
-#pragma unroll
-        for (int h = 0; h < kX3BK / 16; h++) {
-            frag_a[h] = 2 * x3_lds(wm * 64 + (lane & 31), h * 16 + (lane >> 5) * 8);
-            frag_b[h] = 2 * x3_lds(wn * WN + (lane & 31), h * 16 + (lane >> 5) * 8);
-            asm volatile("" : "+v"(frag_a[h]), "+v"(frag_b[h]));
-        }
-    }
-    auto step = [&](auto tail, int k0, f32x4_t (&cur)[NPA], f32x4_t (&nxt)[NPA]) {
-        constexpr int TAIL = decltype(tail)::value;
-        const bool more = TAIL == 1 || (TAIL == 0 && k0 + kX3BK < K);
-        const int k_last = K - kX3BK;
-        if constexpr (TAIL == 0) {
-            fetch_b(k0 + kX3BK < k_last ? k0 + kX3BK : k_last);
-            fetch_a(nxt, k0 + 2 * kX3BK < k_last ? k0 + 2 * kX3BK : k_last);
-        } else if constexpr (TAIL == 1) {
-            fetch_b(k_last);
-            fetch_res(0, 0, VRA);
-        } else {
-            fetch_res(0, VRA, VPL);
-        }
-        __builtin_amdgcn_sched_barrier(0);
-#pragma unroll
-        for (int kk = 0; kk < kX3BK; kk += 16) {
-            bf16x8_t fa[3][2], fb[3][NT];
-            const int kh = OPA_X3_DIAG == 4 ? 0 : kk / 16;
-            const int kof = kh * 16 + (lane >> 5) * 8;
-#pragma unroll
-            for (int pl = 0; pl < 3; pl++) {
-#pragma unroll
-                for (int i = 0; i < 2; i++)
-                    fa[pl][i] = *reinterpret_cast<const bf16x8_t*>(TAIL_RES ? reinterpret_cast<const unsigned short*>(smem + frag_a[kh]) + (pl * LDS_A + i * 32 * kX3Pitch)
-                                                                       : sA + pl * LDS_A + x3_lds(wm * 64 + i * 32 + (lane & 31), kof));
-#pragma unroll
-                for (int j = 0; j < NT; j++)
-                    fb[pl][j] = *reinterpret_cast<const bf16x8_t*>(TAIL_RES ? reinterpret_cast<const unsigned short*>(smem + frag_b[kh]) + (3 * LDS_A + pl * LDS_B + j * 32 * kX3Pitch)
-                                                                       : sB + pl * LDS_B + x3_lds(wn * WN + j * 32 + (lane & 31), kof));
-            }
-#pragma unroll
-            for (int i = 0; i < 2; i++)
-#pragma unroll
-                for (int j = 0; j < NT; j++)
-                    acc[i][j] = __builtin_amdgcn_mfma_f32_32x32x16_bf16(fa[0][i], fb[0][j], acc[i][j], 0, 0, 0);
-#pragma unroll
-            for (int s = 4; s >= 1; s--) {
-                if ((TERMS == 6 && s > 2) || OPA_X3_DIAG == 3) continue;
-#pragma unroll
-                for (int pa_ = 0; pa_ < 3; pa_++) {
-                    const int pb_ = s - pa_;
-                    if (pb_ < 0 || pb_ > 2) continue;
-#pragma unroll
-                    for (int i = 0; i < 2; i++)
-#pragma unroll
-                        for (int j = 0; j < NT; j++)
-                            low[i][j] = __builtin_amdgcn_mfma_f32_32x32x16_bf16(fa[pa_][i], fb[pb_][j], low[i][j], 0, 0, 0);
-                }
-            }
-        }
-        __syncthreads();
-        if (more && (OPA_X3_DIAG != 2 || cur[0][0] == 12345.678f)) store(cur, k0 + kX3BK);
-        __syncthreads();
-    };
-    fetch_b(0);
-    fetch_a(ra0, 0);
-    if constexpr (TAIL_RES) {
-        if (tid < BN) reinterpret_cast<float*>(smem + SMEM_BYTES)[tid] = bias[n0 + tid];
-    }
-    store(ra0, 0);
-    __syncthreads();
-    fetch_a(ra1, kX3BK);
-    constexpr std::integral_constant<int, 0> any_step{};
-    if constexpr (TAIL_RES) {
-        int k0 = 0;
-        for (; k0 < K - 2 * kX3BK; k0 += 2 * kX3BK) {
-            step(any_step, k0, ra1, ra0);
-            step(any_step, k0 + kX3BK, ra0, ra1);
-        }
-        step(std::integral_constant<int, 1>{}, k0, ra1, ra0);
-        step(std::integral_constant<int, 2>{}, k0 + kX3BK, ra0, ra1);
-    } else {
-        for (int k0 = 0; k0 < K; k0 += 2 * kX3BK) {
-            step(any_step, k0, ra1, ra0);
-            step(any_step, k0 + kX3BK, ra0, ra1);
-        }
-    }
-    if constexpr (UNIT) {
-        x3_unit_epilogue<BN, RES, RELU, UX>(reinterpret_cast<float*>(smem), acc, low, bias, res, out, M, m0, n0, lane, wave, sec.ldp, sec.n_real,
-                                            sec.act, sec.act_param);
-        return;
-    }
-
-    float* patch = reinterpret_cast<float*>(smem) + wave * (32 * WN);
-    if constexpr (TAIL_RES) {
-        fetch_res(1, 0, VPL);
-        __builtin_amdgcn_sched_barrier(0);
-    }
-#pragma unroll
-    for (int i = 0; i < 2; i++) {
-#pragma unroll
-        for (int j = 0; j < NT; j++) {
-            const int col = j * 32 + (lane & 31);
-            const float b = TAIL_RES ? reinterpret_cast<const float*>(smem + SMEM_BYTES)[wn * WN + col] : bias[n0 + wn * WN + col];
-#pragma unroll
-            for (int r = 0; r < 16; r++) {
-                const int row = (r & 3) + 8 * (r >> 2) + 4 * (lane >> 5);
-                patch[row * WN + col] = (OPA_X3_ONE_ACC ? acc[i][j][r] : acc[i][j][r] + low[i][j][r]) + b;
-            }
-        }
-        __builtin_amdgcn_fence(__ATOMIC_ACQ_REL, "wavefront");
-        __builtin_amdgcn_wave_barrier();
-#pragma unroll
-        for (int t = 0; t < VPL; t++) {
-            const int v = t * 64 + lane;
-            const int row = v / VEC_PER_ROW, c4 = (v % VEC_PER_ROW) * 4;
-            const int m = m0 + wm * 64 + i * 32 + row;
-            if (m < M) {
-                f32x4_t f = *reinterpret_cast<const f32x4_t*>(patch + row * WN + c4);
-                if constexpr (TAIL_RES) f += rres[i][t];
-                if (RELU) {
-#pragma unroll
-                    for (int e = 0; e < 4; e++) f[e] = fmaxf(f[e], 0.0f);
-                }
-                *reinterpret_cast<f32x4_t*>(out + (size_t)m * N + n0 + wn * WN + c4) = f;
-            }
-        }
-        __builtin_amdgcn_fence(__ATOMIC_ACQ_REL, "wavefront");
-        __builtin_amdgcn_wave_barrier();
-        asm volatile("" ::: "memory");
-    }
+    constexpr int US = 0;
+    constexpr const HeadsX3* heads = nullptr;
+#include "gemm_f32x3_tile.hpp"
+}
+
+template <int TERMS, int US>
+__global__ __launch_bounds__(256, OPA_X3_WGS) void heads_f32x3_kernel(
+        const float* __restrict__ A, const unsigned short* __restrict__ W3, const float* __restrict__ bias, int M, int N, int K,
+        const HeadsX3 heads_by_value) {
+    constexpr int BN = kHeadsX3BN, SRC = 0, UX = 0;
+    constexpr bool RES = false, RELU = false, PRO = false, UNIT = false;
+    const float* const res = nullptr; float* const out = nullptr; const float* const a_bias = nullptr;
+    const X3Second sec{};
+    const HeadsX3* const heads = &heads_by_value;
+#include "gemm_f32x3_tile.hpp"
 }
 
 #if OPA_X3_BK == 32 && OPA_X3_SWIZZLE && !OPA_X3_ONE_ACC && OPA_X3_DIAG == 0
@@ -810,4 +563,21 @@
     return launch_x3(kX3Taps, x, W3, bias, nullptr, out, batch * ho * wo, N, ntaps * tap_floats, relu != 0, 0, terms, nullptr, st, sec);
 }
 
-}
+long long heads_x3_workgroups(const HeadsX3& heads) {
+    const HeadsX3Head& last = heads.head[heads.n_heads - 1];
+    const long long M = (long long)heads.batch * heads.hc * heads.wc;
+    return (M + kX3BM - 1) / kX3BM * (last.tile0 + heads_x3_tiles(heads_x3_n(heads, last)));
+}
+
+hipError_t launch_heads_f32x3(const float* x, const unsigned short* W3, const float* bias, const HeadsX3& heads, int K, int terms, hipStream_t st) {
+    const HeadsX3Head& last = heads.head[heads.n_heads - 1];
+    const int M = heads.batch * heads.hc * heads.wc, Np = (last.tile0 + heads_x3_tiles(heads_x3_n(heads, last))) * kHeadsX3BN;
+    const unsigned blocks = (unsigned)heads_x3_workgroups(heads);
+    return with_value<6, 9>(terms, [&](auto TERMS) {
+    return with_value<1, 2>(heads.us, [&](auto US) {
+        heads_f32x3_kernel<TERMS, US><<<blocks, kHeadsX3Threads, 0, st>>>(x, W3, bias, M, Np, K, heads);
+        return hipGetLastError();
+    }); });
+}
+
+}
diff --git a/openpifpaf_amd/csrc/gemm_f32x3_tile.hpp b/openpifpaf_amd/csrc/gemm_f32x3_tile.hpp
--- /dev/null
+++ b/openpifpaf_amd/csrc/gemm_f32x3_tile.hpp
@@ -0,0 +1,306 @@
+    constexpr int WN = BN / 2;
+    constexpr int NT = WN / 32;
+    constexpr int LDS_A = kX3BM * kX3Pitch, LDS_B = BN * kX3Pitch;
+#ifndef OPA_X3_PAD_LDS
+#define OPA_X3_PAD_LDS 0
+#endif
+    constexpr int STAGE_BYTES = 3 * (LDS_A + LDS_B) * 2 + OPA_X3_PAD_LDS;
+    constexpr int EPI_BYTES = 4 * 32 * WN * 4;
+    constexpr int SMEM_BYTES = STAGE_BYTES > EPI_BYTES ? STAGE_BYTES : EPI_BYTES;
+    __shared__ __attribute__((aligned(16))) unsigned char smem[SMEM_BYTES + (RES && !UNIT ? BN * 4 : 0)];
+    unsigned short* sA = reinterpret_cast<unsigned short*>(smem);
+    unsigned short* sB = sA + 3 * LDS_A;
+
+    const int tid = threadIdx.x, lane = tid & 63, wave = tid >> 6;
+    const int wm = wave >> 1, wn = wave & 1;
+    const int n_tiles = N / BN;
+    const unsigned nwg = gridDim.x, xcd = blockIdx.x & 7u, in_xcd = blockIdx.x >> 3;
+    const unsigned q = nwg >> 3, r8 = nwg & 7u;
+    const unsigned logical = (xcd < r8 ? xcd * (q + 1) : r8 * (q + 1) + (xcd - r8) * q) + in_xcd;
+    const int m0 = (int)(logical / n_tiles) * kX3BM;
+    const int n0 = (int)(logical % n_tiles) * BN;
+
+    constexpr int NL = OPA_X3_ONE_ACC ? 1 : 2;
+    f32x16_t acc[2][NT], low_[NL][NT];
+    f32x16_t (&low)[2][NT] = OPA_X3_ONE_ACC ? acc : reinterpret_cast<f32x16_t (&)[2][NT]>(low_);
+#pragma unroll
+    for (int i = 0; i < 2; i++)
+#pragma unroll
+        for (int j = 0; j < NT; j++)
+#pragma unroll
+            for (int r = 0; r < 16; r++) { acc[i][j][r] = 0.0f; if (!OPA_X3_ONE_ACC) low[i][j][r] = 0.0f; }
+
+    constexpr int VA = kX3BK / 4;
+    constexpr int RPP = 256 / VA;
+    constexpr int NPA = kX3BM / RPP;
+    constexpr int WQ = kX3BK / 8;
+    const int s_row = tid / VA, s_col = (tid % VA) * 4;
+    constexpr int WTOT = 3 * BN * WQ;
+    constexpr int WV = (WTOT + 255) / 256;
+    f32x4_t ra0[NPA], ra1[NPA];
+    u32x4_t rb[WV];
+    constexpr bool TWO = SRC == 1, TAPS = SRC == 2;
+    const int rows_here = M - m0 < kX3BM ? M - m0 : kX3BM;
+    const int KA = TWO ? sec.K1 : TAPS ? sec.C : UNIT ? sec.lda : K;
+    const int shift = TAPS && !sec.padded ? sec.dil * (sec.wi + 1) * sec.pix : 0;
+    const float* a1_base = TAPS ? A - (size_t)shift : A + (size_t)m0 * KA;
+    const int a1_bytes = TAPS ? (int)(((size_t)sec.batch * sec.hi_wi * sec.pix + shift) * 4)
+                       : UNIT ? (int)(((size_t)(rows_here - 1) * KA + sec.k_real) * 4) : (int)((size_t)rows_here * KA * 4);
+    const __amdgpu_buffer_rsrc_t a_rsrc = __builtin_amdgcn_make_buffer_rsrc(const_cast<float*>(a1_base), 0, a1_bytes, 0x00020000);
+    const int K2 = K - KA;
+    auto in_row = [&](int m) -> long long {
+        const int b = m / sec.ho_wo, r = m - b * sec.ho_wo, oy = r / sec.wo, ox = r - oy * sec.wo;
+        return (long long)b * sec.hi_wi + (long long)oy * sec.stride * sec.wi + (long long)ox * sec.stride;
+    };
+    long long row0_2 = 0;
+    const float* a2_base = nullptr;
+    int a2_bytes = 0;
+    unsigned pa2[NPA];
+    if constexpr (TWO) {
+        row0_2 = in_row(__builtin_amdgcn_readfirstlane(m0));
+        const int m_end = m0 + rows_here - 1;
+        a2_base = sec.A2 + (size_t)row0_2 * K2;
+        a2_bytes = (int)((size_t)(in_row(__builtin_amdgcn_readfirstlane(m_end)) - row0_2 + 1) * K2 * 4);
+    }
+    const __amdgpu_buffer_rsrc_t w_rsrc = __builtin_amdgcn_make_buffer_rsrc(
+        const_cast<unsigned short*>(W3 + (size_t)n0 * K), 0, (int)(((size_t)3 * N - n0) * K * 2), 0x00020000);
+    unsigned pa[NPA], pb[WV];
+    unsigned vmask[NPA];
+    int sb_off[WV];
+#pragma unroll
+    for (int p = 0; p < NPA; p++) {
+        int m = m0 + p * RPP + s_row;
+        if (m > M - 1) m = M - 1;
+        pa[p] = ((unsigned)(m - m0) * (unsigned)KA + (unsigned)s_col) * 4u;
+        vmask[p] = 0u;
+        if constexpr (TAPS) {
+            const int b = m / sec.ho_wo, r = m - b * sec.ho_wo, oy = r / sec.wo, ox = r - oy * sec.wo;
+            pa[p] = (unsigned)((long long)b * sec.hi_wi + (long long)oy * sec.stride * sec.wi + (long long)ox * sec.stride) * (unsigned)sec.pix * 4u
+                    + (unsigned)s_col * 4u;
+            if (sec.padded) vmask[p] = 0xffffffffu;
+            else
+                for (int t = 0; t < sec.ntaps; t++) {
+                    const int iy = oy * sec.stride - sec.dil + sec.dil * (t / sec.taps_x), ix = ox * sec.stride - sec.dil + sec.dil * (t % sec.taps_x);
+                    if (iy >= 0 && iy < sec.hi && ix >= 0 && ix < sec.wi) vmask[p] |= 1u << t;
+                }
+        }
+        if constexpr (TWO) pa2[p] = ((unsigned)(in_row(m) - row0_2) * (unsigned)K2 + (unsigned)s_col) * 4u;
+    }
+#pragma unroll
+    for (int t = 0; t < WV; t++) {
+        const int v = t * 256 + tid < WTOT ? t * 256 + tid : WTOT - 1;
+        const int plane = v / (BN * WQ), rem = v - plane * (BN * WQ), row = rem / WQ, c = (rem % WQ) * 8;
+        pb[t] = (((unsigned)plane * (unsigned)N + (unsigned)row) * (unsigned)K + (unsigned)c) * 2u;
+        sb_off[t] = plane * LDS_B + x3_lds(row, c);
+    }
+    auto fetch_a = [&](f32x4_t (&ra)[NPA], int k0) {
+        if constexpr (TAPS) {
+            const int t = k0 / KA, kc = k0 - t * KA;
+            const int soff = (int)((((unsigned)(sec.dil * (t / sec.taps_x)) * (unsigned)sec.wi + (unsigned)(sec.dil * (t % sec.taps_x))) * (unsigned)sec.pix + (unsigned)kc) * 4u);
+#pragma unroll
+            for (int p = 0; p < NPA; p++)
+                ra[p] = __builtin_bit_cast(f32x4_t, __builtin_amdgcn_raw_buffer_load_b128(a_rsrc, (vmask[p] >> t) & 1u ? pa[p] : 0xFFFFFFF0u, soff, 0));
+        } else if constexpr (TWO) {
+            const bool second = k0 >= KA;
+            const __amdgpu_buffer_rsrc_t rs = __builtin_amdgcn_make_buffer_rsrc(
+                const_cast<float*>(second ? a2_base : a1_base), 0, second ? a2_bytes : a1_bytes, 0x00020000);
+            const int ks = (second ? k0 - KA : k0) * 4;
+#pragma unroll
+            for (int p = 0; p < NPA; p++)
+                ra[p] = __builtin_bit_cast(f32x4_t, __builtin_amdgcn_raw_buffer_load_b128(rs, second ? pa2[p] : pa[p], ks, 0));
+        } else if constexpr (UNIT) {
+#pragma unroll
+            for (int p = 0; p < NPA; p++) {
+                const f32x2_t lo = __builtin_bit_cast(f32x2_t, __builtin_amdgcn_raw_buffer_load_b64(a_rsrc, pa[p], k0 * 4, 0));
+                const f32x2_t hi = __builtin_bit_cast(f32x2_t, __builtin_amdgcn_raw_buffer_load_b64(a_rsrc, pa[p] + 8u, k0 * 4, 0));
+                ra[p] = (f32x4_t){lo[0], lo[1], hi[0], hi[1]};
+            }
+        } else {
+#pragma unroll
+            for (int p = 0; p < NPA; p++) ra[p] = __builtin_bit_cast(f32x4_t, __builtin_amdgcn_raw_buffer_load_b128(a_rsrc, pa[p], k0 * 4, 0));
+        }
+        if (PRO) {
+            const f32x4_t ab = *reinterpret_cast<const f32x4_t*>(a_bias + k0 + s_col);
+#pragma unroll
+            for (int p = 0; p < NPA; p++)
+#pragma unroll
+                for (int e = 0; e < 4; e++) ra[p][e] = fmaxf(ra[p][e] + ab[e], 0.0f);
+        }
+    };
+    auto fetch_b = [&](int k0) {
+#pragma unroll
+        for (int t = 0; t < WV; t++) rb[t] = __builtin_bit_cast(u32x4_t, __builtin_amdgcn_raw_buffer_load_b128(w_rsrc, pb[t], k0 * 2, 0));
+    };
+    auto store = [&](const f32x4_t (&ra)[NPA], int kt) {
+#pragma unroll
+        for (int p = 0; p < NPA; p++) {
+            u32x2_t p1, p2, p3;
+            if (OPA_X3_DIAG == 1) { p1[0] = __float_as_uint(ra[p][0]); p1[1] = __float_as_uint(ra[p][2]); p2 = p1; p3 = p1; }
+            else if constexpr (UNIT) {
+                const bool in0 = kt + s_col < sec.k_real, in1 = kt + s_col + 2 < sec.k_real;
+                const f32x4_t v = {in0 ? ra[p][0] : 0.0f, in0 ? ra[p][1] : 0.0f, in1 ? ra[p][2] : 0.0f, in1 ? ra[p][3] : 0.0f};
+                split4(v, p1, p2, p3);
+            }
+            else split4(ra[p], p1, p2, p3);
+            unsigned short* d = sA + x3_lds(p * RPP + s_row, s_col);
+            *reinterpret_cast<u32x2_t*>(d) = p1;
+            *reinterpret_cast<u32x2_t*>(d + LDS_A) = p2;
+            *reinterpret_cast<u32x2_t*>(d + 2 * LDS_A) = p3;
+        }
+#pragma unroll
+        for (int t = 0; t < WV; t++)
+            if (WTOT % 256 == 0 || t * 256 + tid < WTOT) *reinterpret_cast<u32x4_t*>(sB + sb_off[t]) = rb[t];
+    };
+    constexpr int VEC_PER_ROW = WN / 4;
+    constexpr int VPL = 32 * VEC_PER_ROW / 64;
+    constexpr int VRA = 1;
+    constexpr bool TAIL_RES = RES && !UNIT;
+    f32x4_t rres[2][TAIL_RES ? VPL : 1];
+    auto fetch_res = [&](int i, int t_begin, int t_end) {
+        if constexpr (TAIL_RES) {
+            const __amdgpu_buffer_rsrc_t r_rsrc = __builtin_amdgcn_make_buffer_rsrc(
+                const_cast<float*>(res + (size_t)m0 * N + n0), 0, (int)(((size_t)(rows_here - 1) * N + BN) * 4), 0x00020000);
+            const int lrow = wm * 64 + lane / VEC_PER_ROW;
+            const unsigned off = ((unsigned)lrow * (unsigned)N + (unsigned)(wn * WN + (lane % VEC_PER_ROW) * 4)) * 4u;
+#pragma unroll
+            for (int t = t_begin; t < t_end; t++) {
+                const int urow = i * 32 + t * (64 / VEC_PER_ROW);
+                rres[i][t] = __builtin_bit_cast(f32x4_t, __builtin_amdgcn_raw_buffer_load_b128(
+                    r_rsrc, lrow < rows_here - urow ? off : 0xFFFFFFF0u, urow * N * 4, 0));
+            }
+        }
+    };
+    int frag_a[kX3BK / 16], frag_b[kX3BK / 16];
+    if constexpr (TAIL_RES) {
+#pragma unroll
+        for (int h = 0; h < kX3BK / 16; h++) {
+            frag_a[h] = 2 * x3_lds(wm * 64 + (lane & 31), h * 16 + (lane >> 5) * 8);
+            frag_b[h] = 2 * x3_lds(wn * WN + (lane & 31), h * 16 + (lane >> 5) * 8);
+            asm volatile("" : "+v"(frag_a[h]), "+v"(frag_b[h]));
+        }
+    }
+    auto step = [&](auto tail, int k0, f32x4_t (&cur)[NPA], f32x4_t (&nxt)[NPA]) {
+        constexpr int TAIL = decltype(tail)::value;
+        const bool more = TAIL == 1 || (TAIL == 0 && k0 + kX3BK < K);
+        const int k_last = K - kX3BK;
+        if constexpr (TAIL == 0) {
+            fetch_b(k0 + kX3BK < k_last ? k0 + kX3BK : k_last);
+            fetch_a(nxt, k0 + 2 * kX3BK < k_last ? k0 + 2 * kX3BK : k_last);
+        } else if constexpr (TAIL == 1) {
+            fetch_b(k_last);
+            fetch_res(0, 0, VRA);
+        } else {
+            fetch_res(0, VRA, VPL);
+        }
+        __builtin_amdgcn_sched_barrier(0);
+#pragma unroll
+        for (int kk = 0; kk < kX3BK; kk += 16) {
+            bf16x8_t fa[3][2], fb[3][NT];
+            const int kh = OPA_X3_DIAG == 4 ? 0 : kk / 16;
+            const int kof = kh * 16 + (lane >> 5) * 8;
+#pragma unroll
+            for (int pl = 0; pl < 3; pl++) {
+#pragma unroll
+                for (int i = 0; i < 2; i++)
+                    fa[pl][i] = *reinterpret_cast<const bf16x8_t*>(TAIL_RES ? reinterpret_cast<const unsigned short*>(smem + frag_a[kh]) + (pl * LDS_A + i * 32 * kX3Pitch)
+                                                                       : sA + pl * LDS_A + x3_lds(wm * 64 + i * 32 + (lane & 31), kof));
+#pragma unroll
+                for (int j = 0; j < NT; j++)
+                    fb[pl][j] = *reinterpret_cast<const bf16x8_t*>(TAIL_RES ? reinterpret_cast<const unsigned short*>(smem + frag_b[kh]) + (3 * LDS_A + pl * LDS_B + j * 32 * kX3Pitch)
+                                                                       : sB + pl * LDS_B + x3_lds(wn * WN + j * 32 + (lane & 31), kof));
+            }
+#pragma unroll
+            for (int i = 0; i < 2; i++)
+#pragma unroll
+                for (int j = 0; j < NT; j++)
+                    acc[i][j] = __builtin_amdgcn_mfma_f32_32x32x16_bf16(fa[0][i], fb[0][j], acc[i][j], 0, 0, 0);
+#pragma unroll
+            for (int s = 4; s >= 1; s--) {
+                if ((TERMS == 6 && s > 2) || OPA_X3_DIAG == 3) continue;
+#pragma unroll
+                for (int pa_ = 0; pa_ < 3; pa_++) {
+                    const int pb_ = s - pa_;
+                    if (pb_ < 0 || pb_ > 2) continue;
+#pragma unroll
+                    for (int i = 0; i < 2; i++)
+#pragma unroll
+                        for (int j = 0; j < NT; j++)
+                            low[i][j] = __builtin_amdgcn_mfma_f32_32x32x16_bf16(fa[pa_][i], fb[pb_][j], low[i][j], 0, 0, 0);
+                }
+            }
+        }
+        __syncthreads();
+        if (more && (OPA_X3_DIAG != 2 || cur[0][0] == 12345.678f)) store(cur, k0 + kX3BK);
+        __syncthreads();
+    };
+    fetch_b(0);
+    fetch_a(ra0, 0);
+    if constexpr (TAIL_RES) {
+        if (tid < BN) reinterpret_cast<float*>(smem + SMEM_BYTES)[tid] = bias[n0 + tid];
+    }
+    store(ra0, 0);
+    __syncthreads();
+    fetch_a(ra1, kX3BK);
+    constexpr std::integral_constant<int, 0> any_step{};
+    if constexpr (TAIL_RES) {
+        int k0 = 0;
+        for (; k0 < K - 2 * kX3BK; k0 += 2 * kX3BK) {
+            step(any_step, k0, ra1, ra0);
+            step(any_step, k0 + kX3BK, ra0, ra1);
+        }
+        step(std::integral_constant<int, 1>{}, k0, ra1, ra0);
+        step(std::integral_constant<int, 2>{}, k0 + kX3BK, ra0, ra1);
+    } else {
+        for (int k0 = 0; k0 < K; k0 += 2 * kX3BK) {
+            step(any_step, k0, ra1, ra0);
+            step(any_step, k0 + kX3BK, ra0, ra1);
+        }
+    }
+    if constexpr (US != 0) {
+        x3_heads_epilogue<US, NT>(reinterpret_cast<float*>(smem), acc, low, bias, *heads, m0, n0, lane, wave);
+        return;
+    }
+    if constexpr (UNIT) {
+        x3_unit_epilogue<BN, RES, RELU, UX>(reinterpret_cast<float*>(smem), acc, low, bias, res, out, M, m0, n0, lane, wave, sec.ldp, sec.n_real,
+                                            sec.act, sec.act_param);
+        return;
+    }
+
+    float* patch = reinterpret_cast<float*>(smem) + wave * (32 * WN);
+    if constexpr (TAIL_RES) {
+        fetch_res(1, 0, VPL);
+        __builtin_amdgcn_sched_barrier(0);
+    }
+#pragma unroll
+    for (int i = 0; i < 2; i++) {
+#pragma unroll
+        for (int j = 0; j < NT; j++) {
+            const int col = j * 32 + (lane & 31);
+            const float b = TAIL_RES ? reinterpret_cast<const float*>(smem + SMEM_BYTES)[wn * WN + col] : bias[n0 + wn * WN + col];
+#pragma unroll
+            for (int r = 0; r < 16; r++) {
+                const int row = (r & 3) + 8 * (r >> 2) + 4 * (lane >> 5);
+                patch[row * WN + col] = (OPA_X3_ONE_ACC ? acc[i][j][r] : acc[i][j][r] + low[i][j][r]) + b;
+            }
+        }
+        __builtin_amdgcn_fence(__ATOMIC_ACQ_REL, "wavefront");
+        __builtin_amdgcn_wave_barrier();
+#pragma unroll
+        for (int t = 0; t < VPL; t++) {
+            const int v = t * 64 + lane;
+            const int row = v / VEC_PER_ROW, c4 = (v % VEC_PER_ROW) * 4;
+            const int m = m0 + wm * 64 + i * 32 + row;
+            if (m < M) {
+                f32x4_t f = *reinterpret_cast<const f32x4_t*>(patch + row * WN + c4);
+                if constexpr (TAIL_RES) f += rres[i][t];
+                if (RELU) {
+#pragma unroll
+                    for (int e = 0; e < 4; e++) f[e] = fmaxf(f[e], 0.0f);
+                }
+                *reinterpret_cast<f32x4_t*>(out + (size_t)m * N + n0 + wn * WN + c4) = f;
+            }
+        }
+        __builtin_amdgcn_fence(__ATOMIC_ACQ_REL, "wavefront");
+        __builtin_amdgcn_wave_barrier();
+        asm volatile("" ::: "memory");
+    }
diff --git a/openpifpaf_amd/csrc/heads_x3_plan.hpp b/openpifpaf_amd/csrc/heads_x3_plan.hpp
--- /dev/null
+++ b/openpifpaf_amd/csrc/heads_x3_plan.hpp
@@ -0,0 +1,47 @@
+#pragma once
+#include "head16_plan.hpp"
+
+namespace opa {
+
+constexpr int kHeadsX3Max = 4;
+constexpr int kHeadsX3BN = 128;
+constexpr int kHeadsX3BM = 128;
+constexpr int kHeadsX3Threads = 256;
+
+struct HeadsX3Head {
+    int tile0, n_fields, n_comp, n_conf, n_vec;
+    unsigned offset_mask;
+    int n_scales;
+    float* out;
+};
+
+struct HeadsX3 {
+    int n_heads, batch, hc, wc, us;
+    HeadsX3Head head[kHeadsX3Max];
+};
+
+OPA_TILE_HD Head16Geometry heads_x3_geometry(const HeadsX3& d, const HeadsX3Head& h) {
+    return Head16Geometry{d.batch, d.hc, d.wc, h.n_fields, h.n_comp, d.us};
+}
+OPA_TILE_HD int heads_x3_n(const HeadsX3& d, const HeadsX3Head& h) { return head16_n(heads_x3_geometry(d, h)); }
+OPA_TILE_HD int heads_x3_tiles(int n) { return (n + kHeadsX3BN - 1) / kHeadsX3BN; }
+
+OPA_TILE_HD HeadsX3Head heads_x3_head_of(const HeadsX3& d, int tile) {
+    HeadsX3Head h = d.head[0];
+    OPA_TILE_UNROLL
+    for (int i = 1; i < kHeadsX3Max; i++)
+        if (i < d.n_heads && tile >= d.head[i].tile0) h = d.head[i];
+    return h;
+}
+
+OPA_TILE_HD void heads_x3_plan_rows(const HeadsX3& d, const HeadsX3Head& h, int m0, int t, Head16Row (&rows)[2]) {
+    head16_plan_rows(heads_x3_geometry(d, h), m0, t, rows);
+}
+
+template <typename Emit>
+OPA_TILE_HD void heads_x3_plan_block(const HeadsX3& d, const HeadsX3Head& h, const Head16Row& row, int tile, int j, int t, Emit&& emit) {
+    const int wn = (t >> 6) & 1;
+    head16_plan_block(heads_x3_geometry(d, h), row, (tile - h.tile0) * kHeadsX3BN + wn * kHead16WN + j * kHead16WN, t, emit);
+}
+
+}
diff --git a/openpifpaf_amd/fused.py b/openpifpaf_amd/fused.py
--- a/openpifpaf_amd/fused.py
+++ b/openpifpaf_amd/fused.py
@@ -48,6 +48,7 @@
 GCONV_BF16 = _switch('OPA_GCONV_BF16', '0')
 F16 = _switch('OPA_F16', '0')
 HEAD16 = _switch('OPA_HEAD16', '0')
+HEADS_X3 = _switch('OPA_HEADS_X3', '1')
 _ROUTES16 = {torch.bfloat16: (lambda own: own, '_bf16'), torch.float16: (lambda own: F16, '_f16')}
 
 
@@ -748,6 +749,86 @@
     return out[:, :n].contiguous(memory_format=torch.channels_last) if w3.shape[1] != n else out
 
 
+
+HEADS_X3_TILE_N = 128
+HEADS_X3_MAX = 4
+HEADS_X3_DECLINED = frozenset()
+
+
+def heads_x3_operands_of(head_nets):
+    convs = [hn.conv for hn in head_nets]
+
+    def make():
+        planes, biases = [], []
+        for conv in convs:
+            w3, bp = _unit_weight_of(conv)
+            npad = -w3.shape[1] % HEADS_X3_TILE_N
+            planes.append(torch.nn.functional.pad(w3, (0, 0, 0, npad)))
+            biases.append(torch.nn.functional.pad(bp, (0, npad)))
+        return torch.cat(planes, dim=1).contiguous(), torch.cat(biases).contiguous()
+    sources = tuple(t for conv in convs for t in (conv.weight, conv.bias))
+    return derived(convs[0], '_opa_heads_x3', sources, make)
+
+
+def _head_x3_choice(conv, x):
+    if FORCE_PICK == 'conv':
+        return False
+    m = out_pixels(x)
+    choice = _CHOICE.get(('torch.float32/head', int(m), int(conv.in_channels), int(conv.out_channels), False, False))
+    return choice == 'x3' if choice is not None else m >= 16384
+
+
+def heads_conv_fields_x3_supported(head_nets, x):
+    from . import network
+    heads = list(head_nets) if head_nets is not None else []
+    if not (HEADS_X3 and 1 <= len(heads) <= HEADS_X3_MAX and torch.is_tensor(x) and x.dim() == 4 and not torch.is_autocast_enabled()
+            and _lib.available()):
+        return False
+    us = getattr(getattr(heads[0], 'meta', None), 'upsample_stride', None)
+    if us not in (1, 2) or x.shape[0] * x.shape[2] * x.shape[3] >= 2 ** 31 or x.numel() == 0:
+        return False
+    for hn in heads:
+        if not (isinstance(hn, network.CompositeField4) and hn.fused_epilogue and not hn.training and hn.meta.upsample_stride == us):
+            return False
+        conv, meta = hn.conv, hn.meta
+        if not (head_conv_x3_supported(conv, x) and conv.bias is not None and conv.bias.dtype == torch.float32 and conv.dilation == (1, 1)
+                and conv.weight.device == x.device and conv.bias.device == x.device
+                and not (torch.is_grad_enabled() and (conv.weight.requires_grad or conv.bias.requires_grad))):
+            return False
+        n_comp, H, W = _head16_shape(conv, x, meta)
+        counts = (meta.n_fields, meta.n_confidences, meta.n_vectors, meta.n_scales)
+        if not (meta.n_fields > 0 and min(counts) >= 0 and len(meta.vector_offsets) <= 32
+                and conv.out_channels == meta.n_fields * n_comp * us * us and x.shape[0] * meta.n_fields * n_comp * H * W < 2 ** 31
+                and (conv.in_channels, conv.out_channels, us) not in HEADS_X3_DECLINED and _head_x3_choice(conv, x)):
+            return False
+    return True
+
+
+def _head_records(head_nets, outs):
+    records = (_lib.HeadFields * len(outs))()
+    for record, hn, out in zip(records, head_nets, outs):
+        meta = hn.meta
+        record.out_dev = _ptr(out)
+        record.n_fields, record.n_components = meta.n_fields, out.shape[2]
+        record.n_confidences, record.n_vectors, record.n_scales = meta.n_confidences, meta.n_vectors, meta.n_scales
+        record.vector_offset_mask = sum(1 << i for i, on in enumerate(meta.vector_offsets) if on)
+    return records
+
+
+def heads_conv_fields_x3(head_nets, x):
+    import ctypes
+    w3, bp = heads_x3_operands_of(head_nets)
+    B, k, hc, wc = x.shape
+    outs = []
+    for hn in head_nets:
+        n_comp, H, W = _head16_shape(hn.conv, x, hn.meta)
+        outs.append(torch.empty((B, hn.meta.n_fields, n_comp, H, W), dtype=torch.float32, device=x.device))
+    records = _head_records(head_nets, outs)
+    _launch('opa_heads_conv_fields_f32x3', _ptr(x), _ptr(w3), _ptr(bp), ctypes.addressof(records), len(outs), B, hc, wc, k,
+            head_nets[0].meta.upsample_stride, int(X3_TERMS))
+    return tuple(outs)
+
+
 class UnitMode(typing.NamedTuple):
     dtype: torch.dtype
     align: int
diff --git a/openpifpaf_amd/network.py b/openpifpaf_amd/network.py
--- a/openpifpaf_amd/network.py
+++ b/openpifpaf_amd/network.py
@@ -991,6 +991,8 @@
 
     def forward(self, image_batch):
         x = self.base_net(image_batch)
+        if fused.heads_conv_fields_x3_supported(self.head_nets, x):
+            return fused.heads_conv_fields_x3(self.head_nets, x)
         return tuple(hn(x) for hn in self.head_nets)
 
 
```

Result: no change. 678.0 images/s (median of 6 runs) (+0.4%).
